# ap229997/hands

Measured on AMD Instinct MI355X. Metric: hands/sec, higher is better.
Workload: dtype f32; 1 GPU; hands_light ResNet-50 x3 + feature_conv + HMR + MANO, 224x224, bz=256 samples/GPU (512 hands, 768 trunk passes); per_gpu_batch=256, global_batch=256, parallelism=dp1, rccl_ranks=1, launched_by=direct, conv3x3_stride1=winograd_f4x4:stages1234

## Files before the change

### hands_amd/_lib.py

```python
from __future__ import annotations

import ctypes as C
import os

_HERE = os.path.dirname(os.path.abspath(__file__))
LIB_PATH = os.environ.get("HANDS_HIP_LIB") or os.path.join(_HERE, "libhands_hip.so")

c_float_p = C.c_void_p


class ConvDesc(C.Structure):
    _fields_ = [(n, C.c_int32) for n in (
        "B", "H", "W", "Cin", "Ho", "Wo", "Cout", "KH", "KW", "stride", "pad",
        "in_pix_stride", "out_pix_stride", "res_pix_stride", "Kpad", "act")]


ACT_NONE, ACT_RELU, ACT_GELU, ACT_LEAKY_RELU = 0, 1, 2, 3


class ManoConsts(C.Structure):
    _fields_ = [("pose_mean", C.c_void_p), ("J_template", C.c_void_p), ("J_shapedirs", C.c_void_p),
                ("lbs_weights", C.c_void_p), ("tip_ids", C.c_void_p)]


class ManoOut(C.Structure):
    _fields_ = [("vertices", C.c_void_p), ("joints3d", C.c_void_p), ("v3d_cam", C.c_void_p),
                ("j3d_cam", C.c_void_p), ("j2d_norm", C.c_void_p), ("cam_t", C.c_void_p)]


class ManoSide(C.Structure):
    _fields_ = [("consts", ManoConsts), ("blend_w", C.c_void_p), ("blend_bias", C.c_void_p), ("rot", C.c_void_p),
                ("betas", C.c_void_p), ("cam_wp", C.c_void_p), ("out", ManoOut)]


class PackedDims(C.Structure):
    _fields_ = [(n, C.c_int32) for n in ("Cin", "Cout", "Cout_pad", "Kpad")]


class EvalIn(C.Structure):
    _fields_ = [(n, C.c_void_p) for n in (
        "pred_j3d_r", "pred_j3d_l", "gt_j3d_r", "gt_j3d_l", "pred_j2d_r", "pred_j2d_l", "gt_j2d_r", "gt_j2d_l",
        "is_valid", "right_valid", "left_valid", "joints_valid_r", "joints_valid_l")]


class EvalOut(C.Structure):
    _fields_ = [(n, C.c_void_p) for n in (
        "mpjpe_ra_h", "mpjpe_pa_ra_r", "mpjpe_pa_ra_l", "mpjpe_pa_ra_h", "mrrpe_rl", "pix_err_r", "pix_err_l")]


class EvalMaskedOut(C.Structure):
    _fields_ = [(n, C.c_void_p) for n in (
        "rao_r", "rao_l", "rao_h", "abs_r", "abs_l", "abs_h", "pa_ra_r", "pa_ra_l", "pa_ra_h")]


class MeshEvalIn(C.Structure):
    _fields_ = [(n, C.c_void_p) for n in (
        "pred_v3d_r", "pred_v3d_l", "gt_v3d_r", "gt_v3d_l", "pred_j3d_r", "pred_j3d_l", "gt_j3d_r", "gt_j3d_l",
        "is_valid", "right_valid", "left_valid")]


MESH_MAX_V, MESH_NQ = 1024, 10
MESH_QUANTITIES = ("mpvpe_ra", "f5_ra", "f15_ra", "auc_ra_v", "auc_ra_j", "mpvpe_pa", "f5_pa", "f15_pa", "auc_pa_v", "auc_pa_j")


class MeshEvalOut(C.Structure):
    _fields_ = [(f"{q}_{s}", C.c_void_p) for q in MESH_QUANTITIES for s in "rlh"]


SURF_MAX_F, SURF_CHUNK, SURF_NQ = 4096, 512, 4
SIGNED_CHUNK = 256
SURF_QUANTITIES = ("p2s_ra", "p2s_pa", "chamfer_ra", "chamfer_pa")


class SurfEvalOut(C.Structure):
    _fields_ = [(f"{q}_{s}", C.c_void_p) for q in SURF_QUANTITIES for s in "rlh"]


ACCEL_NQ = 3
ACCEL_QUANTITIES = ("acc", "acc_j", "acc_abs")


class AccelEvalOut(C.Structure):
    _fields_ = [(f"{q}_{s}", C.c_void_p) for q in ACCEL_QUANTITIES for s in "rlh"]


class SmoothSide(C.Structure):
    _fields_ = [(n, C.c_void_p) for n in ("pose", "beta", "cam", "valid", "pose_out", "beta_out", "cam_out", "state")]


SMOOTH_SHAPE_MODES = {"filter": 0, "mean": 1, "none": 2}


class SmoothCfg(C.Structure):
    _fields_ = [("min_cutoff", C.c_double * 3), ("beta", C.c_double * 3), ("d_cutoff", C.c_double * 3), ("shape_mode", C.c_int)]


class ManoFitConsts(C.Structure):
    _fields_ = [(n, C.c_void_p) for n in ("pose_mean", "J_template", "J_shapedirs", "tip_v_template", "tip_shapedirs",
                                          "tip_lbs_weights", "tip_posedirs")]


class ManoFitSide(C.Structure):
    _fields_ = [("consts", ManoFitConsts)] + [(n, C.c_void_p) for n in (
        "joints", "weights", "valid", "init_pose", "init_beta", "init_transl", "pose", "beta", "transl", "rmse", "steps")]


class FitCfg(C.Structure):
    _fields_ = [("iters", C.c_int), ("lambda_beta", C.c_double), ("lambda_pose", C.c_double), ("mu0", C.c_double)]


class ManoFit2DSide(C.Structure):
    _fields_ = [("consts", ManoFitConsts)] + [(n, C.c_void_p) for n in (
        "kp2d", "weights", "valid", "init_pose", "init_beta", "init_transl", "pose", "beta", "transl", "rmse", "steps", "start",
        "j3d", "j2d")]


class Fit2DCfg(C.Structure):
    _fields_ = [("iters_rigid", C.c_int), ("iters", C.c_int), ("lambda_beta", C.c_double), ("lambda_pose", C.c_double),
                ("mu0", C.c_double), ("robust_sigma", C.c_double), ("z_min", C.c_double), ("fit_shape", C.c_int),
                ("prior_to_init", C.c_int)]


class ManoFitVertsConsts(C.Structure):
    _fields_ = [(n, C.c_void_p) for n in ("pose_mean", "J_template", "J_shapedirs", "v_template", "shapedirs", "lbs_weights",
                                          "posedirs_vm")]


class ManoFitVertsSide(C.Structure):
    _fields_ = [("consts", ManoFitVertsConsts)] + [(n, C.c_void_p) for n in (
        "verts", "weights", "valid", "init_pose", "init_beta", "init_transl", "pose", "beta", "transl", "rmse", "steps", "j3d")]


class LossIn(C.Structure):
    _fields_ = [(n, C.c_void_p) for n in (
        "pred_pose_r", "pred_pose_l", "pred_beta_r", "pred_beta_l", "pred_j3d_r", "pred_j3d_l", "pred_j2d_r", "pred_j2d_l",
        "pred_cam_wp_r", "pred_cam_wp_l", "pred_cam_wp_init_r", "pred_cam_wp_init_l",
        "gt_pose_r", "gt_pose_l", "gt_beta_r", "gt_beta_l", "gt_j3d_r", "gt_j3d_l", "gt_j2d_r", "gt_j2d_l",
        "gt_cam_wp_r", "gt_cam_wp_l", "right_valid", "left_valid", "joints_valid_r", "joints_valid_l",
        "is_cam_loss", "is_j2d_loss", "is_j3d_loss", "is_pose_loss", "is_beta_loss",
        "pred_grasp_r", "pred_grasp_l", "gt_grasp_r", "gt_grasp_l", "grasp_valid_r", "grasp_valid_l", "is_grasp_loss",
        "pred_mask_r", "pred_mask_l", "gt_mask_r", "gt_mask_l", "render_valid_r", "render_valid_l", "is_mask_loss",
        "pred_depth_r", "pred_depth_l", "gt_depth_r", "gt_depth_l", "is_depth_loss",
        "pred_center_r", "pred_center_l", "gt_center_r", "gt_center_l",
        "pred_corner_r", "pred_corner_l", "gt_corner_r", "gt_corner_l")]


LOSS_NKEYS, LOSS_N_MANDATORY = 21, 31


class ShadeMesh(C.Structure):
    _fields_ = [("workspace", C.c_void_p), ("faces", C.c_void_p), ("valid", C.c_void_p), ("n_verts", C.c_int32),
                ("n_faces", C.c_int32), ("face_offset", C.c_int32), ("color", C.c_float * 3), ("metallic", C.c_float),
                ("roughness", C.c_float)]


SHADE_MAX_MESHES = 4


class ShadeScene(C.Structure):
    _fields_ = [("mesh", ShadeMesh * SHADE_MAX_MESHES), ("n_meshes", C.c_int32)]


_P, _I, _F = C.c_void_p, C.c_int, C.c_float
class ConvJob(C.Structure):
    _fields_ = [("desc", C.POINTER(ConvDesc)), ("in_", C.c_void_p), ("w_packed", C.c_void_p), ("bias", C.c_void_p),
                ("residual", C.c_void_p), ("out", C.c_void_p), ("pre_scale", C.c_void_p), ("pre_shift", C.c_void_p)]


SIGNATURES = {
    "hands_conv2d_nhwc_f32": [C.POINTER(ConvDesc), _P, _P, _P, _P, _P, _P],
    "hands_conv3x3_winograd_supported": [C.POINTER(ConvDesc)],
    "hands_conv3x3_winograd_f32": [C.POINTER(ConvDesc), _P, _P, _P, _P, _P],
    "hands_conv3x3_winograd4_supported": [C.POINTER(ConvDesc)],
    "hands_conv3x3_winograd4_f32": [C.POINTER(ConvDesc), _P, _P, _P, _P, _P],
    "hands_conv2d_splitk_factor": [C.POINTER(ConvDesc)],
    "hands_conv2d_group_class": [C.POINTER(ConvDesc), _I],
    "hands_conv2d_group_f32": [C.POINTER(ConvJob), _I, _P],
    "hands_conv2d_nhwc_splitk_f32": [C.POINTER(ConvDesc), _P, _P, _P, _P, _P, _P, C.c_longlong, _P],
    "hands_conv2d_nhwc_splitk_fused_f32": [C.POINTER(ConvDesc), _P, _P, _P, _P, _P, _I, _P, C.c_longlong, _P, C.c_longlong, _P],
    "hands_conv2d_streamk_grid": [C.POINTER(ConvDesc)],
    "hands_conv2d_nhwc_streamk_f32": [C.POINTER(ConvDesc), _P, _P, _P, _P, _P, _P, C.c_longlong, _I, _P],
    "hands_conv1x1_dual_nhwc_f32": [C.POINTER(ConvDesc), _P, _P, _I, _I, _I, _I, _I, _P, _P, _P, _P],
    "hands_conv2d_nhwc_splitk_n_f32": [C.POINTER(ConvDesc), _P, _P, _P, _P, _P, _I, _P, C.c_longlong, _P],
    "hands_conv2d_nhwc_pre_f32": [C.POINTER(ConvDesc), _P, _P, _P, _P, _P, _P, _P, _I, _P, C.c_longlong, _P],
    "hands_stem_conv_maxpool_nhwc_f32": [_P, _P, _P, _P, _I, _I, _I, _I, _P],
    "hands_stem_conv_maxpool_nchw_f32": [_P, _P, _P, _P, _I, _I, _I, _I, _P],
    "hands_nchw3_to_nhwc4_f32": [_P, _P, _I, _I, _I, _P],
    "hands_maxpool3x3s2_nhwc_f32": [_P, _P, _I, _I, _I, _I, _P],
    "hands_sumpool_nhwc_f32": [_P, _P, _I, _I, _I, _I, _P],
    "hands_avgpool_nhwc_f32": [_P, _P, _I, _I, _I, _I, _P],
    "hands_image_posenc_nhwc_f32": [_P, _P, _P, _P, _I, _I, _I, _I, _I, _I, _P],
    "hands_frontend_dense_maps_f32": [_P, _P, _P, _P, _I, _I, _I, _P],
    "hands_dense_posenc_f32": [_P, _P, _P, _P, _I, _I, _I, _I, _I, _I, _I, _I, _I, _I, _P],
    "hands_concat_nhwc_f32": [_P, _I, _I, _P, _I, _P, C.c_longlong, _I, _P, _I, _I, _I, _I, _P],
    "hands_upsample_bilinear_ac_f32": [_P, _P, _I, _I, _I, _I, _I, _I, _P],
    "hands_rot_leftmul_f32": [_P, _P, _I, _P],
    "hands_perspective_correction_f32": [_P, _P, _P, _P, _I, _P],
    "hands_kpe_concat_f32": [_P, _P, _P, _P, _P, _I, _I, _I, _I, _I, _P],
    "hands_hmr_init_f32": [_P, _P, _I, _I, _I, _P],
    "hands_rot6d_to_matrix_f32": [_P, _I, _P, _I, _P],
    "hands_flip_swap_f32": [_P, _P, _P, _P, _P, _P, _P, _P, _P, _I, _P],
    "hands_matrix_to_axis_angle_f32": [_P, _P, C.c_longlong, _P],
    "hands_axis_angle_to_matrix_f32": [_P, _P, C.c_longlong, _P],
    "hands_grasp_input_f32": [_P, _I, _P, _P, _P, _I, _I, _I, _I, _P],
    "hands_mano_pose_f32": [C.POINTER(ManoConsts), _P, _P, _I, _P, _I, _P, _P, _I, _P],
    "hands_mano_heads_f32": [C.POINTER(ManoSide), _I, _P, _I, _F, _F, _I, _I, _P],
    "hands_mano_heads_vsplit": [_I, _I],
    "hands_mano_skin_f32": [C.POINTER(ManoConsts), _P, _I, _P, _P, _P, _P, _F, _F, C.POINTER(ManoOut), _I, _P],
    "hands_resize_crop_nchw3_to_nhwc4_f32": [_P, _P, _I, _I, _I, _I, _I, _I, _P],
    "hands_layernorm_f32": [_P, _P, _P, _P, _P, _I, _I, _I, _F, _P],
    "hands_add_pos_f32": [_P, _P, _P, _I, _I, _I, _P],
    "hands_kpe_encode_f32": [_P, _P, _P, _I, _I, _I, _P],
    "hands_attention_f32": [_P, _P, _I, _I, _I, _I, _F, _P],
    "hands_cross_attention_1q_f32": [_P, _P, _P, _I, _I, _I, _I, _F, _P],
    "hands_rot6d_to_matrix_cols_f32": [_P, _I, _P, _I, _P],
    "hands_vit_tokens_f32": [_P, _P, _P, _P, _I, _I, _I, _P],
    "hands_vit_tail_f32": [_P, _P, _P, _P, _I, _I, _I, _F, _P],
    "hands_wide_attention_f32": [_P, C.c_longlong, _I, _P, C.c_longlong, _I, _P, C.c_longlong, _I, _P, C.c_longlong, _I,
                                 _I, _I, _I, _I, _F, _P],
    "hands_vector_tokens_f32": [_P, _I, _I, _I, _P, _P, _P, _I, _I, _I, _P],
    "hands_token_mean_f32": [_P, _P, _I, _I, _I, _P],
    "hands_upsample_bilinear_add_f32": [_P, _P, _P, _I, _I, _I, _I, _I, _I, _P],
    "hands_pool2x2_nhwc_f32": [_P, _P, _I, _I, _I, _I, _I, _P],
    "hands_channel_pool_f32": [_P, _P, C.c_longlong, _I, _P],
    "hands_gate_apply_f32": [_P, _P, _I, _P, _P, C.c_longlong, _I, _P],
    "hands_add_embed2_f32": [_P, _P, _P, _P, _P, _P, _P, _I, _I, _I, _P],
    "hands_add_rowvec_f32": [_P, _P, _P, _I, _I, _I, _P],
    "hands_token_sum_f32": [_P, _P, _I, _I, _I, _P],
    "hands_bn_leaky_f32": [_P, _P, _P, _P, C.c_longlong, _I, _P],
    "hands_upsample_nearest2x_add_f32": [_P, _P, _P, _I, _I, _I, _I, _P],
    "hands_spatial_softmax_f32": [_P, _I, _P, _P, _I, _I, _I, _I, _P],
    "hands_flash_attention_f32": [_P, _P, _P, _P, _P, _P, _P, _I, _I, _I, _I, _F, _P],
    "hands_ceiling_hbm_read_f32": [_P, C.c_longlong, _P, _P],
    "hands_eval_metrics_f32": [C.POINTER(EvalIn), C.POINTER(EvalOut), _I, _P],
    "hands_eval_metrics_masked_f32": [C.POINTER(EvalIn), _P, _P, C.POINTER(EvalMaskedOut), _I, _P],
    "hands_eval_mesh_metrics_f32": [C.POINTER(MeshEvalIn), C.POINTER(MeshEvalOut), _I, _I, _P],
    "hands_mesh_closest_f32": [_P, _P, _P, _P, _P, _P, _P, _I, _I, _I, _I, _P],
    "hands_mesh_signed_f32": [_P, _P, _P, _P, _P, _P, _P, _I, _I, _I, _I, _P],
    "hands_eval_surface_metrics_f32": [C.POINTER(MeshEvalIn), _P, _P, _I, _I, C.POINTER(SurfEvalOut), _I, _I, _P],
    "hands_accel_error_f32": [_P, _P, _P, _P, _P, _I, _I, _I, _F, _P],
    "hands_eval_accel_metrics_f32": [C.POINTER(MeshEvalIn), _P, C.POINTER(AccelEvalOut), _I, _I, _F, _P],
    "hands_smooth_mano_f32": [C.POINTER(SmoothSide), _I, _P, _I, _I, _F, C.POINTER(SmoothCfg), _P],
    "hands_mano_fit_f32": [C.POINTER(ManoFitSide), _I, C.POINTER(FitCfg), _I, _P],
    "hands_mano_fit2d_f32": [C.POINTER(ManoFit2DSide), _I, _P, C.POINTER(Fit2DCfg), _I, _P],
    "hands_mano_fit_verts_f32": [C.POINTER(ManoFitVertsSide), _I, C.POINTER(FitCfg), _I, _P],
    "hands_loss_light_f32": [C.POINTER(LossIn), _I, _I, _I, _P, _P, _P, _P, _P],
    "hands_mano_pose_aa_f32": [C.POINTER(ManoConsts), _P, _P, _I, _P, _I, _P, _P, _I, _P],
    "hands_gt_targets_f32": [_P, _P, _P, _P, _F, _P, _P, _P, _I, _I, _P],
    "hands_unnormalize_kp2d_f32": [_P, _P, C.c_longlong, _F, _P],
    "hands_frontend_boxes_f32": [_P, _P, _I, _P, _I, _I, _I, C.c_double] + [_P] * 10 + [_P],
    "hands_warp_affine_cubic_norm_f32": [_P, _P, _P, _I, _I, _I, _I, _I, C.POINTER(C.c_float), C.POINTER(C.c_float), _P],
    "hands_render_silhouette_f32": [_P, _I, _I, _P, _I, _P, _I, _I, _F, _F, _I, _P, _P, _P, _P],
    "hands_mesh_prepare_f32": [_P, _I, _I, _P, _I, _P, _P, _P, _P, _I, _I, _P, _P],
    "hands_render_shaded_f32": [C.POINTER(ShadeScene), _P, _I, _I, _P, _P, _P, _P, _P],
    "hands_pack_conv_dims": [_I, _I, _I, _I, _I, C.POINTER(PackedDims)],
    "hands_fold_bn_f32": [_I, C.c_longlong, _P, _P, _P, _P, _P, C.c_double, _P, _P],
    "hands_pack_conv_f64": [_I, _I, _I, _I, _I, _P, _P, _P, _P],
    "hands_pack_linear_f64": [_I, _I, _P, _P, _P, _I, _P, _I, _P, _P],
    "hands_pack_conv1x1_dual_f64": [_I, _I, _I, _P, _P, _P, _P, _P, _P],
    "hands_pack_mano_f32": [_P] * 10,
    "hands_pack_conv3x3_winograd_f64": [_I, _I, _P, _P],
    "hands_pack_conv3x3_winograd4_f64": [_I, _I, _P, _P],
}
EXTRA_SYMBOLS = ("hands_abi_version", "hands_error_string", "hands_conv2d_workspace_floats", "hands_pack_conv3x3_winograd_floats", "hands_conv3x3_winograd_executed_macs",
                 "hands_pack_conv3x3_winograd4_floats", "hands_conv3x3_winograd4_executed_macs",
                 "hands_conv2d_streamk_workspace_bytes", "hands_stream_is_capturing", "hands_csrc_sha16", "hands_ceiling_mfma_f32", "hands_mesh_workspace_floats",
                 "hands_loss_workspace_bytes", "hands_smooth_state_bytes")

ABI_VERSION = 5
_lib = None


def lib():
    global _lib
    if _lib is not None:
        return _lib
    if not os.path.isfile(LIB_PATH):
        raise RuntimeError(
            f"hands_amd: {LIB_PATH} not found. Build it with `python -c 'import __graft_entry__ as g; "
            "g.build()'` or `make -C hands_amd/csrc`. There is no CPU fallback.")
    h = C.CDLL(LIB_PATH)
    h.hands_abi_version.restype = C.c_int
    if h.hands_abi_version() != ABI_VERSION:
        raise RuntimeError(f"hands_amd: {LIB_PATH} has ABI version {h.hands_abi_version()}, this package needs {ABI_VERSION}: "
                           "rebuild it (`make -C hands_amd/csrc`)")
    for name, argtypes in SIGNATURES.items():
        fn = getattr(h, name)
        fn.argtypes = argtypes
        fn.restype = C.c_int
    h.hands_conv2d_workspace_floats.restype = C.c_longlong
    h.hands_conv2d_workspace_floats.argtypes = [C.POINTER(ConvDesc), C.c_int]
    h.hands_conv2d_streamk_workspace_bytes.restype = C.c_longlong
    h.hands_conv2d_streamk_workspace_bytes.argtypes = []
    h.hands_pack_conv3x3_winograd_floats.restype = C.c_longlong
    h.hands_pack_conv3x3_winograd_floats.argtypes = [C.c_int, C.c_int]
    h.hands_conv3x3_winograd_executed_macs.restype = C.c_longlong
    h.hands_conv3x3_winograd_executed_macs.argtypes = [C.POINTER(ConvDesc)]
    h.hands_pack_conv3x3_winograd4_floats.restype = C.c_longlong
    h.hands_pack_conv3x3_winograd4_floats.argtypes = [C.c_int, C.c_int]
    h.hands_conv3x3_winograd4_executed_macs.restype = C.c_longlong
    h.hands_conv3x3_winograd4_executed_macs.argtypes = [C.POINTER(ConvDesc)]
    h.hands_abi_version.restype = C.c_int
    h.hands_stream_is_capturing.restype = C.c_int
    h.hands_stream_is_capturing.argtypes = [C.c_void_p]
    h.hands_csrc_sha16.restype = C.c_char_p
    h.hands_csrc_sha16.argtypes = []
    h.hands_ceiling_mfma_f32.restype = C.c_longlong
    h.hands_ceiling_mfma_f32.argtypes = [C.c_void_p, C.c_longlong, C.c_int, C.c_int, C.c_void_p]
    h.hands_mesh_workspace_floats.restype = C.c_longlong
    h.hands_mesh_workspace_floats.argtypes = [C.c_int, C.c_int]
    h.hands_loss_workspace_bytes.restype = C.c_longlong
    h.hands_loss_workspace_bytes.argtypes = [C.c_int, C.c_int, C.c_int]
    h.hands_smooth_state_bytes.restype = C.c_longlong
    h.hands_smooth_state_bytes.argtypes = []
    h.hands_error_string.restype = C.c_char_p
    h.hands_error_string.argtypes = [C.c_int]
    _lib = h
    return h


def check(code: int, what: str = ""):
    if code != 0:
        msg = lib().hands_error_string(code).decode()
        raise RuntimeError(f"hands_amd: {what} failed with code {code}: {msg}")


def ptr(t, offset_elems: int = 0):
    if t is None:
        return None
    return t.data_ptr() + offset_elems * t.element_size()
```

### hands_amd/csrc/conv_igemm.hip

```cpp
#include <hip/hip_runtime.h>
#include <stdint.h>
#include "hands_hip.h"
#include "common.h"

namespace {

typedef unsigned int u32x4 __attribute__((ext_vector_type(4)));
typedef double f64x4 __attribute__((ext_vector_type(4)));

__device__ __forceinline__ float gelu_erf(float x) { return x * 0.5f * (1.0f + erff(x * 0.70710678118654752440f)); }

__device__ __forceinline__ float4 apply_act(float4 v, int act) {
  if (act == HANDS_ACT_RELU) {
    v = relu_f32(v);
  } else if (act == HANDS_ACT_GELU) {
    v.x = gelu_erf(v.x); v.y = gelu_erf(v.y); v.z = gelu_erf(v.z); v.w = gelu_erf(v.w);
  } else if (act == HANDS_ACT_LEAKY_RELU) {
    v.x = v.x > 0.f ? v.x : 0.01f * v.x; v.y = v.y > 0.f ? v.y : 0.01f * v.y;
    v.z = v.z > 0.f ? v.z : 0.01f * v.z; v.w = v.w > 0.f ? v.w : 0.01f * v.w;
  }
  return v;
}

__device__ __forceinline__ float f4elem(const float4& v, int t) {
  return t == 0 ? v.x : (t == 1 ? v.y : (t == 2 ? v.z : v.w));
}

constexpr int BK = 16;
constexpr int LDS_ROW = 16;
constexpr int LDS_ROW_B3 = 24;

typedef __bf16 bf16x8 __attribute__((ext_vector_type(8)));

__device__ __forceinline__ void split3(float x, uint32_t& u0, uint32_t& u1, uint32_t& u2) {
  u0 = __float_as_uint(x) & 0xffff0000u;
  const float r1 = x - __uint_as_float(u0);
  u1 = __float_as_uint(r1) & 0xffff0000u;
  const float r2 = r1 - __uint_as_float(u1);
  u2 = __float_as_uint(r2);
}

__device__ __forceinline__ void store_split4(float* dst, float4 v) {
  uint32_t a0, a1, a2, b0, b1, b2, c0, c1, c2, d0, d1, d2;
  split3(v.x, a0, a1, a2); split3(v.y, b0, b1, b2); split3(v.z, c0, c1, c2); split3(v.w, d0, d1, d2);
  *reinterpret_cast<uint2*>(dst) = make_uint2((a0 >> 16) | b0, (c0 >> 16) | d0);
  *reinterpret_cast<uint2*>(dst + 8) = make_uint2((a1 >> 16) | b1, (c1 >> 16) | d1);
  *reinterpret_cast<uint2*>(dst + 16) = make_uint2((a2 >> 16) | (b2 & 0xffff0000u), (c2 >> 16) | (d2 & 0xffff0000u));
}

struct ConvArgs {
  const float* __restrict__ in;
  const float* __restrict__ w;
  const float* __restrict__ bias;
  const float* res;
  float* out;
  int M, N, Kpad;
  int H, W, Cin, Ho, Wo, KH, KW, stride, pad;
  int in_ps, out_ps, res_ps;
  int relu;
  int nblk_m, nblk_n;
  const float* __restrict__ in2;
  int K0, H2, W2, stride2, in2_ps;
  int ksplit;
  float* partial;
  int part_ps;
  const float* pre_scale;
  const float* pre_shift;
  int* counters = nullptr;
  const float* fin_res = nullptr;
  int fin_act = 0;
};

__device__ __forceinline__ int xcd_remap(int bid, int nwg) {
  const int q = nwg >> 3, r = nwg & 7;
  const int xcd = bid & 7, idx = bid >> 3;
  const int base = (xcd < r) ? xcd * (q + 1) : r * (q + 1) + (xcd - r) * q;
  return base + idx;
}

typedef float f32x2 __attribute__((ext_vector_type(2)));

constexpr int EROW = 68;
constexpr int EPI_FLOATS = 4 * 32 * EROW;
template <int ACT, bool RES>
__device__ __forceinline__ void epilogue_full(const f32x16 (&acc)[2][2], float* sE, int lane, const float* bias_p,
                                              const char* res_u, int res_ps, char* out_u, int out_ps) {
  const int half = lane >> 5;
  float* wr = sE + (lane & 31) * EROW + half * 4;
  const float* rd = sE + (lane >> 4) * EROW + (lane & 15) * 4;
  const uint32_t o_off = (uint32_t)((lane >> 4) * out_ps + (lane & 15) * 4) * 4u;
  const uint32_t r_off = (uint32_t)((lane >> 4) * res_ps + (lane & 15) * 4) * 4u;
  const float4 bv4 = *reinterpret_cast<const float4*>(bias_p);
#ifndef HANDS_EPI_SCALAR_ADDS
  const f32x2 b01 = {bv4.x, bv4.y}, b23 = {bv4.z, bv4.w};
#endif
#pragma unroll
  for (int j = 0; j < 2; ++j) {
#pragma unroll
    for (int i = 0; i < 2; ++i)
#pragma unroll
      for (int q = 0; q < 4; ++q)
        *reinterpret_cast<float4*>(wr + i * 32 + q * 8) =
            make_float4(acc[i][j][q * 4 + 0], acc[i][j][q * 4 + 1], acc[i][j][q * 4 + 2], acc[i][j][q * 4 + 3]);
    float4 rv[RES ? 8 : 1];
    if constexpr (RES) {
#pragma unroll
      for (int r = 0; r < 8; ++r)
        rv[r] = *reinterpret_cast<const float4*>(res_u + (size_t)(j * 32 + 4 * r) * (size_t)res_ps * 4 + r_off);
    }
#pragma unroll
    for (int r = 0; r < 8; ++r) {
      const float4 t = *reinterpret_cast<const float4*>(rd + 4 * r * EROW);
#ifdef HANDS_EPI_SCALAR_ADDS
      float4 v = make_float4(t.x + bv4.x, t.y + bv4.y, t.z + bv4.z, t.w + bv4.w);
      if constexpr (RES) { v.x += rv[r].x; v.y += rv[r].y; v.z += rv[r].z; v.w += rv[r].w; }
      asm volatile("" : "+v"(v.x), "+v"(v.y), "+v"(v.z), "+v"(v.w));
#else
      f32x2 v01 = {t.x, t.y}, v23 = {t.z, t.w};
      v01 = v01 + b01;
      v23 = v23 + b23;
      if constexpr (RES) {
        const f32x2 r01 = {rv[r].x, rv[r].y}, r23 = {rv[r].z, rv[r].w};
        v01 = v01 + r01;
        v23 = v23 + r23;
      }
      float4 v = make_float4(v01.x, v01.y, v23.x, v23.y);
#endif
      if constexpr (ACT != HANDS_ACT_NONE) v = apply_act(v, ACT);
      *reinterpret_cast<float4*>(out_u + (size_t)(j * 32 + 4 * r) * (size_t)out_ps * 4 + o_off) = v;
      if (r & 1) __builtin_amdgcn_sched_barrier(0);
    }
  }
}

template <int BM, int BN, bool F64>
__device__ __forceinline__ void splitk_fused_tail(const ConvArgs& a, float* lds, int tile, int m0, int n0, int wave_u) {
  const int tid = wave_u * 64 + (int)__builtin_amdgcn_mbcnt_hi(~0u, __builtin_amdgcn_mbcnt_lo(~0u, 0u));
  volatile int& s_last = *reinterpret_cast<volatile int*>(lds);
  asm volatile("s_waitcnt vmcnt(0)" ::: "memory");
  __syncthreads();
  if (tid == 0) {
    __builtin_amdgcn_fence(__ATOMIC_RELEASE, "agent");
    asm volatile("s_waitcnt vmcnt(0)" ::: "memory");
    const int old = __hip_atomic_fetch_add(a.counters + tile, 1, __ATOMIC_RELAXED, __HIP_MEMORY_SCOPE_AGENT);
    const int last = old == a.ksplit - 1;
    if (last) __hip_atomic_store(a.counters + tile, 0, __ATOMIC_RELAXED, __HIP_MEMORY_SCOPE_AGENT);
    s_last = last;
  }
  __syncthreads();
  if (!s_last) return;
  __builtin_amdgcn_fence(__ATOMIC_ACQUIRE, "agent");
  const size_t slice = (size_t)a.M * a.part_ps;
  if constexpr (F64) {
    const double* part = reinterpret_cast<const double*>(a.partial);
    for (int idx = tid; idx < BM * BN; idx += 256) {
      const int m = m0 + idx / BN, n = n0 + idx % BN;
      if (m >= a.M || n >= a.N) continue;
      const double* p = part + (size_t)m * a.part_ps + n;
      double v = p[0];
      for (int sl = 1; sl < a.ksplit; ++sl) v += p[sl * slice];
      float f = (float)(v + (double)a.bias[n]);
      if (a.fin_res) f += a.fin_res[(size_t)m * a.res_ps + n];
      if (a.fin_act == HANDS_ACT_RELU) f = relu_f32(f);
      else if (a.fin_act == HANDS_ACT_GELU) f = gelu_erf(f);
      else if (a.fin_act == HANDS_ACT_LEAKY_RELU) f = f > 0.f ? f : 0.01f * f;
      a.out[(size_t)m * a.out_ps + n] = f;
    }
  } else {
    constexpr int C4 = BN / 4;
    for (int idx = tid; idx < BM * C4; idx += 256) {
      const int m = m0 + idx / C4, n = n0 + (idx % C4) * 4;
      if (m >= a.M || n >= a.N) continue;
      const float* p = a.partial + (size_t)m * a.part_ps + n;
      float4 v = *reinterpret_cast<const float4*>(p);
      for (int sl = 1; sl < a.ksplit; ++sl) {
        const float4 q = *reinterpret_cast<const float4*>(p + sl * slice);
        v.x += q.x; v.y += q.y; v.z += q.z; v.w += q.w;
      }
      const float4 b = *reinterpret_cast<const float4*>(a.bias + n);
      v.x += b.x; v.y += b.y; v.z += b.z; v.w += b.w;
      if (a.fin_res) {
        const float4 r = *reinterpret_cast<const float4*>(a.fin_res + (size_t)m * a.res_ps + n);
        v.x += r.x; v.y += r.y; v.z += r.z; v.w += r.w;
      }
      *reinterpret_cast<float4*>(a.out + (size_t)m * a.out_ps + n) = apply_act(v, a.fin_act);
    }
  }
}

constexpr int SK_SLOT_FLOATS = 4 * 64 * 64;

__device__ __forceinline__ void tile_coords(const ConvArgs& a, int tile, int& mt, int& nt) {
  constexpr int RASTER_GM = 8;
  if (a.nblk_n >= 8 && a.nblk_m >= RASTER_GM) {
    const int per = RASTER_GM * a.nblk_n;
    const int gidx = tile / per, idx = tile - gidx * per;
    const int gm = min(RASTER_GM, a.nblk_m - gidx * RASTER_GM);
    nt = idx / gm; mt = gidx * RASTER_GM + (idx - nt * gm);
  } else { mt = tile / a.nblk_n; nt = tile - mt * a.nblk_n; }
}

template <int WAVES_M, int WAVES_N, int MODE, int PREC = 0, bool PRE = false, int BLK = 0>
__device__ __forceinline__ void conv_tile(const ConvArgs& a, float* lds, int tile, int split, int kt0, int kt1,
                                          const float* acc_in, float* acc_out) {
  constexpr int ROW = PREC == 1 ? LDS_ROW_B3 : LDS_ROW;
  constexpr bool F64 = PREC == 2;
  constexpr bool STEM = MODE == 1;
  constexpr bool DUAL = MODE == 2;
  constexpr int BM = 64 * WAVES_M;
  constexpr int BN = 64 * WAVES_N;
  constexpr int A_ROWS = BM / 64;
  constexpr int W_ROWS = BN / 64;
  static_assert(WAVES_M * WAVES_N == 4, "4 waves per block");

  float* sX = lds;
  float* sW = lds + 2 * BM * ROW;

  const int tid = threadIdx.x;
  const int lane = tid & 63;
  const int wave = tid >> 6;
  const int wm = wave / WAVES_N;
  const int wn = wave % WAVES_N;

  int mt, nt;
  tile_coords(a, tile, mt, nt);
  const int m0 = mt * BM, n0 = nt * BN;

  const int srow = tid >> 2;
  const int chunk = tid & 3;
  const int swz_chunk = chunk ^ ((srow >> 2) & 3);
  int x_base[A_ROWS];
  int x_hi0[A_ROWS], x_wi0[A_ROWS];
  bool x_ok[A_ROWS];
  int x_base2[DUAL ? A_ROWS : 1];
  uint32_t x_mask[MODE == 0 ? A_ROWS : 1];
  int x_offb[MODE == 0 ? A_ROWS : 1];
  int x_b[A_ROWS];
  const int HoWo = a.Ho * a.Wo;
  const bool same_pixel = DUAL && a.K0 >= a.Kpad && a.stride == 1 && a.H == a.Ho && a.W == a.Wo;
#pragma unroll
  for (int i = 0; i < A_ROWS; ++i) {
    const int m = m0 + srow + 64 * i;
    x_ok[i] = m < a.M;
    const int mm = x_ok[i] ? m : 0;
    if (same_pixel) {
      x_b[i] = 0; x_hi0[i] = 0; x_wi0[i] = 0;
      x_base[i] = mm * a.in_ps;
      if constexpr (DUAL) x_base2[i] = 0;
      continue;
    }
    const int b = mm / HoWo;
    const int rem = mm - b * HoWo;
    const int ho = rem / a.Wo;
    const int wo = rem - ho * a.Wo;
    x_b[i] = b;
    x_hi0[i] = ho * a.stride - a.pad;
    x_wi0[i] = wo * a.stride - a.pad;
    x_base[i] = ((b * a.H + x_hi0[i]) * a.W + x_wi0[i]) * a.in_ps;
    if constexpr (DUAL) {
      x_base2[i] = ((b * a.H2 + ho * a.stride2) * a.W2 + wo * a.stride2) * a.in2_ps;
    }
  }
  __amdgpu_buffer_rsrc_t x_rsrc = __builtin_amdgcn_make_buffer_rsrc(const_cast<float*>(a.in), 0, (int)0x80000000u, 0x00020000);
  if constexpr (MODE == 0) {
    const int b_w = __builtin_amdgcn_readfirstlane(x_b[0]);
    x_rsrc = __builtin_amdgcn_make_buffer_rsrc(const_cast<float*>(a.in) + (size_t)b_w * a.H * a.W * a.in_ps, 0,
                                               (int)0x80000000u, 0x00020000);
#pragma unroll
    for (int i = 0; i < A_ROWS; ++i) {
      const int hb = max(0, -x_hi0[i]), he = min(a.KH, a.H - x_hi0[i]);
      const int wb = max(0, -x_wi0[i]), we = min(a.KW, a.W - x_wi0[i]);
      const uint32_t hm = he > hb ? ((1u << he) - 1u) & ~((1u << hb) - 1u) : 0u;
      const uint32_t wm = we > wb ? ((1u << we) - 1u) & ~((1u << wb) - 1u) : 0u;
      x_mask[i] = (x_ok[i] && hm != 0u && wm != 0u) ? (hm | (wm << 16)) : 0u;
      x_offb[i] = (((((x_b[i] - b_w) * a.H + x_hi0[i]) * a.W + x_wi0[i]) * a.in_ps) + chunk * 4) * 4;
    }
  }
  int x_off1[DUAL ? A_ROWS : 1], x_off2[DUAL ? A_ROWS : 1];
  __amdgpu_buffer_rsrc_t x_rsrc2 = x_rsrc;
  if constexpr (DUAL) {
    const int base1 = __builtin_amdgcn_readfirstlane(x_base[0]);
    const int base2 = __builtin_amdgcn_readfirstlane(x_base2[0]);
    x_rsrc = __builtin_amdgcn_make_buffer_rsrc(const_cast<float*>(a.in) + base1, 0, (int)0x80000000u, 0x00020000);
    x_rsrc2 = __builtin_amdgcn_make_buffer_rsrc(const_cast<float*>(a.in2) + base2, 0, (int)0x80000000u, 0x00020000);
#pragma unroll
    for (int i = 0; i < A_ROWS; ++i) {
      x_off1[i] = x_ok[i] ? (x_base[i] - base1 + chunk * 4) * 4 : chunk * 16;
      x_off2[i] = x_ok[i] ? (x_base2[i] - base2 + chunk * 4) * 4 : chunk * 16;
    }
  }
  const __amdgpu_buffer_rsrc_t w_rsrc =
      __builtin_amdgcn_make_buffer_rsrc(const_cast<float*>(a.w) + (size_t)n0 * a.Kpad, 0, (int)0x80000000u, 0x00020000);
  int w_offb[W_ROWS];
#pragma unroll
  for (int i = 0; i < W_ROWS; ++i) w_offb[i] = ((srow + 64 * i) * a.Kpad + chunk * 4) * 4;

  float4 xr[A_ROWS], wr[W_ROWS];
  static_assert(!PRE || (MODE == 2 && PREC != 1), "the input affine + LeakyReLU exists for exact-fp32 pointwise layers");
  float4 psr = make_float4(1.f, 1.f, 1.f, 1.f), pbr = make_float4(0.f, 0.f, 0.f, 0.f);
  int kh = 0, kw = 0, c0 = 0, woff = 0;
  const int ntaps = a.KH * a.KW;
  const int cw = (a.Cin & 31) == 0 ? 2 * BK : BK;

#define LOAD_TILES(KT)                                                                              \
  do {                                                                                              \
    if constexpr (STEM) {                                                                           \
                                          \
      const int tap = (KT) * 4 + chunk;                                                             \
      const int tkh = tap / a.KW;                                                                   \
      const int tkw = tap - tkh * a.KW;                                                             \
      const int toff = (tkh * a.W + tkw) * a.in_ps;                                                 \
      _Pragma("unroll") for (int i = 0; i < A_ROWS; ++i) {                                          \
        const bool ok = x_ok[i] && tap < ntaps && (unsigned)(x_hi0[i] + tkh) < (unsigned)a.H &&     \
                        (unsigned)(x_wi0[i] + tkw) < (unsigned)a.W;                                 \
        xr[i] = ok ? *reinterpret_cast<const float4*>(a.in + (x_base[i] + toff))                    \
                   : make_float4(0.f, 0.f, 0.f, 0.f);                                               \
      }                                                                                             \
    } else if constexpr (DUAL) {                                                                    \
       \
       \
       \
      const bool second = (KT) * BK >= a.K0;                                                        \
      const int soff = ((KT) * BK - (second ? a.K0 : 0)) * 4;                                       \
      _Pragma("unroll") for (int i = 0; i < A_ROWS; ++i) {                                          \
        const u32x4 ld = second ? __builtin_amdgcn_raw_buffer_load_b128(x_rsrc2, x_off2[i], soff, 0) \
                                : __builtin_amdgcn_raw_buffer_load_b128(x_rsrc, x_off1[i], soff, 0);  \
        xr[i] = make_float4(__uint_as_float(ld.x), __uint_as_float(ld.y), __uint_as_float(ld.z), __uint_as_float(ld.w)); \
      }                                                                                             \
    } else {                                                                                        \
       \
       \
       \
      const bool kvalid = c0 < a.Cin;              \
      const uint32_t sel = kvalid ? ((1u << kh) | (0x10000u << kw)) : 0x80000000u;   \
      const int toffb = ((kh * a.W + kw) * a.in_ps + c0) * 4;                                       \
      _Pragma("unroll") for (int i = 0; i < A_ROWS; ++i) {                                          \
        const bool ok = (x_mask[i] & sel) == sel;                                                   \
        const u32x4 ld = __builtin_amdgcn_raw_buffer_load_b128(x_rsrc, ok ? x_offb[i] + toffb : (int)0x80000000u, 0, 0); \
        xr[i] = make_float4(__uint_as_float(ld.x), __uint_as_float(ld.y), __uint_as_float(ld.z), __uint_as_float(ld.w)); \
      }                                                                                             \
      woff = kvalid ? (kh * a.KW + kw) * a.Cin + c0 : (KT) * BK;                                    \
      c0 += BK;                                                                                     \
      if ((c0 & (cw - 1)) == 0) {              \
        c0 -= cw;                                                                                   \
        if (++kw == a.KW) { kw = 0; if (++kh == a.KH) { kh = 0; c0 += cw; } }                       \
      }                                                                                             \
    }                                                                                               \
    if constexpr (MODE != 0) woff = (KT) * BK;                                                      \
    if constexpr (PRE) {                                                                            \
      psr = *reinterpret_cast<const float4*>(a.pre_scale + (KT) * BK + chunk * 4);                  \
      pbr = *reinterpret_cast<const float4*>(a.pre_shift + (KT) * BK + chunk * 4);                  \
    }                                                                                               \
    _Pragma("unroll") for (int i = 0; i < W_ROWS; ++i) {                                            \
      const u32x4 ld = __builtin_amdgcn_raw_buffer_load_b128(w_rsrc, w_offb[i], woff * 4, 0);        \
      wr[i] = make_float4(__uint_as_float(ld.x), __uint_as_float(ld.y), __uint_as_float(ld.z), __uint_as_float(ld.w)); \
    }                                                                                               \
  } while (0)

#define STORE_TILES(BUF)                                                                            \
  do {                                                                                              \
    if constexpr (PRE) {                                                                            \
      _Pragma("unroll") for (int i = 0; i < A_ROWS; ++i) {                                          \
        float4 v = make_float4(xr[i].x * psr.x + pbr.x, xr[i].y * psr.y + pbr.y, xr[i].z * psr.z + pbr.z, xr[i].w * psr.w + pbr.w); \
        v.x = v.x > 0.f ? v.x : 0.01f * v.x; v.y = v.y > 0.f ? v.y : 0.01f * v.y;                   \
        v.z = v.z > 0.f ? v.z : 0.01f * v.z; v.w = v.w > 0.f ? v.w : 0.01f * v.w;                   \
        xr[i] = v;                                                                                  \
      }                                                                                             \
    }                                                                                               \
    if constexpr (PREC != 1) {                                                                      \
      float* dx = sX + (BUF) * BM * ROW + srow * ROW + swz_chunk * 4;                               \
      float* dw = sW + (BUF) * BN * ROW + srow * ROW + swz_chunk * 4;                               \
      _Pragma("unroll") for (int i = 0; i < A_ROWS; ++i)                                            \
        *reinterpret_cast<float4*>(dx + 64 * i * ROW) = xr[i];                                      \
      _Pragma("unroll") for (int i = 0; i < W_ROWS; ++i)                                            \
        *reinterpret_cast<float4*>(dw + 64 * i * ROW) = wr[i];                                      \
    } else {                                                                                        \
      float* dx = sX + (BUF) * BM * ROW + srow * ROW + chunk * 2;                                   \
      float* dw = sW + (BUF) * BN * ROW + srow * ROW + chunk * 2;                                   \
      _Pragma("unroll") for (int i = 0; i < A_ROWS; ++i) store_split4(dx + 64 * i * ROW, xr[i]);    \
      _Pragma("unroll") for (int i = 0; i < W_ROWS; ++i) store_split4(dw + 64 * i * ROW, wr[i]);    \
    }                                                                                               \
  } while (0)

  f64x4 accd[F64 ? 4 : 1][F64 ? 4 : 1];
  if constexpr (F64) {
#pragma unroll
    for (int i = 0; i < 4; ++i)
#pragma unroll
      for (int j = 0; j < 4; ++j) accd[i][j] = f64x4{0.0, 0.0, 0.0, 0.0};
  }
  f32x16 acc[2][2];
  if (acc_in != nullptr) {
    const float4* src = reinterpret_cast<const float4*>(acc_in) + (wave * 16) * 64 + lane;
#pragma unroll
    for (int i = 0; i < 2; ++i)
#pragma unroll
      for (int j = 0; j < 2; ++j)
#pragma unroll
        for (int q = 0; q < 4; ++q) {
          const float4 v = src[((i * 2 + j) * 4 + q) * 64];
          acc[i][j][q * 4 + 0] = v.x; acc[i][j][q * 4 + 1] = v.y; acc[i][j][q * 4 + 2] = v.z; acc[i][j][q * 4 + 3] = v.w;
        }
  } else {
#pragma unroll
    for (int i = 0; i < 2; ++i)
#pragma unroll
      for (int j = 0; j < 2; ++j)
#pragma unroll
        for (int r = 0; r < 16; ++r) acc[i][j][r] = 0.f;
  }

  if constexpr (MODE == 0) {
    if (kt0 > 0) {
      const int spt = cw / BK;
      const int ch0 = kt0 / (ntaps * spt);
      const int r0 = kt0 - ch0 * ntaps * spt;
      const int tap0 = r0 / spt;
      c0 = ch0 * cw + (r0 - tap0 * spt) * BK;
      kh = tap0 / a.KW;
      kw = tap0 - kh * a.KW;
    }
  }
#ifdef HANDS_PRO_PRIO
  __builtin_amdgcn_s_setprio(HANDS_PRO_PRIO);
#endif
  LOAD_TILES(kt0);
  STORE_TILES(0);
  __syncthreads();
#ifdef HANDS_PRO_PRIO
  __builtin_amdgcn_s_setprio(0);
#endif

  const int frag = PREC == 1 ? (lane & 31) * ROW + (lane >> 5) * 4
                   : F64     ? (lane & 15) * ROW + (((lane >> 4) ^ ((lane >> 2) & 3)) * 4)
                             : (lane & 31) * ROW + (((lane >> 5) ^ ((lane >> 2) & 3)) * 4);
  const float* fw = sW + (wn * 64) * ROW + frag;
  const float* fx = sX + (wm * 64) * ROW + frag;
  const float* fw1 = sW + (wn * 64) * ROW + (frag ^ 8);
  const float* fx1 = sX + (wm * 64) * ROW + (frag ^ 8);

#define COMPUTE_STEP(BUF)                                                                           \
  do {                                                                                              \
    if constexpr (F64) {                                                                            \
      float4 wf[4], xf[4];                 \
      _Pragma("unroll") for (int i = 0; i < 4; ++i) {                                               \
        wf[i] = *reinterpret_cast<const float4*>(fw + (BUF) * BN * ROW + i * 16 * ROW);             \
        xf[i] = *reinterpret_cast<const float4*>(fx + (BUF) * BM * ROW + i * 16 * ROW);             \
      }                                                                                             \
      _Pragma("unroll") for (int t = 0; t < 4; ++t) {                                               \
        double wd[4], xd[4];                                                                        \
        _Pragma("unroll") for (int i = 0; i < 4; ++i) {                                             \
          wd[i] = (double)f4elem(wf[i], t);                                                         \
          xd[i] = (double)f4elem(xf[i], t);                                                         \
        }                                                                                           \
        _Pragma("unroll") for (int i = 0; i < 4; ++i) {                                             \
          _Pragma("unroll") for (int j = 0; j < 4; ++j) {                                           \
            accd[i][j] = __builtin_amdgcn_mfma_f64_16x16x4f64(wd[i], xd[j], accd[i][j], 0, 0, 0);   \
          }                                                                                         \
        }                                                                                           \
      }                                                                                             \
    } else if constexpr (PREC == 0) {                                                               \
      float4 wf[2][2], xf[2][2];                                            \
      _Pragma("unroll") for (int kk = 0; kk < 2; ++kk) {                                            \
        _Pragma("unroll") for (int i = 0; i < 2; ++i) {                                             \
          wf[i][kk] = *reinterpret_cast<const float4*>((kk ? fw1 : fw) + (BUF) * BN * ROW + i * 32 * ROW); \
          xf[i][kk] = *reinterpret_cast<const float4*>((kk ? fx1 : fx) + (BUF) * BM * ROW + i * 32 * ROW); \
        }                                                                                           \
      }                                                                                             \
      _Pragma("unroll") for (int kk = 0; kk < 2; ++kk) {                                            \
        _Pragma("unroll") for (int t = 0; t < 4; ++t) {                                             \
          _Pragma("unroll") for (int i = 0; i < 2; ++i) {                                           \
            _Pragma("unroll") for (int j = 0; j < 2; ++j) {                                         \
              acc[i][j] = __builtin_amdgcn_mfma_f32_32x32x2f32(f4elem(wf[i][kk], t), f4elem(xf[j][kk], t), \
                                                               acc[i][j], 0, 0, 0);                  \
            }                                                                                       \
          }                                                                                         \
        }                                                                                           \
      }                                                                                             \
    } else {                                                                                        \
        \
      bf16x8 wf[2][3], xf[2][3];                                         \
      _Pragma("unroll") for (int p = 0; p < 3; ++p) {                                               \
        _Pragma("unroll") for (int i = 0; i < 2; ++i) {                                             \
          wf[i][p] = *reinterpret_cast<const bf16x8*>(fw + (BUF) * BN * ROW + i * 32 * ROW + p * 8); \
          xf[i][p] = *reinterpret_cast<const bf16x8*>(fx + (BUF) * BM * ROW + i * 32 * ROW + p * 8); \
        }                                                                                           \
      }                                                                                             \
                             \
      _Pragma("unroll") for (int q = 0; q < 6; ++q) {                                               \
        constexpr int PA[6] = {2, 1, 0, 1, 0, 0};                                                   \
        constexpr int PB[6] = {0, 1, 2, 0, 1, 0};                                                   \
        _Pragma("unroll") for (int i = 0; i < 2; ++i) {                                             \
          _Pragma("unroll") for (int j = 0; j < 2; ++j) {                                           \
            acc[i][j] = __builtin_amdgcn_mfma_f32_32x32x16_bf16(wf[i][PA[q]], xf[j][PB[q]], acc[i][j], 0, 0, 0); \
          }                                                                                         \
        }                                                                                           \
      }                                                                                             \
    }                                                                                               \
  } while (0)

  static_assert(BLK == 0 || ((BLK & (BLK - 1)) == 0 && PREC == 0), "block length: a power of two k-steps, exact fp32 only");
  static_assert(!F64 || (WAVES_M == 2 && WAVES_N == 2), "fp64 accumulation: the 128 x 128 tile only");
  f32x16 tot[BLK ? 2 : 1][BLK ? 2 : 1];
  if constexpr (BLK > 0) {
#pragma unroll
    for (int i = 0; i < 2; ++i)
#pragma unroll
      for (int j = 0; j < 2; ++j)
#pragma unroll
        for (int r = 0; r < 16; ++r) tot[i][j][r] = 0.f;
  }
  for (int kt = kt0; kt + 1 < kt1; ++kt) {
    const int buf = (kt - kt0) & 1;
    LOAD_TILES(kt + 1);
    COMPUTE_STEP(buf);
    if constexpr (BLK > 0) {
      if (((kt - kt0 + 1) & (BLK - 1)) == 0) {
#pragma unroll
        for (int i = 0; i < 2; ++i)
#pragma unroll
          for (int j = 0; j < 2; ++j)
#pragma unroll
            for (int r = 0; r < 16; ++r) { tot[i][j][r] += acc[i][j][r]; acc[i][j][r] = 0.f; }
      }
    }
    STORE_TILES(buf ^ 1);
    __syncthreads();
  }
  COMPUTE_STEP((kt1 - 1 - kt0) & 1);
#ifdef HANDS_EPI_PRIO
  __builtin_amdgcn_s_setprio(HANDS_EPI_PRIO);
#endif
  if constexpr (BLK > 0) {
#pragma unroll
    for (int i = 0; i < 2; ++i)
#pragma unroll
      for (int j = 0; j < 2; ++j)
#pragma unroll
        for (int r = 0; r < 16; ++r) acc[i][j][r] += tot[i][j][r];
  }
#undef COMPUTE_STEP

  __syncthreads();
  if (acc_out != nullptr) {
    float4* dst = reinterpret_cast<float4*>(acc_out) + (wave * 16) * 64 + lane;
#pragma unroll
    for (int i = 0; i < 2; ++i)
#pragma unroll
      for (int j = 0; j < 2; ++j)
#pragma unroll
        for (int q = 0; q < 4; ++q)
          dst[((i * 2 + j) * 4 + q) * 64] =
              make_float4(acc[i][j][q * 4 + 0], acc[i][j][q * 4 + 1], acc[i][j][q * 4 + 2], acc[i][j][q * 4 + 3]);
    return;
  }
  float* sE = lds + wave * (32 * EROW);
  const int half = lane >> 5;
  const int c4 = lane & 15;
  const int n_lane = n0 + wn * 64 + c4 * 4;
  const bool n_ok = n_lane < a.N;
  const bool part = a.ksplit > 1;
#ifdef HANDS_ABL_NO_EPI
  if (!part && m0 + BM <= a.M && n0 + BN <= a.N) {
    float sacc = 0.f;
#pragma unroll
    for (int i = 0; i < 2; ++i)
#pragma unroll
      for (int j = 0; j < 2; ++j) sacc += acc[i][j][0] + acc[i][j][7] + acc[i][j][15];
    if (sacc == 123456.789f) a.out[(size_t)m0 * a.out_ps + n0 + lane] = sacc;
    return;
  }
#endif
  if (!F64 && !part && m0 + BM <= a.M && n0 + BN <= a.N) {
    const int wave_u = __builtin_amdgcn_readfirstlane(wave);
    const int mw = m0 + (wave_u / WAVES_N) * 64, nw = n0 + (wave_u % WAVES_N) * 64;
    char* ou = reinterpret_cast<char*>(a.out) + ((size_t)mw * a.out_ps + nw) * 4;
    const char* ru = reinterpret_cast<const char*>(a.res) + ((size_t)mw * a.res_ps + nw) * 4;
    const float* bp = a.bias + n_lane;
#define HANDS_EPI(ACT)                                                                            \
    if (a.res != nullptr) epilogue_full<ACT, true>(acc, sE, lane, bp, ru, a.res_ps, ou, a.out_ps); \
    else                  epilogue_full<ACT, false>(acc, sE, lane, bp, ru, a.res_ps, ou, a.out_ps)
    if (a.relu == HANDS_ACT_RELU) { HANDS_EPI(HANDS_ACT_RELU); }
    else if (a.relu == HANDS_ACT_NONE) { HANDS_EPI(HANDS_ACT_NONE); }
    else if (a.relu == HANDS_ACT_LEAKY_RELU) { HANDS_EPI(HANDS_ACT_LEAKY_RELU); }
    else { HANDS_EPI(HANDS_ACT_GELU); }
#undef HANDS_EPI
    return;
  }
  const float4 bv = (part || F64) ? make_float4(0.f, 0.f, 0.f, 0.f) : *reinterpret_cast<const float4*>(a.bias + n_lane);
  double bd[F64 ? 4 : 1][F64 ? 4 : 1];
  if constexpr (F64) {
#pragma unroll
    for (int i = 0; i < 4; ++i)
#pragma unroll
      for (int r = 0; r < 4; ++r) {
        const int ch = n0 + wn * 64 + 16 * i + (lane >> 4) + 4 * r;
        bd[i][r] = (!part && ch < a.N) ? (double)a.bias[ch] : 0.0;
      }
    if (part) {
      double* pd = reinterpret_cast<double*>(a.partial) + (size_t)split * a.M * a.part_ps;
#pragma unroll
      for (int i = 0; i < 4; ++i)
#pragma unroll
        for (int jb = 0; jb < 4; ++jb)
#pragma unroll
          for (int r = 0; r < 4; ++r) {
            const int ch = n0 + wn * 64 + 16 * i + (lane >> 4) + 4 * r;
            const int m = m0 + wm * 64 + 16 * jb + (lane & 15);
            if (m < a.M && ch < a.N) pd[(size_t)m * a.part_ps + ch] = accd[i][jb][r];
          }
      return;
    }
  }
  const bool has_res = !part && a.res != nullptr;
  const int act = part ? HANDS_ACT_NONE : a.relu;
  float* const obase = part ? a.partial + (size_t)split * a.M * a.part_ps : a.out;
  const int ops = part ? a.part_ps : a.out_ps;
#pragma unroll
  for (int j = 0; j < 2; ++j) {
    if constexpr (F64) {
#pragma unroll
      for (int i = 0; i < 4; ++i)
#pragma unroll
        for (int jj = 0; jj < 2; ++jj)
#pragma unroll
          for (int r = 0; r < 4; ++r)
            sE[(jj * 16 + (lane & 15)) * EROW + 16 * i + (lane >> 4) + 4 * r] = (float)(accd[i][2 * j + jj][r] + bd[i][r]);
    } else {
#pragma unroll
    for (int i = 0; i < 2; ++i)
#pragma unroll
      for (int q = 0; q < 4; ++q)
        *reinterpret_cast<float4*>(sE + (lane & 31) * EROW + i * 32 + q * 8 + half * 4) =
            make_float4(acc[i][j][q * 4 + 0], acc[i][j][q * 4 + 1], acc[i][j][q * 4 + 2], acc[i][j][q * 4 + 3]);
    }
    const int mbase = m0 + wm * 64 + j * 32 + (lane >> 4);
    float4 rv[8];
#pragma unroll
    for (int r = 0; r < 8; ++r) {
      const int m = mbase + 4 * r;
      const int mc = m < a.M ? m : a.M - 1;
      rv[r] = has_res ? *reinterpret_cast<const float4*>(a.res + (size_t)mc * a.res_ps + (n_ok ? n_lane : 0))
                      : make_float4(0.f, 0.f, 0.f, 0.f);
    }
#pragma unroll
    for (int r = 0; r < 8; ++r) {
      const int m = mbase + 4 * r;
      const float4 t = *reinterpret_cast<const float4*>(sE + ((lane >> 4) + 4 * r) * EROW + c4 * 4);
      float4 v;
      v.x = t.x + bv.x + rv[r].x;
      v.y = t.y + bv.y + rv[r].y;
      v.z = t.z + bv.z + rv[r].z;
      v.w = t.w + bv.w + rv[r].w;
      v = apply_act(v, act);
      if (m < a.M && n_ok) *reinterpret_cast<float4*>(obase + (size_t)m * ops + n_lane) = v;
    }
  }
#undef LOAD_TILES
#undef STORE_TILES
}

template <int WAVES_M, int WAVES_N, int MODE, int PREC = 0, bool PRE = false, int BLK = 0>
__global__ void __launch_bounds__(256, 2) conv_igemm_f32_kernel(ConvArgs a) {
  constexpr int RING = 2 * (64 * WAVES_M + 64 * WAVES_N) * (PREC == 1 ? LDS_ROW_B3 : LDS_ROW);
  __shared__ __attribute__((aligned(16))) float lds[RING > EPI_FLOATS ? RING : EPI_FLOATS];
  const int ntiles = a.nblk_m * a.nblk_n;
  const int split = a.ksplit > 1 ? blockIdx.x / ntiles : 0;
  const int tile = xcd_remap(a.ksplit > 1 ? blockIdx.x - split * ntiles : blockIdx.x, ntiles);
  const int nk_all = a.Kpad / BK;
  const int kt0 = a.ksplit > 1 ? (int)((long long)split * nk_all / a.ksplit) : 0;
  const int kt1 = a.ksplit > 1 ? (int)((long long)(split + 1) * nk_all / a.ksplit) : nk_all;
  const int wave_u = __builtin_amdgcn_readfirstlane((int)(threadIdx.x >> 6));
  conv_tile<WAVES_M, WAVES_N, MODE, PREC, PRE, BLK>(a, lds, tile, split, kt0, kt1, nullptr, nullptr);
  if (a.ksplit > 1 && a.counters != nullptr) {
    int mt, nt;
    tile_coords(a, tile, mt, nt);
    splitk_fused_tail<64 * WAVES_M, 64 * WAVES_N, PREC == 2>(a, lds, tile, mt * 64 * WAVES_M, nt * 64 * WAVES_N, wave_u);
  }
}

constexpr int GROUP_MAX = 8;
struct GroupArgs {
  ConvArgs a[GROUP_MAX];
  int start[GROUP_MAX + 1];
  int n;
};

template <int WAVES_M, int WAVES_N, int MODE, bool PRE, int BLK>
__global__ void __launch_bounds__(256, 2) conv_igemm_group_f32_kernel(GroupArgs g) {
  constexpr int RING = 2 * (64 * WAVES_M + 64 * WAVES_N) * LDS_ROW;
  __shared__ __attribute__((aligned(16))) float lds[RING > EPI_FLOATS ? RING : EPI_FLOATS];
  int p = 0;
#pragma unroll
  for (int i = 1; i < GROUP_MAX; ++i)
    if (i < g.n && (int)blockIdx.x >= g.start[i]) p = i;
  const ConvArgs& a = g.a[p];
  const int ntiles = a.nblk_m * a.nblk_n;
  const int local = (int)blockIdx.x - g.start[p];
  if ((local >> 3) >= (ntiles >> 3) + ((local & 7) < (ntiles & 7) ? 1 : 0)) return;
  conv_tile<WAVES_M, WAVES_N, MODE, 0, PRE, BLK>(a, lds, xcd_remap(local, ntiles), 0, 0, a.Kpad / BK, nullptr, nullptr);
}

struct SkArgs {
  float* slots;
  int* flags;
  int epoch;
};

template <int WAVES_M, int WAVES_N, int MODE>
__global__ void __launch_bounds__(256, 2) conv_igemm_sk_f32_kernel(ConvArgs a, SkArgs sk) {
  constexpr int RING = 2 * (64 * WAVES_M + 64 * WAVES_N) * LDS_ROW;
  __shared__ __attribute__((aligned(16))) float lds[RING > EPI_FLOATS ? RING : EPI_FLOATS];
  __shared__ int s_ready;
  const int G = gridDim.x;
  const int g = xcd_remap(blockIdx.x, G);
  const int ntiles = a.nblk_m * a.nblk_n;
  const int nk = a.Kpad / BK;
  const long long total = (long long)ntiles * nk;
  const long long u0 = total * g / G, u1 = total * (g + 1) / G;
  const int ta = (int)(u0 / nk), ka = (int)(u0 - (long long)ta * nk);
  const int tb = (int)(u1 / nk), kb = (int)(u1 - (long long)tb * nk);

  const bool inside = ta == tb;
  const int first_full = ka > 0 ? ta + 1 : ta;
  const int nfull = inside ? 0 : tb - first_full;
  const int head = (!inside && kb > 0) ? 1 : 0;
  const int nseg = inside ? 1 : head + nfull + (ka > 0 ? 1 : 0);
  for (int sgi = 0; sgi < nseg; ++sgi) {
    int tile, k0 = 0, k1 = nk;
    const float* ain = nullptr;
    float* aout = nullptr;
    if (sgi < head) {
      tile = tb; k1 = kb;
      aout = sk.slots + (size_t)g * SK_SLOT_FLOATS;
    } else if (sgi - head < nfull) {
      tile = first_full + (sgi - head);
    } else if (inside && ka == 0) {
      tile = ta; k1 = kb;
      aout = sk.slots + (size_t)g * SK_SLOT_FLOATS;
    } else {
      if (threadIdx.x == 0) {
        int ok = 0;
        for (int spin = 0; spin < 4096 && !ok; ++spin) {
          ok = __hip_atomic_load(sk.flags + (g - 1), __ATOMIC_RELAXED, __HIP_MEMORY_SCOPE_AGENT) == sk.epoch;
          if (!ok) __builtin_amdgcn_s_sleep(8);
        }
        if (ok) __builtin_amdgcn_fence(__ATOMIC_ACQUIRE, "agent");
        s_ready = ok;
      }
      __syncthreads();
      tile = ta;
      if (s_ready != 0) { k0 = ka; ain = sk.slots + (size_t)(g - 1) * SK_SLOT_FLOATS; }
      if (inside) { k1 = kb; aout = sk.slots + (size_t)g * SK_SLOT_FLOATS; }
    }
    __syncthreads();
    conv_tile<WAVES_M, WAVES_N, MODE>(a, lds, tile, 0, k0, k1, ain, aout);
    if (aout != nullptr) {
      asm volatile("s_waitcnt vmcnt(0)" ::: "memory");
      __syncthreads();
      if (threadIdx.x == 0) {
        __builtin_amdgcn_fence(__ATOMIC_RELEASE, "agent");
        asm volatile("s_waitcnt vmcnt(0)" ::: "memory");
        if (sk.epoch > 0) __hip_atomic_store(sk.flags + g, sk.epoch, __ATOMIC_RELAXED, __HIP_MEMORY_SCOPE_AGENT);
      }
    }
  }
}

template <int WAVES_M, int WAVES_N, int MODE, int PREC = 0, bool PRE = false, int BLK = 0>
int launch(ConvArgs& a, hipStream_t stream) {
  constexpr int BM = 64 * WAVES_M, BN = 64 * WAVES_N;
  a.nblk_m = (a.M + BM - 1) / BM;
  a.nblk_n = (a.N + BN - 1) / BN;
  const long long nwg = (long long)a.nblk_m * a.nblk_n * (a.ksplit > 1 ? a.ksplit : 1);
  if (nwg <= 0 || nwg > 0x7fffffffLL) return HANDS_EINVAL;
  hipLaunchKernelGGL((conv_igemm_f32_kernel<WAVES_M, WAVES_N, MODE, PREC, PRE, BLK>), dim3((unsigned)nwg), dim3(256), 0,
                     stream, a);
  return (int)hipGetLastError();
}

template <int MODE, bool PRE = false>
int launch_fp32(const hands_conv_desc* d, ConvArgs& a, hipStream_t s) {
  const bool narrow = d->Cout <= 64;
  if (d->act & HANDS_ACC_F64) return launch<2, 2, MODE, 2, PRE>(a, s);
  if (d->act & HANDS_SUM_BLOCK128) return narrow ? launch<4, 1, MODE, 0, PRE, 8>(a, s) : launch<2, 2, MODE, 0, PRE, 8>(a, s);
  if (d->act & HANDS_SUM_BLOCK64) return narrow ? launch<4, 1, MODE, 0, PRE, 4>(a, s) : launch<2, 2, MODE, 0, PRE, 4>(a, s);
  return narrow ? launch<4, 1, MODE, 0, PRE>(a, s) : launch<2, 2, MODE, 0, PRE>(a, s);
}

constexpr int SK_MAX_G = 1024;

int device_cus() {
  static int cus = 0;
  if (cus == 0) {
    int dev = 0, n = 0;
    if (hipGetDevice(&dev) == hipSuccess &&
        hipDeviceGetAttribute(&n, hipDeviceAttributeMultiprocessorCount, dev) == hipSuccess && n > 0)
      cus = n;
    else
      cus = 256;
  }
  return cus;
}

template <int WAVES_M, int WAVES_N, int MODE>
int sk_blocks_per_cu() {
  static int occ = 0;
  if (occ == 0) {
    int n = 0;
    if (hipOccupancyMaxActiveBlocksPerMultiprocessor(&n, conv_igemm_sk_f32_kernel<WAVES_M, WAVES_N, MODE>, 256, 0) != hipSuccess || n < 1)
      n = 1;
    occ = n > 4 ? 4 : n;
  }
  return occ;
}

int streamk_grid(long long ntiles, int nk, int cus, int max_per_cu) {
  if (ntiles > cus + cus / 8 && ntiles < 2LL * cus && nk >= 128 && max_per_cu >= 2) {
    return 2 * cus;
  }
  if (nk < 16 || ntiles < 2LL * cus || ntiles > 8LL * cus) return 0;
  const double per_cu = (double)ntiles / cus;
  const long long rounds = (ntiles + cus - 1) / cus;
  if (per_cu / (double)rounds > 0.95) return 0;
  long long j = ntiles / cus;
  if (j > max_per_cu) j = max_per_cu;
  long long G = j * cus;
  if (G > SK_MAX_G) G = SK_MAX_G / cus * cus;
  return G >= cus ? (int)G : 0;
}

template <int WAVES_M, int WAVES_N, int MODE>
int launch_streamk(ConvArgs& a, hipStream_t stream, void* workspace, long long workspace_bytes, int epoch) {
  constexpr int BM = 64 * WAVES_M, BN = 64 * WAVES_N;
  a.nblk_m = (a.M + BM - 1) / BM;
  a.nblk_n = (a.N + BN - 1) / BN;
  const long long ntiles = (long long)a.nblk_m * a.nblk_n;
  const int G = (workspace && epoch != 0 && a.ksplit <= 1)
                    ? streamk_grid(ntiles, a.Kpad / BK, device_cus(), sk_blocks_per_cu<WAVES_M, WAVES_N, MODE>()) : 0;
  const long long need = (long long)G * SK_SLOT_FLOATS * 4 + (long long)SK_MAX_G * 4;
  if (G == 0 || workspace_bytes < need) return launch<WAVES_M, WAVES_N, MODE>(a, stream);
  SkArgs sk;
  sk.flags = reinterpret_cast<int*>(workspace);
  sk.slots = reinterpret_cast<float*>(reinterpret_cast<char*>(workspace) + SK_MAX_G * 4);
  sk.epoch = epoch;
  hipLaunchKernelGGL((conv_igemm_sk_f32_kernel<WAVES_M, WAVES_N, MODE>), dim3((unsigned)G), dim3(256), 0, stream, a, sk);
  return (int)hipGetLastError();
}

__global__ void splitk_reduce_kernel(const float* __restrict__ partial, int S, int M, int N4, int part_ps,
                                     const float* __restrict__ bias, const float* res, int res_ps, float* out, int out_ps,
                                     int act) {
  const long long total = (long long)M * N4;
  for (long long i = blockIdx.x * (long long)blockDim.x + threadIdx.x; i < total; i += (long long)gridDim.x * blockDim.x) {
    const int n = (int)(i % N4) * 4;
    const long long m = i / N4;
    float4 v = *reinterpret_cast<const float4*>(partial + m * part_ps + n);
    for (int s = 1; s < S; ++s) {
      const float4 p = *reinterpret_cast<const float4*>(partial + ((long long)s * M + m) * part_ps + n);
      v.x += p.x; v.y += p.y; v.z += p.z; v.w += p.w;
    }
    const float4 b = *reinterpret_cast<const float4*>(bias + n);
    v.x += b.x; v.y += b.y; v.z += b.z; v.w += b.w;
    if (res) {
      const float4 r = *reinterpret_cast<const float4*>(res + m * res_ps + n);
      v.x += r.x; v.y += r.y; v.z += r.z; v.w += r.w;
    }
    *reinterpret_cast<float4*>(out + m * out_ps + n) = apply_act(v, act);
  }
}

__global__ void splitk_reduce_f64_kernel(const double* __restrict__ partial, int S, int M, int N, int part_ps,
                                         const float* __restrict__ bias, const float* res, int res_ps, float* out, int out_ps,
                                         int act) {
  const long long total = (long long)M * N;
  for (long long i = blockIdx.x * (long long)blockDim.x + threadIdx.x; i < total; i += (long long)gridDim.x * blockDim.x) {
    const int n = (int)(i % N);
    const long long m = i / N;
    double v = partial[m * part_ps + n];
    for (int s = 1; s < S; ++s) v += partial[((long long)s * M + m) * part_ps + n];
    float f = (float)(v + (double)bias[n]);
    if (res) f += res[m * res_ps + n];
    if (act == HANDS_ACT_RELU) f = relu_f32(f);
    else if (act == HANDS_ACT_GELU) f = gelu_erf(f);
    else if (act == HANDS_ACT_LEAKY_RELU) f = f > 0.f ? f : 0.01f * f;
    out[m * out_ps + n] = f;
  }
}

int splitk_factor(const hands_conv_desc* d) {
  if (d->KH != 1 || d->KW != 1 || d->H != 1 || d->W != 1 || d->stride != 1 || d->pad != 0 || d->Cin == 4) return 1;
  const long long M = d->B;
  if (M > 2048 || d->Kpad < 512) return 1;
  int s = d->Kpad / 256;
  return s > 8 ? 8 : s;
}

bool conv_geometry_ok(const hands_conv_desc* d) {
  if (d->B <= 0 || d->H <= 0 || d->W <= 0 || d->Ho <= 0 || d->Wo <= 0 || d->KH <= 0 || d->KW <= 0 || d->stride <= 0 ||
      d->pad < 0)
    return false;
  if ((d->act & HANDS_ACT_MASK) > HANDS_ACT_LEAKY_RELU || (d->act & ~(HANDS_ACT_MASK | HANDS_MATH_BF16X3 | HANDS_SUM_BLOCK128 | HANDS_SUM_BLOCK64 | HANDS_ACC_F64))) return false;
  if ((d->act & HANDS_ACC_F64) && ((d->act & (HANDS_MATH_BF16X3 | HANDS_SUM_BLOCK128 | HANDS_SUM_BLOCK64)) || d->Cin == 4)) return false;
  if ((d->act & HANDS_SUM_BLOCK128) && (d->act & (HANDS_SUM_BLOCK64 | HANDS_MATH_BF16X3))) return false;
  if ((d->act & HANDS_SUM_BLOCK64) && (d->act & HANDS_MATH_BF16X3)) return false;
  if (d->Cin % 4 || d->Cout % 4 || d->Kpad % BK || d->Kpad < d->KH * d->KW * d->Cin) return false;
  if (d->Cin != 4 && d->Cin % 16) return false;
  if (d->in_pix_stride < d->Cin || d->out_pix_stride < d->Cout) return false;
  if (d->in_pix_stride % 4 || d->out_pix_stride % 4) return false;
  if (d->H + 2 * d->pad < d->KH || d->W + 2 * d->pad < d->KW) return false;
  if (d->Ho > (d->H + 2 * d->pad - d->KH) / d->stride + 1 || d->Wo > (d->W + 2 * d->pad - d->KW) / d->stride + 1) return false;
  if ((long long)d->B * d->H * d->W * d->in_pix_stride >= (1LL << 31)) return false;
  if (d->Cin != 4) {
    const long long imgs = 256 / ((long long)d->Ho * d->Wo) + 2;
    if (imgs * d->H * d->W * d->in_pix_stride * 4 >= (1LL << 31)) return false;
    if (256LL * d->Kpad * 4 >= (1LL << 31)) return false;
    if (!(d->KH == 1 && d->KW == 1 && d->pad == 0) && (d->KH > 15 || d->KW > 15)) return false;
  }
  return true;
}

bool residual_ok(const hands_conv_desc* d, const float* residual) {
  return residual == nullptr || (d->res_pix_stride >= 0 && d->res_pix_stride % 4 == 0);
}

bool pointwise_route_ok(const hands_conv_desc* d) {
  return d->KH == 1 && d->KW == 1 && d->pad == 0 && d->Cin != 4 && d->Kpad == d->Cin &&
         (long long)(d->Ho - 1) * d->stride < d->H && (long long)(d->Wo - 1) * d->stride < d->W;
}

void fill_plain_args(const hands_conv_desc* d, const float* in, const float* w_packed, const float* bias, const float* residual,
                     float* out, const float* pre_scale, const float* pre_shift, ConvArgs& a) {
  a.in = in; a.w = w_packed; a.bias = bias; a.res = residual; a.out = out;
  a.M = d->B * d->Ho * d->Wo; a.N = d->Cout; a.Kpad = d->Kpad;
  a.H = d->H; a.W = d->W; a.Cin = d->Cin; a.Ho = d->Ho; a.Wo = d->Wo;
  a.KH = d->KH; a.KW = d->KW; a.stride = d->stride; a.pad = d->pad;
  a.in_ps = d->in_pix_stride; a.out_ps = d->out_pix_stride; a.res_ps = d->res_pix_stride;
  a.relu = d->act & HANDS_ACT_MASK;
  a.ksplit = 1; a.partial = nullptr; a.part_ps = 0; a.pre_scale = pre_scale; a.pre_shift = pre_shift;
  a.in2 = in; a.K0 = 1 << 30; a.H2 = a.W2 = a.stride2 = a.in2_ps = 0;
  a.nblk_m = a.nblk_n = 0;
}

int launch_conv(const hands_conv_desc* d, ConvArgs& a, bool pre, bool bf16x3, hipStream_t s) {
  const bool narrow = d->Cout <= 64;
  if (d->Cin == 4) return narrow ? launch<4, 1, 1>(a, s) : launch<2, 2, 1>(a, s);
  if (pre) return launch_fp32<2, true>(d, a, s);
  const bool pointwise = a.K0 < a.Kpad || pointwise_route_ok(d);
  if (bf16x3) {
    if (pointwise) return narrow ? launch<4, 1, 2, 1>(a, s) : launch<2, 2, 2, 1>(a, s);
    return narrow ? launch<4, 1, 0, 1>(a, s) : launch<2, 2, 0, 1>(a, s);
  }
  return pointwise ? launch_fp32<2>(d, a, s) : launch_fp32<0>(d, a, s);
}

int group_class(const hands_conv_desc* d, bool pre) {
  if (!d || !conv_geometry_ok(d) || !pointwise_route_ok(d)) return -1;
  if (d->act & (HANDS_MATH_BF16X3 | HANDS_SUM_BLOCK128 | HANDS_ACC_F64)) return -1;
  return (d->Cout <= 64 ? 1 : 0) | ((d->act & HANDS_SUM_BLOCK64) ? 2 : 0) | (pre ? 4 : 0);
}

template <int WAVES_M, int WAVES_N, bool PRE, int BLK>
int launch_group(GroupArgs& g, hipStream_t stream) {
  constexpr int BM = 64 * WAVES_M, BN = 64 * WAVES_N;
  long long total = 0;
  for (int p = 0; p < g.n; ++p) {
    ConvArgs& a = g.a[p];
    a.nblk_m = (a.M + BM - 1) / BM;
    a.nblk_n = (a.N + BN - 1) / BN;
    g.start[p] = (int)total;
    total += ((long long)a.nblk_m * a.nblk_n + 7) / 8 * 8;
    if (total > 0x7fffffffLL) return HANDS_EINVAL;
  }
  for (int p = g.n; p <= GROUP_MAX; ++p) g.start[p] = (int)total;
  hipLaunchKernelGGL((conv_igemm_group_f32_kernel<WAVES_M, WAVES_N, 2, PRE, BLK>), dim3((unsigned)total), dim3(256), 0, stream, g);
  return (int)hipGetLastError();
}

}

extern "C" int hands_conv2d_group_class(const hands_conv_desc* d, int pre) { return group_class(d, pre != 0); }

extern "C" int hands_conv2d_group_f32(const hands_conv_job* jobs, int n, hands_stream_t stream) {
  if (!jobs || n < 1 || n > GROUP_MAX) return HANDS_EINVAL;
  GroupArgs g{};
  g.n = n;
  int cls = -2;
  for (int p = 0; p < n; ++p) {
    const hands_conv_job& j = jobs[p];
    if (!j.desc || !j.in || !j.w_packed || !j.bias || !j.out || ((j.pre_scale != nullptr) != (j.pre_shift != nullptr))) return HANDS_EINVAL;
    const int c = group_class(j.desc, j.pre_scale != nullptr);
    if (c < 0 || (cls != -2 && c != cls)) return HANDS_EINVAL;
    if (!residual_ok(j.desc, j.residual)) return HANDS_EINVAL;
    cls = c;
    fill_plain_args(j.desc, j.in, j.w_packed, j.bias, j.residual, j.out, j.pre_scale, j.pre_shift, g.a[p]);
  }
  hipStream_t s = (hipStream_t)stream;
  switch (cls) {
    case 0: return launch_group<2, 2, false, 0>(g, s);
    case 1: return launch_group<4, 1, false, 0>(g, s);
    case 2: return launch_group<2, 2, false, 4>(g, s);
    case 3: return launch_group<4, 1, false, 4>(g, s);
    case 4: return launch_group<2, 2, true, 0>(g, s);
    case 5: return launch_group<4, 1, true, 0>(g, s);
    case 6: return launch_group<2, 2, true, 4>(g, s);
    case 7: return launch_group<4, 1, true, 4>(g, s);
  }
  return HANDS_EINVAL;
}

extern "C" int hands_conv2d_splitk_factor(const hands_conv_desc* d) { return d ? splitk_factor(d) : 0; }

extern "C" long long hands_conv2d_workspace_floats(const hands_conv_desc* d, int S) {
  if (!d || !conv_geometry_ok(d)) return -1;
  if (S <= 0) S = splitk_factor(d);
  if (S > d->Kpad / BK) S = d->Kpad / BK;
  if (S <= 1) return 0;
  return (long long)S * d->B * d->Ho * d->Wo * d->Cout * ((d->act & HANDS_ACC_F64) ? 2 : 1);
}

extern "C" int hands_conv2d_nhwc_f32(const hands_conv_desc* d, const float* in, const float* w_packed,
                                     const float* bias, const float* residual, float* out,
                                     hands_stream_t stream) {
  if (!d || !in || !w_packed || !bias || !out) return HANDS_EINVAL;
  if (!conv_geometry_ok(d) || !residual_ok(d, residual)) return HANDS_EINVAL;
  ConvArgs a;
  fill_plain_args(d, in, w_packed, bias, residual, out, nullptr, nullptr, a);
  return launch_conv(d, a, false, (d->act & HANDS_MATH_BF16X3) != 0, (hipStream_t)stream);
}

extern "C" long long hands_conv2d_streamk_workspace_bytes(void) {
  return (long long)SK_MAX_G * SK_SLOT_FLOATS * 4 + (long long)SK_MAX_G * 4;
}

extern "C" int hands_conv2d_streamk_grid(const hands_conv_desc* d) {
  if (!d || !conv_geometry_ok(d) || d->Cin == 4) return 0;
  const bool narrow = d->Cout <= 64;
  const long long M = (long long)d->B * d->Ho * d->Wo;
  const long long ntiles = narrow ? ((M + 255) / 256) * ((d->Cout + 63) / 64) : ((M + 127) / 128) * ((d->Cout + 127) / 128);
  return streamk_grid(ntiles, d->Kpad / BK, device_cus(), 4);
}

extern "C" int hands_conv2d_nhwc_streamk_f32(const hands_conv_desc* d, const float* in, const float* w_packed,
                                             const float* bias, const float* residual, float* out, void* workspace,
                                             long long workspace_bytes, int epoch, hands_stream_t stream) {
  if (!d || !in || !w_packed || !bias || !out) return HANDS_EINVAL;
  if (!conv_geometry_ok(d) || !residual_ok(d, residual)) return HANDS_EINVAL;
  if (d->Cin == 4 || (d->act & (HANDS_MATH_BF16X3 | HANDS_SUM_BLOCK128 | HANDS_SUM_BLOCK64 | HANDS_ACC_F64)))
    return hands_conv2d_nhwc_f32(d, in, w_packed, bias, residual, out, stream);
  ConvArgs a;
  fill_plain_args(d, in, w_packed, bias, residual, out, nullptr, nullptr, a);
  hipStream_t s = (hipStream_t)stream;
  if (pointwise_route_ok(d))
    return (d->Cout <= 64) ? launch_streamk<4, 1, 2>(a, s, workspace, workspace_bytes, epoch)
                           : launch_streamk<2, 2, 2>(a, s, workspace, workspace_bytes, epoch);
  return (d->Cout <= 64) ? launch_streamk<4, 1, 0>(a, s, workspace, workspace_bytes, epoch)
                         : launch_streamk<2, 2, 0>(a, s, workspace, workspace_bytes, epoch);
}

extern "C" int hands_conv1x1_dual_nhwc_f32(const hands_conv_desc* d, const float* in, const float* in2, int Cin2, int H2,
                                           int W2, int stride2, int in2_pix_stride, const float* w_packed,
                                           const float* bias, float* out, hands_stream_t stream) {
  if (!d || !in || !in2 || !w_packed || !bias || !out) return HANDS_EINVAL;
  if (d->B <= 0 || d->KH != 1 || d->KW != 1 || d->stride != 1 || d->pad != 0 || d->H != d->Ho || d->W != d->Wo)
    return HANDS_EINVAL;
  if (d->Cin % 16 || Cin2 <= 0 || Cin2 % 16 || d->Cout % 4 || d->Kpad != d->Cin + Cin2) return HANDS_EINVAL;
  if (d->in_pix_stride < d->Cin || in2_pix_stride < Cin2 || d->out_pix_stride < d->Cout || stride2 < 1) return HANDS_EINVAL;
  if (d->in_pix_stride % 4 || in2_pix_stride % 4 || d->out_pix_stride % 4) return HANDS_EINVAL;
  if ((d->Ho - 1) * stride2 >= H2 || (d->Wo - 1) * stride2 >= W2) return HANDS_EINVAL;
  if ((long long)d->B * d->H * d->W * d->in_pix_stride >= (1LL << 31) ||
      (long long)d->B * H2 * W2 * in2_pix_stride >= (1LL << 31))
    return HANDS_EINVAL;
  {
    const long long imgs = 256 / ((long long)d->Ho * d->Wo) + 2;
    if (imgs * d->H * d->W * d->in_pix_stride * 4 >= (1LL << 31) || imgs * H2 * W2 * in2_pix_stride * 4 >= (1LL << 31) ||
        256LL * d->Kpad * 4 >= (1LL << 31))
      return HANDS_EINVAL;
  }
  if (d->act & HANDS_ACC_F64) return HANDS_EINVAL;
  ConvArgs a;
  fill_plain_args(d, in, w_packed, bias, nullptr, out, nullptr, nullptr, a);
  a.in2 = in2; a.K0 = d->Cin; a.H2 = H2; a.W2 = W2; a.stride2 = stride2; a.in2_ps = in2_pix_stride;
  hands_conv_desc one_chain = *d;
  one_chain.act &= ~(HANDS_SUM_BLOCK128 | HANDS_SUM_BLOCK64);
  return launch_conv(&one_chain, a, false, (d->act & HANDS_MATH_BF16X3) != 0, (hipStream_t)stream);
}

namespace {
int splitk_launch(const hands_conv_desc* d, const float* in, const float* w_packed, const float* bias, const float* residual,
                  float* out, int S, float* workspace, long long workspace_floats,
                  hands_stream_t stream, const float* pre_scale = nullptr, const float* pre_shift = nullptr,
                  int* counters = nullptr, long long n_counters = 0) {
  if (!d) return HANDS_EINVAL;
  const bool pre = pre_scale != nullptr;
  if (pre && (!pre_shift || !pointwise_route_ok(d) || (d->act & HANDS_MATH_BF16X3))) return HANDS_EINVAL;
  const long long M = (long long)d->B * d->Ho * d->Wo;
  const int part_ps = d->Cout;
  if (S > d->Kpad / BK) S = d->Kpad / BK;
  const bool f64 = (d->act & HANDS_ACC_F64) != 0;
  const bool split = S > 1 && workspace && workspace_floats >= (long long)S * M * part_ps * (f64 ? 2 : 1) &&
                     !(f64 && (((uintptr_t)workspace) & 7));
  if (!split && !pre) return hands_conv2d_nhwc_f32(d, in, w_packed, bias, residual, out, stream);
  if (!in || !w_packed || !bias || !out || !conv_geometry_ok(d) || !residual_ok(d, residual) || (split && S > 64)) return HANDS_EINVAL;
  ConvArgs a;
  fill_plain_args(d, in, w_packed, bias, residual, out, pre_scale, pre_shift, a);
  if (split) {
    a.ksplit = S; a.partial = workspace; a.part_ps = part_ps;
    const bool narrow = d->Cout <= 64 && !f64;
    const long long ntiles = narrow ? ((M + 255) / 256) * ((d->Cout + 63) / 64) : ((M + 127) / 128) * ((d->Cout + 127) / 128);
    if (counters && n_counters >= ntiles) { a.counters = counters; a.fin_res = residual; a.fin_act = d->act & HANDS_ACT_MASK; }
  }
  hipStream_t s = (hipStream_t)stream;
  const int rc = launch_conv(d, a, pre, false, s);
  if (rc || !split || a.counters != nullptr) return rc;
  if (f64) {
    hipLaunchKernelGGL(splitk_reduce_f64_kernel, dim3(hands_grid_1d(M * d->Cout, 256)), dim3(256), 0, s,
                       reinterpret_cast<const double*>(workspace), S, (int)M, d->Cout, part_ps, bias, residual, d->res_pix_stride,
                       out, d->out_pix_stride, d->act & HANDS_ACT_MASK);
    return (int)hipGetLastError();
  }
  const long long total = M * (d->Cout / 4);
  hipLaunchKernelGGL(splitk_reduce_kernel, dim3(hands_grid_1d(total, 256)), dim3(256), 0, s, workspace, S, (int)M,
                     d->Cout / 4, part_ps, bias, residual, d->res_pix_stride, out, d->out_pix_stride, d->act & HANDS_ACT_MASK);
  return (int)hipGetLastError();
}
}

extern "C" int hands_conv2d_nhwc_pre_f32(const hands_conv_desc* d, const float* in, const float* pre_scale,
                                         const float* pre_shift, const float* w_packed, const float* bias,
                                         const float* residual, float* out, int S, float* workspace,
                                         long long workspace_floats, hands_stream_t stream) {
  if (!pre_scale || !pre_shift) return HANDS_EINVAL;
  return splitk_launch(d, in, w_packed, bias, residual, out, S, workspace, workspace_floats, stream, pre_scale, pre_shift);
}

extern "C" int hands_conv2d_nhwc_splitk_n_f32(const hands_conv_desc* d, const float* in, const float* w_packed,
                                              const float* bias, const float* residual, float* out, int S,
                                              float* workspace, long long workspace_floats, hands_stream_t stream) {
  return splitk_launch(d, in, w_packed, bias, residual, out, S, workspace, workspace_floats, stream);
}

extern "C" int hands_conv2d_nhwc_splitk_fused_f32(const hands_conv_desc* d, const float* in, const float* w_packed,
                                                  const float* bias, const float* residual, float* out, int S,
                                                  float* workspace, long long workspace_floats, int* counters,
                                                  long long n_counters, hands_stream_t stream) {
  return splitk_launch(d, in, w_packed, bias, residual, out, S, workspace, workspace_floats, stream, nullptr, nullptr, counters,
                       n_counters);
}

extern "C" int hands_conv2d_nhwc_splitk_f32(const hands_conv_desc* d, const float* in, const float* w_packed,
                                            const float* bias, const float* residual, float* out, float* workspace,
                                            long long workspace_floats, hands_stream_t stream) {
  if (!d) return HANDS_EINVAL;
  return hands_conv2d_nhwc_splitk_n_f32(d, in, w_packed, bias, residual, out, splitk_factor(d), workspace,
                                        workspace_floats, stream);
}
```

### hands_amd/engine.py

```python
from __future__ import annotations

import ctypes as C
from typing import NamedTuple

import torch

from ._lib import ConvDesc, ConvJob, check, ptr

MATH_BF16X3 = 0x100
_SUM_BLOCK = {128: 0x200, 64: 0x400}
ACC_F64 = 0x800


class ConvEngine:
    def __init__(self):
        self.use_splitk = True
        self.latency_mode = False
        self.overlap = True
        self.fuse_stem_pool = True
        self.fuse_downsample = True
        self.stream_k = "auto"
        self.math = "fp32"
        self.winograd = True
        self.winograd4 = False
        self.fuse_mano = True
        self.fuse_pre = True
        self.chain_limit = 0
        self.chain_min_k = 0
        self.chain_skip_tokens = False
        self.chain_max_pix = 0
        self.chain_in_kernel = False
        self.acc64 = True
        self.fuse_splitk_reduce = True
        self.group_launches = True
        self.last_acc64 = False
        self.hook = None
        self.last_wino_macs = 0
        self.last_sum_block = 0
        self._splitk_ws = {}
        self._sk_ws = {}
        self._capture_ws = {}
        self._capture_tables = {}
        self._capture_seq = 0

    def clone_settings(self) -> "ConvEngine":
        e = ConvEngine()
        for k in ("use_splitk", "latency_mode", "overlap", "fuse_stem_pool", "fuse_downsample", "winograd", "winograd4", "fuse_mano", "fuse_pre", "stream_k", "math", "chain_limit",
                  "chain_min_k", "chain_max_pix", "chain_skip_tokens", "chain_in_kernel", "acc64", "group_launches", "fuse_splitk_reduce"):
            setattr(e, k, getattr(self, k))
        return e

    def begin_capture(self) -> int:
        self._capture_seq += 1
        self._capture_ws = self._capture_tables[self._capture_seq] = {}
        return self._capture_seq

    def drop_capture(self, token: int):
        t = self._capture_tables.pop(token, None)
        if t is not None and t is self._capture_ws:
            self._capture_ws = {}

    def release_workspaces(self, dev=None):
        for table in (self._splitk_ws, self._sk_ws, self._capture_ws, *self._capture_tables.values()):
            for key in [k for k in table if dev is None or k[0] == dev]:
                del table[key]

    @staticmethod
    def _capturing(L, stream):
        st = L.hands_stream_is_capturing(stream)
        if st < 0:
            raise RuntimeError(f"hands_amd: hipStreamIsCapturing failed: {L.hands_error_string(-st).decode()}")
        return bool(st)

    def _workspace(self, dev, stream, need, capturing):
        key = (dev, stream)
        table = self._capture_ws if capturing else self._splitk_ws
        ws = table.get(key)
        if ws is None or ws.numel() < need:
            if ws is not None and not capturing:
                torch.cuda.synchronize(dev)
            ws = table[key] = torch.empty(max(need, 1 << 22), dtype=torch.float32, device=dev)
        return ws

    def _counters(self, L, dev, stream):
        if self._capturing(L, stream):
            return None
        key = (dev, stream, "ctr")
        c = self._splitk_ws.get(key)
        if c is None:
            c = self._splitk_ws[key] = torch.zeros(16384, dtype=torch.int32, device=dev)
            torch.cuda.current_stream(dev).synchronize()
        return c

    def _desc(self, pc, B, H, W, act, in_ps, out_ps, res_ps, has_res, out_hw=None):
        Ho = (H + 2 * pc.pad - pc.KH) // pc.stride + 1
        Wo = (W + 2 * pc.pad - pc.KW) // pc.stride + 1
        if out_hw is not None:
            if not (0 < out_hw[0] <= Ho and 0 < out_hw[1] <= Wo):
                raise ValueError(f"hands_amd: out_hw {tuple(out_hw)} is not inside the layer's {Ho} x {Wo} output map")
            Ho, Wo = out_hw
        return ConvDesc(B, H, W, pc.Cin, Ho, Wo, pc.Cout, pc.KH, pc.KW, pc.stride, pc.pad, in_ps or pc.Cin, out_ps or pc.Cout,
                        (pc.Cout if res_ps is None else res_ps) if has_res else 0, pc.Kpad,
                        int(act) | (MATH_BF16X3 if self.math == "bf16x3" else 0))

    def _route(self, L, pc, d, stream, kind="conv", has_res=False, pre=False, splitk=False, splitk_n=0, aligned=False):
        fp32 = self.math == "fp32"
        acc64 = bool(self.acc64 and pc.acc64 and fp32 and pc.Cin != 4)
        if acc64:
            d.act |= ACC_F64
        if kind == "dual":
            return _Route("dual", 1, 0, acc64, "conv_igemm_f32_kernel")
        S = 1
        if kind == "conv":
            if self.use_splitk:
                S = splitk_n if splitk_n > 1 else (L.hands_conv2d_splitk_factor(C.byref(d)) if splitk else 1)
            if self.latency_mode and not acc64:
                bm, bn = (256, 64) if pc.Cout <= 64 else (128, 128)
                tiles = -(-(d.B * d.Ho * d.Wo) // bm) * -(-pc.Cout // bn)
                if tiles <= 128:
                    S = max(S, min(256 // tiles, pc.Kpad // 128, 32))
            if not acc64 and self.winograd and not has_res and not pre and S <= 1 and fp32 and aligned:
                if self.winograd4 and pc.wino4 is not None and L.hands_conv3x3_winograd4_supported(C.byref(d)):
                    return _Route("wino4", S, 0, False, "conv_wino4_f32_kernel")
                if pc.wino is not None and L.hands_conv3x3_winograd_supported(C.byref(d)):
                    return _Route("wino", S, 0, False, "conv_wino_f32_kernel")
        limit = self.chain_limit if pc.sum_block < 0 else (pc.sum_block if self.chain_limit else 0)
        sum_block = 0
        if (limit and not acc64 and fp32 and (self.chain_in_kernel or self.use_splitk)
                and pc.Kpad >= max(2 * limit, self.chain_min_k)
                and (not self.chain_max_pix or d.Ho * d.Wo <= self.chain_max_pix)
                and not (self.chain_skip_tokens and d.H * d.W == 1 and d.B >= 4096)):
            sum_block = limit
            if self.chain_in_kernel:
                if limit not in _SUM_BLOCK:
                    raise ValueError(f"hands_amd: chain_in_kernel takes chain_limit 64 or 128, not {limit}")
                d.act |= _SUM_BLOCK[limit]
            else:
                S = max(S, min(pc.Kpad // limit, 32))
        if kind == "group":
            groupable = not acc64 and (self.chain_in_kernel or not limit)
            cls = L.hands_conv2d_group_class(C.byref(d), int(pre)) if groupable else -1
            return _Route("group" if cls >= 0 else "conv", S, sum_block, acc64, "conv_igemm_group_f32_kernel", cls=cls)
        if S > 1:
            capturing = self._capturing(L, stream)
            entry = "pre" if pre else ("splitk_fused" if self.fuse_splitk_reduce and not capturing else "splitk")
            return _Route(entry, S, sum_block, acc64, "conv_igemm_splitk_f32_kernel", capturing)
        if pre:
            return _Route("pre", S, sum_block, acc64, "conv_igemm_f32_kernel")
        if (not sum_block and not acc64 and fp32 and ((not self.overlap) if self.stream_k == "auto" else self.stream_k)
                and L.hands_conv2d_streamk_grid(C.byref(d)) > 0 and not self._capturing(L, stream)):
            return _Route("streamk", S, 0, False, "conv_igemm_sk_f32_kernel")
        return _Route("plain", S, sum_block, acc64, "conv_igemm_f32_kernel")

    def _launch(self, kernel, pc, npix, stream, has_res, fn, *args):
        hook = self.hook
        if hook is not None:
            hook("begin", pc, npix, stream, has_res, kernel)
        check(fn(*args), fn.__name__)
        if hook is not None:
            hook("end", pc, npix, stream, has_res, kernel)

    def conv(self, L, pc, x, B, H, W, out, relu, stream, res=None, in_ps=None, out_ps=None, res_ps=None,
             x_off=0, out_off=0, res_off=0, splitk=False, splitk_n=0, pre=None, out_hw=None):
        d = self._desc(pc, B, H, W, relu, in_ps, out_ps, res_ps, res is not None, out_hw)
        xp, op, wp, bp = ptr(x, x_off), ptr(out, out_off), ptr(pc.w), ptr(pc.bias)
        rp = ptr(res, res_off) if res is not None else None
        r = self._route(L, pc, d, stream, "conv", res is not None, pre is not None, splitk, splitk_n, (xp | op) % 16 == 0)
        self.last_sum_block, self.last_acc64 = r.sum_block, r.acc64
        dp = C.byref(d)
        if r.entry == "wino4":
            if self.hook is not None:
                self.last_wino_macs = L.hands_conv3x3_winograd4_executed_macs(dp)
            fn, args = L.hands_conv3x3_winograd4_f32, (dp, xp, ptr(pc.wino4), bp, op, stream)
        elif r.entry == "wino":
            if self.hook is not None:
                self.last_wino_macs = L.hands_conv3x3_winograd_executed_macs(dp)
            fn, args = L.hands_conv3x3_winograd_f32, (dp, xp, ptr(pc.wino), bp, op, stream)
        elif r.entry == "streamk":
            key = (x.device, stream)
            sk = self._sk_ws.get(key)
            if sk is None:
                nbytes = L.hands_conv2d_streamk_workspace_bytes()
                sk = self._sk_ws[key] = [torch.zeros(nbytes // 4, dtype=torch.int32, device=x.device), 0]
                torch.cuda.current_stream(x.device).synchronize()
            sk[1] = sk[1] % 0x7FFFFFF0 + 1
            fn, args = L.hands_conv2d_nhwc_streamk_f32, (dp, xp, wp, bp, rp, op, ptr(sk[0]), sk[0].numel() * 4, sk[1], stream)
        elif r.entry == "plain":
            fn, args = L.hands_conv2d_nhwc_f32, (dp, xp, wp, bp, rp, op, stream)
        else:
            ws = self._workspace(x.device, stream, L.hands_conv2d_workspace_floats(dp, r.S), r.capturing) if r.S > 1 else None
            wsp, wsn = (ptr(ws), ws.numel()) if ws is not None else (None, 0)
            if r.entry == "pre":
                fn, args = L.hands_conv2d_nhwc_pre_f32, (dp, xp, ptr(pre[0]), ptr(pre[1]), wp, bp, rp, op, r.S, wsp, wsn, stream)
            elif r.entry == "splitk_fused":
                ctr = self._counters(L, x.device, stream)
                fn, args = L.hands_conv2d_nhwc_splitk_fused_f32, (dp, xp, wp, bp, rp, op, r.S, wsp, wsn, ptr(ctr), ctr.numel(), stream)
            else:
                fn, args = L.hands_conv2d_nhwc_splitk_n_f32, (dp, xp, wp, bp, rp, op, r.S, wsp, wsn, stream)
        self._launch(r.kernel, pc, B * d.Ho * d.Wo, stream, res is not None, fn, *args)
        return d.Ho, d.Wo

    def conv_group(self, L, jobs, stream):
        single = lambda j: self.conv(L, j["pc"], j["x"], j["B"], j["H"], j["W"], j["out"], j.get("relu", 0), stream,
                                     **{k: j[k] for k in ("res", "pre", "in_ps", "out_ps", "res_ps", "x_off", "out_off", "res_off") if k in j})
        if len(jobs) < 2 or not self.group_launches or self.latency_mode or self.math != "fp32":
            for j in jobs:
                single(j)
            return
        classes = {}
        for j in jobs:
            pc = j["pc"]
            d = self._desc(pc, j["B"], j["H"], j["W"], j.get("relu", 0), j.get("in_ps"), j.get("out_ps"), j.get("res_ps"),
                           j.get("res") is not None)
            r = self._route(L, pc, d, stream, "group", pre=j.get("pre") is not None)
            j["_d"], j["_npix"], j["_sum_block"] = d, j["B"] * d.Ho * d.Wo, r.sum_block
            classes.setdefault(r.cls, []).append(j)
        for cls, members in classes.items():
            for chunk in ([members[i:i + 8] for i in range(0, len(members), 8)] if cls >= 0 else [[j] for j in members]):
                if len(chunk) == 1:
                    single(chunk[0])
                    continue
                arr = (ConvJob * len(chunk))()
                for k, j in enumerate(chunk):
                    pc, res, pre = j["pc"], j.get("res"), j.get("pre")
                    arr[k] = ConvJob(C.pointer(j["_d"]), ptr(j["x"], j.get("x_off", 0)), ptr(pc.w), ptr(pc.bias),
                                     ptr(res, j.get("res_off", 0)) if res is not None else None, ptr(j["out"], j.get("out_off", 0)),
                                     ptr(pre[0]) if pre is not None else None, ptr(pre[1]) if pre is not None else None)
                self.last_sum_block, self.last_acc64 = chunk[0]["_sum_block"], False
                gp = _GroupPC(chunk) if self.hook is not None else None
                self._launch("conv_igemm_group_f32_kernel", gp, gp.npix if gp else 0, stream,
                             any(j.get("res") is not None for j in chunk), L.hands_conv2d_group_f32, arr, len(chunk), stream)

    def conv_dual(self, L, pc, split, x, x2, B, Ho, Wo, H2, W2, out, stream, act=1, out_off=0):
        K0, K1, stride2 = split
        d = ConvDesc(B, Ho, Wo, K0, Ho, Wo, pc.Cout, 1, 1, 1, 0, K0, pc.Cout, 0, pc.Kpad,
                     int(act) | (MATH_BF16X3 if self.math == "bf16x3" else 0))
        if self._route(L, pc, d, stream, "dual").acc64:
            raise ValueError("hands_amd: conv_dual has no fp64 accumulation (hands_conv1x1_dual_nhwc_f32): a layer marked acc64 "
                             "takes its conv3 and downsample as separate launches")
        self._launch("conv_igemm_f32_kernel", pc, B * Ho * Wo, stream, False, L.hands_conv1x1_dual_nhwc_f32,
                     C.byref(d), ptr(x), ptr(x2), K1, H2, W2, stride2, K1, ptr(pc.w), ptr(pc.bias), ptr(out, out_off), stream)

    def stem_pool(self, L, pc, x4, x_off, out, B, H, W, act, stream):
        Hc, Wc = (H - 1) // 2 + 1, (W - 1) // 2 + 1
        self._launch("stem_pool_kernel", pc, B * Hc * Wc, stream, False, L.hands_stem_conv_maxpool_nhwc_f32,
                     ptr(x4, x_off), ptr(pc.w), ptr(pc.bias), ptr(out), B, H, W, int(act), stream)
        return Hc, Wc

    def stem_pool_nchw(self, L, pc, x, x_off, out, out_off, B, H, W, act, stream):
        Hc, Wc = (H - 1) // 2 + 1, (W - 1) // 2 + 1
        self._launch("stem_pool_planar_kernel", pc, B * Hc * Wc, stream, False, L.hands_stem_conv_maxpool_nchw_f32,
                     ptr(x, x_off), ptr(pc.w), ptr(pc.bias), ptr(out, out_off), B, H, W, int(act), stream)
        return Hc, Wc


class _Route(NamedTuple):
    entry: str
    S: int
    sum_block: int
    acc64: bool
    kernel: str
    capturing: bool = False
    cls: int = -1


class _GroupPC:

    def __init__(self, chunk):
        self.npix = sum(j["_npix"] for j in chunk)
        self.group_macs = sum(j["pc"].macs_per_pixel * j["_npix"] for j in chunk)
        self.group_bytes = sum(4.0 * (j["_npix"] * j["pc"].Cout * (2 if j.get("res") is not None else 1)
                                      + j["_npix"] * j["pc"].stride ** 2 * j["pc"].Cin + j["pc"].w.numel()) for j in chunk)
        pc0 = chunk[0]["pc"]
        self.Cin, self.Cout, self.KH, self.stride, self.w, self.Kpad = pc0.Cin, pc0.Cout, 1, pc0.stride, pc0.w, pc0.Kpad
        self.macs_per_pixel = self.group_macs / max(self.npix, 1)
        self.members = len(chunk)


DEFAULT_ENGINE = ConvEngine()


def linear_chain(engine, L, layers, x, rows, stream, buf, names, out=None, in_ps=None, x_off=0, out_ps=None, out_off=0):
    last = len(layers) - 1
    for i, (pc, act, splitk) in enumerate(layers):
        y = out if (i == last and out is not None) else buf(names[i], rows * pc.Cout)
        kw = {"in_ps": in_ps, "x_off": x_off} if i == 0 else {}
        if i == last:
            kw.update(out_ps=out_ps, out_off=out_off)
        engine.conv(L, pc, x, rows, 1, 1, y, act, stream, splitk=splitk, **kw)
        x = y
    return x


class EngineSwitches:

    @property
    def latency_mode(self):
        return self.engine.latency_mode

    @latency_mode.setter
    def latency_mode(self, v):
        self.engine.latency_mode = bool(v)

    @property
    def overlap_trunks(self):
        return self.engine.overlap

    @overlap_trunks.setter
    def overlap_trunks(self, v):
        self.engine.overlap = bool(v)

    @property
    def conv_hook(self):
        return self.engine.hook

    @conv_hook.setter
    def conv_hook(self, fn):
        self.engine.hook = fn
```

### hands_amd/hands_light.py

```python
from __future__ import annotations

import torch
import torch.nn as nn

from . import _lib
from ._lib import check, ptr
from .engine import DEFAULT_ENGINE, ConvEngine, EngineSwitches, linear_chain
from .grasp_head import GRASP_SPLITK, pack_grasp_head, run_grasp_head
from .hmr_head import TF_PASS, HandHMR, depth_head, iter_head, pack_hmr_head, tf_head
from .mano_head import MANOHead, ManoHeadsPlan, pack_mano_pair, run_mano_heads
from .packing import HMR_VEC, pack_conv, pack_linear
from .resnet50 import ResNet50Params, pack_resnet50_trunk, resnet50_trunk
from .streams import SideJobs
from .vit_b16 import ViTB16Params, pack_vit_b16_trunk, vit_b16_trunk, vit_conv_params
from .xdict import _Args, args_getter, stream_xdict, xdict

BACKBONES = ("resnet50", "vit_b_16")

LATENT_ENC = ("center+corner_latent", "sinusoidal_cc")
IMAGE_ENC = {"center": 1, "corner": 2, "center+corner": 3}

DEFAULT_ARGS = _Args(backbone="resnet50", pos_enc="center+corner_latent", n_freq_pos_enc=4,
                     use_glb_feat=True, separate_hands=False, tf_decoder=False, use_grasp_loss=True,
                     use_glb_feat_w_grasp=True, no_crops=False, use_depth_loss=False,
                     regress_center_corner=False, use_render_seg_loss=False, img_res=224,
                     focal_length=1000.0)


class _PackedHolder:

    def __init__(self):
        self.packed, self.dev, self.version = None, None, 0

    def invalidate(self):
        self.packed = None
        self.version += 1


class HandsLight(EngineSwitches, nn.Module):
    def __init__(self, backbone="resnet50", focal_length=1000.0, img_res=224, args=None,
                 mano_assets=None, tf_decoder=False):
        super().__init__()
        self.engine = ConvEngine()
        self.winograd4_stages = (1, 2, 3, 4)
        self.engine.winograd4 = True
        self.trunk_chunks = (1, 2)
        self.async_tail = True
        self._calls = 0
        args = args if args is not None else DEFAULT_ARGS
        get = args_getter(args)
        self.args = args
        if backbone not in BACKBONES:
            raise NotImplementedError(f"hands_amd.HandsLight: backbone={backbone!r} is not built (built: {BACKBONES})")
        self.backbone_name = backbone
        pos_enc = get("pos_enc")
        self.pos_enc = pos_enc
        self.enc_mode = ("latent" if pos_enc in LATENT_ENC else "image" if pos_enc in IMAGE_ENC else
                         "dense" if pos_enc == "dense" else "dense_latent" if pos_enc in ("dense_latent", "cam_conv") else
                         "none" if pos_enc in (None, "pcl", "perspective_correction") else None)
        self.rot_fix = {"pcl": 1, "perspective_correction": 2}.get(pos_enc, 0)
        self.use_depth_loss = bool(get("use_depth_loss", False))
        self.img_res_ds = int(get("img_res_ds", img_res) or img_res)
        self.no_crops = bool(get("no_crops", False))
        self.use_grasp_loss = bool(get("use_grasp_loss", False))
        self.use_glb_feat_w_grasp = bool(get("use_glb_feat_w_grasp", False))
        self.separate_hands = bool(get("separate_hands", False))
        self.regress_center_corner = bool(get("regress_center_corner", False))
        self.use_glb_feat = bool(get("use_glb_feat", False))
        self.tf_decoder = bool(tf_decoder)
        self.tf_pass = TF_PASS
        tf = self.tf_decoder
        unsupported = {
            f"pos_enc={pos_enc!r}": self.enc_mode is None,
            "args.tf_decoder (the transformer head is built: ask for it with HandsLight(..., tf_decoder=True))":
                bool(get("tf_decoder", False)) and not tf,
            "tf_decoder with sinusoidal_cc": tf and pos_enc == "sinusoidal_cc",
            "tf_decoder with cam_conv": tf and pos_enc == "cam_conv",
            "tf_decoder with no_crops": tf and self.no_crops,
            "tf_decoder with regress_center_corner": tf and self.regress_center_corner,
            f"tf_decoder with pos_enc={pos_enc!r} (checked: 'center+corner_latent', 'dense_latent', None)":
                tf and pos_enc not in ("center+corner_latent", "dense_latent", None, "sinusoidal_cc", "cam_conv"),
            "use_depth_loss with no_crops": self.use_depth_loss and self.no_crops,
            "use_render_seg_loss (call hands_amd.MANORenderer on the output instead)": bool(get("use_render_seg_loss", False)),
            "use_glb_feat=False with no_crops": not self.use_glb_feat and self.no_crops,
            "use_glb_feat=False with use_glb_feat_w_grasp": (not self.use_glb_feat and self.use_grasp_loss and self.use_glb_feat_w_grasp),
            "regress_center_corner with no_crops": self.regress_center_corner and self.no_crops,
            "separate_hands with a widened conv_proj on vit_b_16": (backbone == "vit_b_16" and self.separate_hands
                                                                    and self.enc_mode in ("image", "dense")),
        }
        bad = [k for k, v in unsupported.items() if v]
        if bad:
            raise NotImplementedError(f"hands_amd.HandsLight: unsupported config switches {bad}")
        self.n_freq = int(get("n_freq_pos_enc", 4))
        feat_dim = 2048
        self.feat_dim = feat_dim
        vit = backbone == "vit_b_16"
        Trunk = ViTB16Params if vit else ResNet50Params
        self.backbone = Trunk()
        if vit:
            self.vit_conv = vit_conv_params()
            self.trunk_chunks = (1, 1)
        self.enc_channels = ({1: 4, 2: 16, 3: 20}[IMAGE_ENC[pos_enc]] * self.n_freq if self.enc_mode == "image" else
                             4 * self.n_freq if self.enc_mode == "dense" else 0)
        if self.separate_hands:
            self.hand_backbone_r = Trunk(3 + self.enc_channels)
            self.hand_backbone_l = Trunk(3 + self.enc_channels)
            if vit:
                self.hand_backbone_r_vit_conv = vit_conv_params()
                self.hand_backbone_l_vit_conv = vit_conv_params()
        else:
            self.hand_backbone = Trunk(3 + self.enc_channels)
            if vit:
                self.hand_backbone_vit_conv = vit_conv_params()
        self.latent_channels = (5 * 4 * self.n_freq if self.enc_mode == "latent" else 4 * self.n_freq if pos_enc == "dense_latent" else
                                6 if pos_enc == "cam_conv" else 0)
        fc_dim = feat_dim + self.latent_channels
        self.head_r = HandHMR(feat_dim, True, 3, tf_in=fc_dim if tf else None)
        self.head_l = HandHMR(feat_dim, False, 3, tf_in=fc_dim if tf else None)
        self.feature_conv = nn.Sequential(
            nn.Conv2d(fc_dim, 1024, 1, bias=False), nn.ReLU(inplace=True),
            nn.Conv2d(1024, 512, 3, bias=False), nn.ReLU(inplace=True),
            nn.Conv2d(512, 256, 3, bias=False), nn.ReLU(inplace=True),
            nn.Flatten(), nn.Linear(256 * 3 * 3, feat_dim), nn.ReLU(inplace=True))
        assets = mano_assets or (None, None)
        self.mano_r = MANOHead(True, focal_length, img_res, assets[0])
        self.mano_l = MANOHead(False, focal_length, img_res, assets[1])
        if self.use_grasp_loss:
            gdim = 10 + 144 + (feat_dim if self.use_glb_feat_w_grasp else 0)
            self.grasp_classifier = nn.Sequential(
                nn.Linear(gdim, 1024), nn.ReLU(inplace=True), nn.Linear(1024, 512),
                nn.ReLU(inplace=True), nn.Linear(512, 128), nn.ReLU(inplace=True), nn.Linear(128, 9))
        if self.use_depth_loss:
            cv = lambda i, o: nn.Conv2d(i, o, 3, 1, 1)
            up = lambda k: nn.Upsample(scale_factor=k, mode="bilinear", align_corners=True)
            self.depth_mlp = nn.Sequential(
                cv(fc_dim + 2, 256), nn.ReLU(True), cv(256, 256), nn.ReLU(True), up(4), cv(256, 128), nn.ReLU(True),
                cv(128, 128), nn.ReLU(True), up(4), cv(128, 64), nn.ReLU(True), cv(64, 32), nn.ReLU(True), up(2),
                cv(32, 16), nn.ReLU(True), cv(16, 1))
        if self.regress_center_corner:
            mk = lambda n: nn.Sequential(nn.Linear(feat_dim, 512), nn.ReLU(inplace=True), nn.Linear(512, 128),
                                         nn.ReLU(inplace=True), nn.Linear(128, n))
            self.corner_head = mk(8)
            self.center_head = mk(2)
        self.mode = "train"
        self.img_res = img_res
        self.focal_length = focal_length
        self._holder = _PackedHolder()
        self._ws = {}
        self.register_load_state_dict_post_hook(lambda m, k: m.invalidate_packed())

    @property
    def _packed(self):
        return self._holder.packed

    def invalidate_packed(self):
        self._holder.invalidate()
        if any(isinstance(v, torch.Tensor) and v.is_cuda for v in self._ws.values()):
            torch.cuda.synchronize()
        self._ws = {}

    def _apply(self, fn, *a, **k):
        self.invalidate_packed()
        return super()._apply(fn, *a, **k)

    @torch.no_grad()
    def _pack(self, dev):
        cpu = lambda t: t.detach().cpu()
        F = self.feat_dim
        P = {"head_r": pack_hmr_head(self.head_r, dev, F, self.tf_decoder), "head_l": pack_hmr_head(self.head_l, dev, F, self.tf_decoder)}
        if self.backbone_name == "vit_b_16":
            pack_trunk = lambda name: pack_vit_b16_trunk(getattr(self, name), getattr(self, "vit_conv" if name == "backbone" else name + "_vit_conv"), dev)
        else:
            pack_trunk = lambda name: pack_resnet50_trunk(getattr(self, name), dev, self.winograd4_stages)
        if self.use_glb_feat:
            P["backbone"] = pack_trunk("backbone")
        if not self.no_crops:
            if self.separate_hands:
                P["hand_backbone_r"] = pack_trunk("hand_backbone_r")
                P["hand_backbone_l"] = pack_trunk("hand_backbone_l")
            else:
                P["hand_backbone"] = pack_trunk("hand_backbone")
        if self.regress_center_corner:
            for nm, head in (("cc_center", self.center_head), ("cc_corner", self.corner_head)):
                P[nm] = [pack_linear(cpu(head[0].weight), cpu(head[0].bias), dev), pack_linear(cpu(head[2].weight), cpu(head[2].bias), dev),
                         pack_linear(cpu(head[4].weight), cpu(head[4].bias), dev, n_total=8)]
        fc = self.feature_conv
        if not self.tf_decoder:
            P["fc0"] = pack_conv(cpu(fc[0].weight), None, 1, 0, dev,
                                 cin_pad_to=self._cat_ld() if self.enc_mode == "dense_latent" else None)
        if self.use_depth_loss:
            dm = self.depth_mlp
            P["depth"] = [pack_conv(cpu(dm[i].weight), cpu(dm[i].bias), 1, 1, dev,
                                    cin_pad_to=self._depth_ld() if i == 0 else None) for i in (0, 2, 5, 7, 10, 12, 15, 17)]
            lin = torch.linspace(-1, 1, 7)
            xg, yg = torch.meshgrid(lin, lin, indexing="ij")
            P["depth_grid"] = torch.stack([xg, yg], dim=-1).reshape(49, 2).contiguous().to(dev)
        if not self.tf_decoder:
            P["fc2"] = pack_conv(cpu(fc[2].weight), None, 1, 0, dev)
            P["fc4"] = pack_conv(cpu(fc[4].weight), None, 1, 0, dev)
            col = [(k % 9) * 256 + (k // 9) for k in range(256 * 9)]
            P["fc7"] = pack_linear(cpu(fc[7].weight), cpu(fc[7].bias), dev, col_index=col)
        if self.use_grasp_loss:
            P["grasp"] = pack_grasp_head(self.grasp_classifier[0::2], dev, F if self.use_glb_feat_w_grasp else 0)
        P["mano_r"], P["mano_l"] = pack_mano_pair(self.mano_r, self.mano_l, dev)
        return P

    def _cat_ld(self):
        n = self.feat_dim + self.latent_channels
        return (n + 15) // 16 * 16 if self.enc_mode == "dense_latent" else n

    def _depth_ld(self):
        return (self.feat_dim + self.latent_channels + 2 + 15) // 16 * 16

    def replica(self):
        self.packed(next(self.parameters()).device)
        import copy
        r = copy.copy(self)
        r._ws = {}
        r.engine = self.engine.clone_settings()
        return r

    def packed(self, dev):
        h = self._holder
        if h.packed is None or h.dev != dev:
            h.packed, h.dev = self._pack(dev), dev
        return h.packed

    def _side_stream(self, dev, name="side_stream"):
        st = self._ws.get(name)
        if st is None or st.device != dev:
            st = torch.cuda.Stream(device=dev)
            self._ws[name] = st
        return st

    def _buf(self, name, numel, dev):
        t = self._ws.get(name)
        if t is None or t.numel() < numel or t.device != dev:
            if t is not None and t.is_cuda:
                torch.cuda.synchronize(t.device)
            t = torch.empty(numel, dtype=torch.float32, device=dev)
            self._ws[name] = t
        return t

    _conv = staticmethod(lambda *a, **kw: DEFAULT_ENGINE.conv(*a, **kw))
    _conv_dual = staticmethod(lambda *a, **kw: DEFAULT_ENGINE.conv_dual(*a, **kw))

    def _trunk(self, L, P, segs, B, res_in, stream, tag, cap_B, out=None, out_off=0):
        dev = segs[0][0].device
        trunk = vit_b16_trunk if "vit" in P else resnet50_trunk
        return trunk(self.engine, lambda name, numel: self._buf(name, numel, dev), L, P, segs, B, res_in, stream, tag, cap_B, out, out_off)

    @torch.no_grad()
    def forward(self, inputs, meta_info):
        L = _lib.lib()
        img = inputs["img"]
        dev = img.device
        if dev.type != "cuda":
            raise RuntimeError("hands_amd.HandsLight runs on a HIP device only (no CPU fallback); "
                               "move the module and its inputs to 'cuda'")
        f32 = lambda t: t.to(device=dev, dtype=torch.float32).contiguous()
        img, r_img, l_img = f32(img), f32(inputs["r_img"]), f32(inputs["l_img"])
        K = f32(meta_info["intrinsics"])
        assert K.shape[1:] == (3, 3)
        bz, c, res, res_w = img.shape
        assert c == 3 and res == res_w and r_img.shape == img.shape and l_img.shape == img.shape
        B2 = 2 * bz
        F = self.feat_dim
        P = self.packed(dev)
        stream = torch.cuda.current_stream(dev).cuda_stream
        buf = lambda n, numel: self._buf(n, numel, dev)

        main = torch.cuda.current_stream(dev)
        async_tail = bool(self.async_tail and self.engine.overlap and not torch.cuda.is_current_stream_capturing())
        par = self._calls & 1 if async_tail else 0
        self._calls += 1
        if not torch.cuda.is_current_stream_capturing():
            for q in ((par,) if async_tail else (0, 1)):
                prev_tail = self._ws.get(f"tail_done{q}")
                if prev_tail is not None:
                    main.wait_event(prev_tail)
        featg = buf(f"feat_g{par}", bz * 49 * F) if self.use_glb_feat else None
        feath = buf(f"feat_h{par}", B2 * 49 * F) if not self.no_crops else None
        gch, hch = self.trunk_chunks if self.engine.overlap else (1, 1)
        if self.no_crops:
            gch, hch = (2 if self.engine.overlap else 1), 0
        if self.separate_hands and hch:
            hch = 2
        gch, hch = (max(1, min(gch, bz)) if self.use_glb_feat else 0), min(hch, B2)
        need_cc = (not self.no_crops) and self.enc_mode in ("latent", "image")
        center = (torch.cat([f32(inputs["r_center_angle"]), f32(inputs["l_center_angle"])], 0)
                  if (need_cc or self.rot_fix == 2) else None)
        corner = torch.cat([f32(inputs["r_corner_angle"]), f32(inputs["l_corner_angle"])], 0) if need_cc else None
        rot_in = torch.cat([f32(inputs["r_rot"]), f32(inputs["l_rot"])], 0) if self.rot_fix == 1 else None
        wide = None
        dense_enc = None
        if self.enc_mode in ("dense", "dense_latent") and not self.no_crops:
            ang = [f32(inputs["r_dense_angle"]), f32(inputs["l_dense_angle"])]
            msk = [f32(inputs["r_dense_mask"]), f32(inputs["l_dense_mask"])]
            Ca, Hs, Ws = ang[0].shape[1:]
            L_enc = 0 if self.pos_enc == "cam_conv" else self.n_freq
            assert (2 * L_enc * Ca if L_enc else Ca) == (self.enc_channels if self.enc_mode == "dense" else self.latent_channels)
            if self.enc_mode == "dense":
                assert res == self.img_res_ds, "pos_enc='dense': the crops must have the size args.img_res_ds"
                Cp = P["hand_backbone_r" if self.separate_hands else "hand_backbone"]["stem_wide"].Cin
                wide = buf("wide_in", B2 * res * res * Cp)
                for side, im in enumerate((r_img, l_img)):
                    check(L.hands_dense_posenc_f32(ptr(ang[side]), ptr(msk[side]), ptr(im), ptr(wide, side * bz * res * res * Cp),
                                                   bz, Ca, Hs, Ws, L_enc, self.img_res_ds, res, res, Cp, 3, stream), "dense_posenc")
            else:
                Ce = self.latent_channels
                dense_enc = buf(f"dense_enc{par}", B2 * 49 * Ce)
                for side in (0, 1):
                    check(L.hands_dense_posenc_f32(ptr(ang[side]), ptr(msk[side]), None, ptr(dense_enc, side * bz * 49 * Ce),
                                                   bz, Ca, Hs, Ws, L_enc, self.img_res_ds, 7, 7, Ce, 0, stream), "dense_posenc")
        if self.enc_mode == "image" and not self.no_crops:
            Cp = P["hand_backbone_r" if self.separate_hands else "hand_backbone"]["stem_wide"].Cin
            wide = buf("wide_in", B2 * res * res * Cp)
            mode = IMAGE_ENC[self.pos_enc]
            for side, im in enumerate((r_img, l_img)):
                check(L.hands_image_posenc_nhwc_f32(ptr(im), ptr(center, side * bz * 2), ptr(corner, side * bz * 8),
                                                    ptr(wide, side * bz * res * res * Cp), bz, res, res, self.n_freq, mode, Cp,
                                                    stream), "image_posenc")
        jobs = []
        for c in range(gch):
            lo, hi = c * bz // gch, (c + 1) * bz // gch
            jobs.append((P["backbone"], [(img, lo, hi - lo)], lo, hi - lo, featg))
        for c in range(hch):
            lo, hi = c * B2 // hch, (c + 1) * B2 // hch
            segs = []
            if wide is not None:
                segs.append((wide, lo, hi - lo))
            else:
                if lo < bz:
                    segs.append((r_img, lo, min(hi, bz) - lo))
                if hi > bz:
                    segs.append((l_img, max(lo, bz) - bz, hi - max(lo, bz)))
            jobs.append((P[("hand_backbone_r", "hand_backbone_l")[c]] if self.separate_hands else P["hand_backbone"], segs, lo, hi - lo, feath))
        side_jobs = SideJobs(main)
        fh = fw = 7
        for ji, (Pt, segs, lo, n, ob) in enumerate(jobs):
            st = main if (ji == len(jobs) - 1 or not self.engine.overlap) else self._side_stream(dev, f"side{ji}")
            side_jobs.begin(st)
            _, fh, fw = self._trunk(L, Pt, segs, n, res, st.cuda_stream, f"j{ji}", n, out=ob, out_off=lo * 49 * F)
            side_jobs.end(st)
        side_jobs.join()
        assert fh * fw == 49
        HW = fh * fw
        flipped = meta_info["is_flipped"].to(device=dev, dtype=torch.int64).contiguous()
        if async_tail:
            K, flipped = K.clone(), flipped.clone()
            tail = self._side_stream(dev, "tail")
            evt = torch.cuda.Event()
            evt.record(main)
            tail.wait_event(evt)
            for t in (center, corner, K, flipped, rot_in):
                if t is not None:
                    t.record_stream(tail)
        else:
            tail = main
        with torch.cuda.stream(tail):
            output = self._forward_tail(L, P, dev, tail, bz, fh, fw, featg, feath, center, corner, K, flipped, dense_enc, rot_in)
        if not async_tail:
            return output
        ready = torch.cuda.Event()
        ready.record(tail)
        self._ws[f"tail_done{par}"] = ready
        return stream_xdict(output, ready, dev)

    def _forward_tail(self, L, P, dev, main, bz, fh, fw, featg, feath, center, corner, K, flipped, dense_enc=None, rot_in=None):
        B2, F, HW = 2 * bz, self.feat_dim, fh * fw
        stream = main.cuda_stream
        buf = lambda n, numel: self._buf(n, numel, dev)
        feat_vec = buf("feat_vec", bz * F)
        if self.use_grasp_loss and self.use_glb_feat_w_grasp:
            check(L.hands_sumpool_nhwc_f32(ptr(featg), ptr(feat_vec), bz, HW, F, F, stream), "sumpool")
        ld, vo = (HMR_VEC, 0) if self.tf_decoder else (F + HMR_VEC, F)
        state = buf("state", B2 * ld)
        cat_ld = self._cat_ld() if self.enc_mode in ("latent", "dense_latent") else F
        if self.no_crops:
            for side in (0, 1):
                check(L.hands_avgpool_nhwc_f32(ptr(featg), ptr(state, side * bz * ld), bz, HW, F, ld, stream), "avgpool")
        else:
            if self.enc_mode == "latent":
                Cc = F + 20 * self.n_freq
                cat = buf("cat", B2 * HW * Cc)
                check(L.hands_kpe_concat_f32(ptr(feath), ptr(featg) if self.use_glb_feat else None, ptr(center), ptr(corner),
                                             ptr(cat), B2, bz, HW, F, self.n_freq, stream), "kpe_concat")
            elif self.enc_mode == "dense_latent":
                Cc, Ce = self._cat_ld(), self.latent_channels
                cat = buf("cat", B2 * HW * Cc)
                check(L.hands_concat_nhwc_f32(ptr(feath), F, F, ptr(featg) if self.use_glb_feat else None, F, ptr(dense_enc),
                                              HW * Ce, Ce, ptr(cat), Cc, B2, bz, HW, stream), "concat")
            else:
                cat = feath
            depth = (depth_head(self.engine, buf, L, P, dev, stream, cat, B2, bz, fh, fw, F + self.latent_channels, cat_ld, self._depth_ld())
                     if self.use_depth_loss else None)
            if not self.tf_decoder:
                f1 = buf("fc1", B2 * HW * 1024)
                self.engine.conv(L, P["fc0"], cat, B2, fh, fw, f1, True, stream)
                f2 = buf("fc2", B2 * (fh - 2) * (fw - 2) * 512)
                h2, w2 = self.engine.conv(L, P["fc2"], f1, B2, fh, fw, f2, True, stream)
                f3 = buf("fc3", B2 * (h2 - 2) * (w2 - 2) * 256)
                h3, w3 = self.engine.conv(L, P["fc4"], f2, B2, h2, w2, f3, True, stream, splitk_n=8)
                assert h3 * w3 * 256 == P["fc7"].Cin
                self.engine.conv(L, P["fc7"], f3, B2, 1, 1, state, True, stream, out_ps=ld, splitk=True)

        caminit4 = buf("caminit4", B2 * 4)
        heads = SideJobs(main)
        for side, hp in ((0, P["head_r"]), (1, P["head_l"])):
            hs = main if (side == 1 or not self.engine.overlap) else self._side_stream(dev, "side_head")
            heads.begin(hs)
            sh = hs.cuda_stream
            if self.tf_decoder:
                tf_head(self.engine, buf, L, hp, sh, side, bz, HW, cat, state, caminit4, F, cat_ld, self.tf_pass)
            else:
                iter_head(self.engine, buf, L, hp, sh, side, bz, state, caminit4, F)
            heads.end(hs)
        heads.join()
        rotmat = buf("rotmat", B2 * 144)
        check(L.hands_rot6d_to_matrix_f32(ptr(state, vo), ld, ptr(rotmat), B2, stream), "rot6d")
        if self.rot_fix == 1:
            check(L.hands_rot_leftmul_f32(ptr(rotmat), ptr(rot_in), B2, stream), "rot_leftmul")
        st = state[: B2 * ld].view(B2, ld)
        shape = st[:, vo + 96:vo + 106].contiguous()
        cam = st[:, vo + 108:vo + 111].contiguous()
        caminit = caminit4[: B2 * 4].view(B2, 4)[:, :3].contiguous()

        rot_m = torch.empty(B2, 16, 3, 3, device=dev)
        shape_m = torch.empty(B2, 10, device=dev)
        cam_m = torch.empty(B2, 3, device=dev)
        caminit_m = torch.empty(B2, 3, device=dev)
        check(L.hands_flip_swap_f32(ptr(flipped), ptr(rotmat), ptr(shape), ptr(cam), ptr(caminit),
                                    ptr(rot_m), ptr(shape_m), ptr(cam_m), ptr(caminit_m), bz, stream),
              "flip_swap")

        if self.rot_fix == 2:
            check(L.hands_perspective_correction_f32(ptr(rot_m), ptr(rotmat), ptr(center), ptr(flipped), bz, stream), "persp")

        output = run_mano_heads(L, P["mano_r"], P["mano_l"], rot_m, shape_m, cam_m, caminit_m, K,
                                float(self.img_res), bz, stream, buf, self.engine)

        extra = None
        if self.regress_center_corner:
            extra = xdict()
            for nm, key in (("cc_center", "center"), ("cc_corner", "corner")):
                l0, l1, l2 = P[nm]
                o = torch.empty(B2, 8, device=dev)
                linear_chain(self.engine, L, [(l0, True, True), (l1, True, True), (l2, False, False)], state, B2, stream, buf,
                             ("cc_h1", "cc_h2"), out=o, in_ps=ld)
                n = 2 if key == "center" else 8
                extra[key + ".r"] = o[:bz, :n].contiguous()
                extra[key + ".l"] = o[bz:, :n].contiguous()
        if self.use_depth_loss and not self.no_crops:
            dx = xdict()
            dx["depth.r"], dx["depth.l"] = depth
            if extra is None:
                extra = dx
            else:
                dx.merge(extra)
                extra = dx
        if not self.use_grasp_loss:
            if extra is not None:
                output.merge(extra)
            return output
        output.merge(run_grasp_head(self.engine, L, P["grasp"], GRASP_SPLITK["hands_light"], state, rotmat, bz, stream, buf, shape_ld=ld,
                                    shape_off=vo + 96, feat=feat_vec, feat_dim=F if self.use_glb_feat_w_grasp else 0))
        if extra is not None:
            output.merge(extra)
        return output
```

### include/hands_hip.h

```cpp
#ifndef HANDS_HIP_H
#define HANDS_HIP_H

#include <stddef.h>
#include <stdint.h>

#ifdef __cplusplus
extern "C" {
#endif

#define HANDS_EINVAL 10001
#define HANDS_ABI_VERSION 5

typedef void* hands_stream_t;

int hands_abi_version(void);
const char* hands_error_string(int code);
int hands_stream_is_capturing(hands_stream_t stream);
const char* hands_csrc_sha16(void);

long long hands_ceiling_mfma_f32(float* out, long long out_floats, int iters, int random_operands, hands_stream_t stream);
int hands_ceiling_hbm_read_f32(const float* in, long long n_floats, float* out, hands_stream_t stream);

typedef struct hands_conv_desc {
  int32_t B, H, W, Cin;
  int32_t Ho, Wo, Cout;
  int32_t KH, KW, stride, pad;
  int32_t in_pix_stride;
  int32_t out_pix_stride;
  int32_t res_pix_stride;
  int32_t Kpad;
  int32_t act;
} hands_conv_desc;

#define HANDS_ACT_NONE 0
#define HANDS_ACT_RELU 1
#define HANDS_ACT_GELU 2
#define HANDS_ACT_LEAKY_RELU 3
#define HANDS_ACT_MASK 0xff
#define HANDS_MATH_BF16X3 0x100
#define HANDS_SUM_BLOCK128 0x200
#define HANDS_SUM_BLOCK64 0x400
#define HANDS_ACC_F64 0x800

int hands_conv2d_nhwc_f32(const hands_conv_desc* d, const float* in, const float* w_packed,
                          const float* bias, const float* residual, float* out,
                          hands_stream_t stream);

typedef struct hands_conv_job {
  const hands_conv_desc* desc;
  const float* in;
  const float* w_packed;
  const float* bias;
  const float* residual;
  float* out;
  const float* pre_scale;
  const float* pre_shift;
} hands_conv_job;
int hands_conv2d_group_class(const hands_conv_desc* d, int pre);
int hands_conv2d_group_f32(const hands_conv_job* jobs, int n, hands_stream_t stream);

int hands_conv3x3_winograd_supported(const hands_conv_desc* d);
long long hands_conv3x3_winograd_executed_macs(const hands_conv_desc* d);
int hands_conv3x3_winograd_f32(const hands_conv_desc* d, const float* in, const float* u_packed, const float* bias,
                               float* out, hands_stream_t stream);

int hands_conv3x3_winograd4_supported(const hands_conv_desc* d);
long long hands_conv3x3_winograd4_executed_macs(const hands_conv_desc* d);
int hands_conv3x3_winograd4_f32(const hands_conv_desc* d, const float* in, const float* u_packed, const float* bias,
                                float* out, hands_stream_t stream);

int hands_conv2d_splitk_factor(const hands_conv_desc* d);
int hands_conv2d_nhwc_splitk_f32(const hands_conv_desc* d, const float* in, const float* w_packed,
                                 const float* bias, const float* residual, float* out, float* workspace,
                                 long long workspace_floats, hands_stream_t stream);
int hands_conv2d_nhwc_splitk_n_f32(const hands_conv_desc* d, const float* in, const float* w_packed,
                                   const float* bias, const float* residual, float* out, int S,
                                   float* workspace, long long workspace_floats, hands_stream_t stream);
int hands_conv2d_nhwc_splitk_fused_f32(const hands_conv_desc* d, const float* in, const float* w_packed,
                                       const float* bias, const float* residual, float* out, int S,
                                       float* workspace, long long workspace_floats, int* counters,
                                       long long n_counters, hands_stream_t stream);

int hands_conv2d_nhwc_pre_f32(const hands_conv_desc* desc, const float* in, const float* pre_scale, const float* pre_shift,
                              const float* w_packed, const float* bias, const float* residual, float* out, int S,
                              float* workspace, long long workspace_floats, hands_stream_t stream);

long long hands_conv2d_streamk_workspace_bytes(void);
int hands_conv2d_streamk_grid(const hands_conv_desc* d);
int hands_conv2d_nhwc_streamk_f32(const hands_conv_desc* d, const float* in, const float* w_packed,
                                  const float* bias, const float* residual, float* out, void* workspace,
                                  long long workspace_bytes, int epoch, hands_stream_t stream);

int hands_conv1x1_dual_nhwc_f32(const hands_conv_desc* d, const float* in, const float* in2, int Cin2, int H2,
                                int W2, int stride2, int in2_pix_stride, const float* w_packed,
                                const float* bias, float* out, hands_stream_t stream);

int hands_stem_conv_maxpool_nhwc_f32(const float* x4, const float* w_packed, const float* bias, float* out,
                                     int B, int H, int W, int act, hands_stream_t stream);

int hands_stem_conv_maxpool_nchw_f32(const float* x_nchw, const float* w_planar, const float* bias, float* out,
                                     int B, int H, int W, int act, hands_stream_t stream);

int hands_nchw3_to_nhwc4_f32(const float* in, float* out, int B, int H, int W, hands_stream_t stream);

int hands_maxpool3x3s2_nhwc_f32(const float* in, float* out, int B, int H, int W, int C,
                                hands_stream_t stream);

int hands_sumpool_nhwc_f32(const float* feat, float* out, int B, int HW, int C, int out_stride,
                           hands_stream_t stream);

int hands_avgpool_nhwc_f32(const float* feat, float* out, int B, int HW, int C, int out_stride,
                           hands_stream_t stream);

int hands_image_posenc_nhwc_f32(const float* img_nchw, const float* center_angle, const float* corner_angle, float* out,
                                int B, int H, int W, int n_freq, int mode, int Cpad, hands_stream_t stream);


int hands_dense_posenc_f32(const float* angle, const float* mask, const float* img_nchw, float* out, int B, int Ca, int Hs, int Ws,
                           int n_freq, int R, int Ho, int Wo, int ld, int c_off, hands_stream_t stream);

int hands_concat_nhwc_f32(const float* a, int lda, int Ca, const float* add, int ld_add, const float* extra,
                          long long extra_batch_stride, int Cb, float* out, int ld, int B, int Bg, int HW, hands_stream_t stream);

int hands_upsample_bilinear_ac_f32(const float* x, float* out, int B, int h, int w, int H, int W, int C, hands_stream_t stream);

int hands_rot_leftmul_f32(float* rotmat, const float* rot, int B, hands_stream_t stream);

int hands_perspective_correction_f32(float* rot_swapped, float* rotmat, const float* center_angle, const int64_t* is_flipped,
                                     int Bg, hands_stream_t stream);

int hands_kpe_concat_f32(const float* crop, const float* glb, const float* center_angle,
                         const float* corner_angle, float* out, int B2, int Bg, int HW, int C,
                         int n_freq, hands_stream_t stream);

int hands_hmr_init_f32(float* state, const float* cam_init, int B, int ld, int F,
                       hands_stream_t stream);

int hands_rot6d_to_matrix_f32(const float* pose6d, int ld6, float* rotmat, int B,
                              hands_stream_t stream);

int hands_flip_swap_f32(const int64_t* is_flipped, const float* rotmat, const float* shape,
                        const float* cam, const float* cam_init, float* rotmat_out,
                        float* shape_out, float* cam_out, float* cam_init_out, int Bg,
                        hands_stream_t stream);

int hands_matrix_to_axis_angle_f32(const float* rotmat, float* axis_angle, long long n, hands_stream_t stream);
int hands_axis_angle_to_matrix_f32(const float* axis_angle, float* rotmat, long long n, hands_stream_t stream);

int hands_grasp_input_f32(const float* shape, int ld_shape, const float* rotmat,
                          const float* feat_vec, float* out, int B2, int Bg, int F, int ld_out,
                          hands_stream_t stream);

typedef struct hands_mano_consts {
  const float* pose_mean;
  const float* J_template;
  const float* J_shapedirs;
  const float* lbs_weights;
  const int32_t* tip_ids;
} hands_mano_consts;

int hands_mano_pose_f32(const hands_mano_consts* c, const float* rotmat, const float* betas,
                        int ld_betas, float* blend_in, int ld_blend, float* A, float* joints16,
                        int B, hands_stream_t stream);

typedef struct hands_mano_out {
  float* vertices;
  float* joints3d;
  float* v3d_cam;
  float* j3d_cam;
  float* j2d_norm;
  float* cam_t;
} hands_mano_out;

int hands_mano_skin_f32(const hands_mano_consts* c, const float* v_posed, int ld_vp,
                        const float* A, const float* joints16, const float* cam_wp,
                        const float* K, float img_res, float min_s, const hands_mano_out* out,
                        int B, hands_stream_t stream);

typedef struct hands_mano_side {
  hands_mano_consts consts;
  const float* blend_w;
  const float* blend_bias;
  const float* rot;
  const float* betas;
  const float* cam_wp;
  hands_mano_out out;
} hands_mano_side;

int hands_mano_heads_f32(const hands_mano_side* sides, int n_sides, const float* K, int ld_betas,
                         float img_res, float min_s, int B, int axis_angle_input, hands_stream_t stream);
int hands_mano_heads_vsplit(int B, int n_sides);


int hands_resize_crop_nchw3_to_nhwc4_f32(const float* in, float* out, int B, int Hin, int Win, int S,
                                         int col0, int Wc, hands_stream_t stream);

int hands_layernorm_f32(const float* x, const float* gamma, const float* beta, float* out,
                        const float* addvec, int rows_per_vec, int M, int C, float eps,
                        hands_stream_t stream);

int hands_add_pos_f32(float* x, const float* pos, const float* vec, int B, int T, int C,
                      hands_stream_t stream);

int hands_kpe_encode_f32(const float* center_angle, const float* corner_angle, float* out, int B, int ld,
                         int n_freq, hands_stream_t stream);

int hands_attention_f32(const float* qkv, float* out, int B, int T, int heads, int head_dim, float scale,
                        hands_stream_t stream);


int hands_vit_tokens_f32(const float* patch, const float* class_token, const float* pos, float* x, int B, int T, int C,
                         hands_stream_t stream);

int hands_vit_tail_f32(const float* x, const float* gamma, const float* beta, float* out, int B, int grid, int C, float eps,
                       hands_stream_t stream);


int hands_wide_attention_f32(const float* q, long long q_batch_stride, int ldq, const float* k, long long k_batch_stride, int ldk,
                             const float* v, long long v_batch_stride, int ldv, float* out, long long out_batch_stride, int ldo,
                             int B, int Tq, int Tk, int D, float scale, hands_stream_t stream);

int hands_vector_tokens_f32(const float* vec, int ldvec, int split, int gap, const float* w, const float* bias, float* out, int B,
                            int T, int C, hands_stream_t stream);

int hands_token_mean_f32(const float* x, float* out, int B, int N, int C, hands_stream_t stream);

int hands_cross_attention_1q_f32(const float* q, const float* kv, float* out, int B, int T, int heads,
                                 int head_dim, float scale, hands_stream_t stream);

int hands_rot6d_to_matrix_cols_f32(const float* pose6d, int ld6, float* rotmat, int B,
                                   hands_stream_t stream);


int hands_upsample_bilinear_add_f32(const float* x, const float* y, float* out, int B, int h, int w,
                                    int H, int W, int C, hands_stream_t stream);

int hands_pool2x2_nhwc_f32(const float* in, float* out, int B, int H, int W, int C, int mode,
                           hands_stream_t stream);

int hands_channel_pool_f32(const float* x, float* out, long long npix, int C, hands_stream_t stream);

int hands_gate_apply_f32(const float* x, const float* logit, int logit_stride, float* primary,
                         float* secondary, long long npix, int C, hands_stream_t stream);

int hands_add_embed2_f32(const float* query, const float* key, const float* q_emb, const float* k_emb,
                         const float* kpe, float* out_q, float* out_k, int B, int N, int C,
                         hands_stream_t stream);

int hands_add_rowvec_f32(const float* x, const float* vec, float* out, int B, int N, int C,
                         hands_stream_t stream);

int hands_token_sum_f32(const float* x, float* out, int B, int N, int C, hands_stream_t stream);

int hands_bn_leaky_f32(const float* x, const float* scale, const float* shift, float* out,
                       long long npix, int C, hands_stream_t stream);

int hands_upsample_nearest2x_add_f32(const float* low, const float* up1, float* out, int B, int h,
                                     int w, int C, hands_stream_t stream);

int hands_spatial_softmax_f32(const float* latents, int ld_in, const float* betas, float* heatmaps,
                              int ld_out, int B, int N, int J, hands_stream_t stream);

int hands_flash_attention_f32(const float* q, const float* k, const float* v, const float* q2,
                              const float* k2sum, const float* resid, float* out, int B, int N,
                              int heads, int head_dim, float scale, hands_stream_t stream);

typedef struct hands_eval_in {
  const float *pred_j3d_r, *pred_j3d_l, *gt_j3d_r, *gt_j3d_l;
  const float *pred_j2d_r, *pred_j2d_l, *gt_j2d_r, *gt_j2d_l;
  const float *is_valid, *right_valid, *left_valid, *joints_valid_r, *joints_valid_l;
} hands_eval_in;

typedef struct hands_eval_out {
  float *mpjpe_ra_h, *mpjpe_pa_ra_r, *mpjpe_pa_ra_l, *mpjpe_pa_ra_h, *mrrpe_rl;
  float *pix_err_r, *pix_err_l;
} hands_eval_out;

int hands_eval_metrics_f32(const hands_eval_in* in, const hands_eval_out* out, int B,
                           hands_stream_t stream);

typedef struct hands_eval_masked_out {
  float *rao_r, *rao_l, *rao_h, *abs_r, *abs_l, *abs_h, *pa_ra_r, *pa_ra_l, *pa_ra_h;
} hands_eval_masked_out;

int hands_eval_metrics_masked_f32(const hands_eval_in* in, const float* joints3d_valid_r, const float* joints3d_valid_l,
                                  const hands_eval_masked_out* out, int B, hands_stream_t stream);

#define HANDS_MESH_MAX_V 1024
#define HANDS_MESH_NQ 10
typedef struct hands_mesh_eval_in {
  const float *pred_v3d_r, *pred_v3d_l, *gt_v3d_r, *gt_v3d_l;
  const float *pred_j3d_r, *pred_j3d_l, *gt_j3d_r, *gt_j3d_l;
  const float *is_valid, *right_valid, *left_valid;
} hands_mesh_eval_in;

typedef struct hands_mesh_eval_out {
  float *mpvpe_ra_r, *mpvpe_ra_l, *mpvpe_ra_h, *f5_ra_r, *f5_ra_l, *f5_ra_h, *f15_ra_r, *f15_ra_l, *f15_ra_h;
  float *auc_ra_v_r, *auc_ra_v_l, *auc_ra_v_h, *auc_ra_j_r, *auc_ra_j_l, *auc_ra_j_h;
  float *mpvpe_pa_r, *mpvpe_pa_l, *mpvpe_pa_h, *f5_pa_r, *f5_pa_l, *f5_pa_h, *f15_pa_r, *f15_pa_l, *f15_pa_h;
  float *auc_pa_v_r, *auc_pa_v_l, *auc_pa_v_h, *auc_pa_j_r, *auc_pa_j_l, *auc_pa_j_h;
} hands_mesh_eval_out;

int hands_eval_mesh_metrics_f32(const hands_mesh_eval_in* in, const hands_mesh_eval_out* out, int B, int V,
                                hands_stream_t stream);

#define HANDS_SURF_MAX_F 4096
#define HANDS_SURF_CHUNK 512
#define HANDS_SURF_NQ 4
int hands_mesh_closest_f32(const float* points, const float* verts, const int32_t* faces, const float* valid, float* dist,
                           int32_t* face_idx, float* closest, int B, int P, int V, int F, hands_stream_t stream);
#define HANDS_SIGNED_CHUNK 256
int hands_mesh_signed_f32(const float* points, const float* verts, const int32_t* faces, const float* valid, float* sdf,
                          float* winding, int32_t* face_idx, int B, int P, int V, int F, hands_stream_t stream);

typedef struct hands_surf_eval_out {
  float *p2s_ra_r, *p2s_ra_l, *p2s_ra_h, *p2s_pa_r, *p2s_pa_l, *p2s_pa_h;
  float *chamfer_ra_r, *chamfer_ra_l, *chamfer_ra_h, *chamfer_pa_r, *chamfer_pa_l, *chamfer_pa_h;
} hands_surf_eval_out;

int hands_eval_surface_metrics_f32(const hands_mesh_eval_in* in, const int32_t* faces_r, const int32_t* faces_l, int F_r,
                                   int F_l, const hands_surf_eval_out* out, int B, int V, hands_stream_t stream);

#define HANDS_ACCEL_NQ 3
int hands_accel_error_f32(const float* gt, const float* pred, const float* valid, const int32_t* seq_id, float* out, int T,
                          int N, int D, float fps, hands_stream_t stream);

typedef struct hands_accel_eval_out {
  float *acc_r, *acc_l, *acc_h, *acc_j_r, *acc_j_l, *acc_j_h, *acc_abs_r, *acc_abs_l, *acc_abs_h;
} hands_accel_eval_out;

int hands_eval_accel_metrics_f32(const hands_mesh_eval_in* in, const int32_t* seq_id, const hands_accel_eval_out* out, int T,
                                 int V, float fps, hands_stream_t stream);

#define HANDS_SMOOTH_SHAPE_FILTER 0
#define HANDS_SMOOTH_SHAPE_MEAN 1
#define HANDS_SMOOTH_SHAPE_NONE 2

typedef struct hands_smooth_side {
  const float *pose, *beta, *cam, *valid;
  float *pose_out, *beta_out, *cam_out;
  void* state;
} hands_smooth_side;

typedef struct hands_smooth_cfg {
  double min_cutoff[3], beta[3], d_cutoff[3];
  int shape_mode;
} hands_smooth_cfg;

long long hands_smooth_state_bytes(void);
int hands_smooth_mano_f32(const hands_smooth_side* sides, int nsides, const long long* seq_id, int T, int S, float fps,
                          const hands_smooth_cfg* cfg, hands_stream_t stream);

typedef struct hands_mano_fit_consts {
  const float *pose_mean, *J_template, *J_shapedirs;
  const float *tip_v_template, *tip_shapedirs, *tip_lbs_weights, *tip_posedirs;
} hands_mano_fit_consts;

typedef struct hands_mano_fit_side {
  hands_mano_fit_consts consts;
  const float *joints, *weights, *valid, *init_pose, *init_beta, *init_transl;
  float *pose, *beta, *transl, *rmse;
  int32_t* steps;
} hands_mano_fit_side;

typedef struct hands_fit_cfg {
  int iters;
  double lambda_beta, lambda_pose, mu0;
} hands_fit_cfg;

int hands_mano_fit_f32(const hands_mano_fit_side* sides, int n_sides, const hands_fit_cfg* cfg, int B, hands_stream_t stream);

typedef struct hands_mano_fit2d_side {
  hands_mano_fit_consts consts;
  const float *kp2d, *weights, *valid, *init_pose, *init_beta, *init_transl;
  float *pose, *beta, *transl, *rmse;
  int32_t *steps, *start;
  float *j3d, *j2d;
} hands_mano_fit2d_side;

typedef struct hands_fit2d_cfg {
  int iters_rigid, iters;
  double lambda_beta, lambda_pose, mu0, robust_sigma, z_min;
  int fit_shape, prior_to_init;
} hands_fit2d_cfg;

int hands_mano_fit2d_f32(const hands_mano_fit2d_side* sides, int n_sides, const float* K, const hands_fit2d_cfg* cfg, int B,
                         hands_stream_t stream);

typedef struct hands_mano_fit_verts_consts {
  const float *pose_mean, *J_template, *J_shapedirs;
  const float *v_template, *shapedirs, *lbs_weights;
  const float* posedirs_vm;
} hands_mano_fit_verts_consts;

typedef struct hands_mano_fit_verts_side {
  hands_mano_fit_verts_consts consts;
  const float *verts, *weights, *valid, *init_pose, *init_beta, *init_transl;
  float *pose, *beta, *transl, *rmse;
  int32_t* steps;
  float* j3d;
} hands_mano_fit_verts_side;

int hands_mano_fit_verts_f32(const hands_mano_fit_verts_side* sides, int n_sides, const hands_fit_cfg* cfg, int B,
                             hands_stream_t stream);

#define HANDS_LOSS_NKEYS 21
#define HANDS_LOSS_N_MANDATORY 31
typedef struct hands_loss_in {
  const float *pred_pose_r, *pred_pose_l, *pred_beta_r, *pred_beta_l, *pred_j3d_r, *pred_j3d_l, *pred_j2d_r, *pred_j2d_l;
  const float *pred_cam_wp_r, *pred_cam_wp_l, *pred_cam_wp_init_r, *pred_cam_wp_init_l;
  const float *gt_pose_r, *gt_pose_l, *gt_beta_r, *gt_beta_l, *gt_j3d_r, *gt_j3d_l, *gt_j2d_r, *gt_j2d_l;
  const float *gt_cam_wp_r, *gt_cam_wp_l;
  const float *right_valid, *left_valid, *joints_valid_r, *joints_valid_l;
  const float *is_cam_loss, *is_j2d_loss, *is_j3d_loss, *is_pose_loss, *is_beta_loss;
  const float *pred_grasp_r, *pred_grasp_l;
  const long long *gt_grasp_r, *gt_grasp_l;
  const float *grasp_valid_r, *grasp_valid_l, *is_grasp_loss;
  const float *pred_mask_r, *pred_mask_l, *gt_mask_r, *gt_mask_l, *render_valid_r, *render_valid_l, *is_mask_loss;
  const float *pred_depth_r, *pred_depth_l, *gt_depth_r, *gt_depth_l, *is_depth_loss;
  const float *pred_center_r, *pred_center_l, *gt_center_r, *gt_center_l;
  const float *pred_corner_r, *pred_corner_l, *gt_corner_r, *gt_corner_l;
} hands_loss_in;

long long hands_loss_workspace_bytes(int B, int S_mask, int S_depth);
int hands_loss_light_f32(const hands_loss_in* in, int B, int S_mask, int S_depth, void* workspace,
                         float* out_unweighted21, float* out_weighted21, float* out_total, hands_stream_t stream);

int hands_mano_pose_aa_f32(const hands_mano_consts* c, const float* axis_angle, const float* betas,
                           int ld_betas, float* blend_in, int ld_blend, float* A, float* joints16,
                           int B, hands_stream_t stream);
int hands_gt_targets_f32(const float* joints, const float* verts, const float* j3d_full, const float* K,
                         float img_res, float* v3d_cam, float* cam_t, float* cam_t_wp, int B, int NV,
                         hands_stream_t stream);
int hands_unnormalize_kp2d_f32(const float* x, float* out, long long n, float img_res,
                               hands_stream_t stream);

int hands_frontend_dense_maps_f32(const int32_t* bbox, const float* K, float* angle, float* mask, int B, int img_res, int nch,
                                  hands_stream_t stream);

int hands_frontend_boxes_f32(const float* j2d_r, const float* j2d_l, int ld, const float* K, int B,
                             int img_res, int out_res, double bbox_scale,
                             int32_t* bbox_r, int32_t* bbox_l, int32_t* bbox_og_r, int32_t* bbox_og_l,
                             float* trans_r, float* trans_l, float* center_r, float* center_l,
                             float* corner_r, float* corner_l, hands_stream_t stream);
int hands_warp_affine_cubic_norm_f32(const float* src, const float* trans, float* out, int B, int H, int W,
                                     int Ho, int Wo, const float* mean3, const float* std3,
                                     hands_stream_t stream);

int hands_render_silhouette_f32(const float* verts, int ld_verts, int n_verts, const int32_t* faces, int n_faces, const float* K, int B, int S, float sigma, float blur_radius, int faces_per_pixel, float* mask, int32_t* face_idx, float* zbuf, hands_stream_t stream);

#define HANDS_SHADE_MAX_MESHES 4
#define HANDS_SHADE_TILE_W 32
#define HANDS_SHADE_TILE_H 8
#define HANDS_SHADE_LIST_CAP 384
typedef struct hands_shade_mesh {
  const float* workspace;
  const int32_t* faces;
  const float* valid;
  int32_t n_verts, n_faces;
  int32_t face_offset;
  float color[3];
  float metallic, roughness;
} hands_shade_mesh;
typedef struct hands_shade_scene {
  hands_shade_mesh mesh[HANDS_SHADE_MAX_MESHES];
  int32_t n_meshes;
} hands_shade_scene;
long long hands_mesh_workspace_floats(int B, int n_verts);
int hands_mesh_prepare_f32(const float* verts, int ld_verts, int n_verts, const int32_t* faces, int n_faces, const int32_t* csr_off, const int32_t* csr_face, const float* K, const float* T, int B, int S, float* workspace, hands_stream_t stream);
int hands_render_shaded_f32(const hands_shade_scene* scene, const float* image, int B, int S, float* rgb, unsigned char* rgb8, float* depth, int32_t* face_id, hands_stream_t stream);

typedef struct hands_packed_dims {
  int32_t Cin;
  int32_t Cout;
  int32_t Cout_pad;
  int32_t Kpad;
} hands_packed_dims;

int hands_pack_conv_dims(int Cout, int Cin, int KH, int KW, int cin_pad_to, hands_packed_dims* dims);
int hands_fold_bn_f32(int Cout, long long per_out, const float* w, const float* gamma, const float* beta,
                      const float* mean, const float* var, double eps, double* w_folded, double* bias_folded);
int hands_pack_conv_f64(int Cout, int Cin, int KH, int KW, int cin_pad_to, const double* w_oihw,
                        const double* bias, float* w_packed, float* bias_packed);
int hands_pack_linear_f64(int N, int K, const double* w, const double* bias, const int32_t* col_index,
                          int k_total, const int32_t* row_index, int n_total, float* w_packed,
                          float* bias_packed);
int hands_pack_conv1x1_dual_f64(int Cout, int K0, int K1, const double* w0, const double* b0,
                                const double* w1, const double* b1, float* w_packed, float* bias_packed);
int hands_pack_mano_f32(const float* v_template, const float* shapedirs, const float* posedirs,
                        const float* J_regressor, const float* hands_mean, float* pose_mean,
                        float* J_template, float* J_shapedirs, float* blend_w_packed,
                        float* blend_bias_packed);
long long hands_conv2d_workspace_floats(const hands_conv_desc* d, int S);
long long hands_pack_conv3x3_winograd_floats(int Cout, int Cin);
int hands_pack_conv3x3_winograd_f64(int Cout, int Cin, const double* w_oihw, float* u_packed);
long long hands_pack_conv3x3_winograd4_floats(int Cout, int Cin);
int hands_pack_conv3x3_winograd4_f64(int Cout, int Cin, const double* w_oihw, float* u_packed);

#ifdef __cplusplus
}
#endif
#endif
```

Measured before the change: 12160 hands/s.

## Add half-height wave tile conv kernel for small-tile-count pointwise layers

Adds a conv_tile variant in which each wave computes 32 pixels by 64 channels instead of 64 by 64. It comes with its own epilogue, C entry points and engine routing. Pointwise and dual 1x1 layers with few plain tiles take this path, which is meant to launch more blocks and fill more CUs on late, small-M stages. The trade is lower per-wave reuse of weight fragments, plus more template code and kernel variants. It is enabled by default for hands_light and disabled for the ViT configuration.

```diff
diff --git a/hands_amd/_lib.py b/hands_amd/_lib.py
--- a/hands_amd/_lib.py
+++ b/hands_amd/_lib.py
@@ -181,6 +181,9 @@
     "hands_conv2d_streamk_grid": [C.POINTER(ConvDesc)],
     "hands_conv2d_nhwc_streamk_f32": [C.POINTER(ConvDesc), _P, _P, _P, _P, _P, _P, C.c_longlong, _I, _P],
     "hands_conv1x1_dual_nhwc_f32": [C.POINTER(ConvDesc), _P, _P, _I, _I, _I, _I, _I, _P, _P, _P, _P],
+    "hands_conv2d_ht_supported": [C.POINTER(ConvDesc)],
+    "hands_conv2d_nhwc_ht_f32": [C.POINTER(ConvDesc), _P, _P, _P, _P, _P, _P],
+    "hands_conv1x1_dual_nhwc_ht_f32": [C.POINTER(ConvDesc), _P, _P, _I, _I, _I, _I, _I, _P, _P, _P, _P],
     "hands_conv2d_nhwc_splitk_n_f32": [C.POINTER(ConvDesc), _P, _P, _P, _P, _P, _I, _P, C.c_longlong, _P],
     "hands_conv2d_nhwc_pre_f32": [C.POINTER(ConvDesc), _P, _P, _P, _P, _P, _P, _P, _I, _P, C.c_longlong, _P],
     "hands_stem_conv_maxpool_nhwc_f32": [_P, _P, _P, _P, _I, _I, _I, _I, _P],
diff --git a/hands_amd/csrc/conv_igemm.hip b/hands_amd/csrc/conv_igemm.hip
--- a/hands_amd/csrc/conv_igemm.hip
+++ b/hands_amd/csrc/conv_igemm.hip
@@ -133,6 +133,48 @@
   }
 }
 
+constexpr int EROW_H = 36;
+constexpr int EPI_FLOATS_H = 4 * 32 * EROW_H;
+template <int ACT, bool RES>
+__device__ __forceinline__ void epilogue_full_ht(const f32x16 (&acc)[2][1], float* sE, int lane, const float* bias_p,
+                                                 const char* res_u, int res_ps, char* out_u, int out_ps) {
+  float* wr = sE + (lane & 31) * EROW_H + (lane >> 5) * 4;
+  const float* rd = sE + (lane >> 3) * EROW_H + (lane & 7) * 4;
+  const uint32_t o_off = (uint32_t)((lane >> 3) * out_ps + (lane & 7) * 4) * 4u;
+  const uint32_t r_off = (uint32_t)((lane >> 3) * res_ps + (lane & 7) * 4) * 4u;
+#pragma unroll
+  for (int i = 0; i < 2; ++i) {
+    const float4 bv4 = *reinterpret_cast<const float4*>(bias_p + i * 32);
+    const f32x2 b01 = {bv4.x, bv4.y}, b23 = {bv4.z, bv4.w};
+#pragma unroll
+    for (int q = 0; q < 4; ++q)
+      *reinterpret_cast<float4*>(wr + q * 8) =
+          make_float4(acc[i][0][q * 4 + 0], acc[i][0][q * 4 + 1], acc[i][0][q * 4 + 2], acc[i][0][q * 4 + 3]);
+    float4 rv[RES ? 4 : 1];
+    if constexpr (RES) {
+#pragma unroll
+      for (int r = 0; r < 4; ++r)
+        rv[r] = *reinterpret_cast<const float4*>(res_u + (size_t)(8 * r) * (size_t)res_ps * 4 + i * 128 + r_off);
+    }
+#pragma unroll
+    for (int r = 0; r < 4; ++r) {
+      const float4 t = *reinterpret_cast<const float4*>(rd + 8 * r * EROW_H);
+      f32x2 v01 = {t.x, t.y}, v23 = {t.z, t.w};
+      v01 = v01 + b01;
+      v23 = v23 + b23;
+      if constexpr (RES) {
+        const f32x2 r01 = {rv[r].x, rv[r].y}, r23 = {rv[r].z, rv[r].w};
+        v01 = v01 + r01;
+        v23 = v23 + r23;
+      }
+      float4 v = make_float4(v01.x, v01.y, v23.x, v23.y);
+      if constexpr (ACT != HANDS_ACT_NONE) v = apply_act(v, ACT);
+      *reinterpret_cast<float4*>(out_u + (size_t)(8 * r) * (size_t)out_ps * 4 + i * 128 + o_off) = v;
+      if (r & 1) __builtin_amdgcn_sched_barrier(0);
+    }
+  }
+}
+
 template <int BM, int BN, bool F64>
 __device__ __forceinline__ void splitk_fused_tail(const ConvArgs& a, float* lds, int tile, int m0, int n0, int wave_u) {
   const int tid = wave_u * 64 + (int)__builtin_amdgcn_mbcnt_hi(~0u, __builtin_amdgcn_mbcnt_lo(~0u, 0u));
@@ -200,18 +242,20 @@
   } else { mt = tile / a.nblk_n; nt = tile - mt * a.nblk_n; }
 }
 
-template <int WAVES_M, int WAVES_N, int MODE, int PREC = 0, bool PRE = false, int BLK = 0>
+template <int WAVES_M, int WAVES_N, int MODE, int PREC = 0, bool PRE = false, int BLK = 0, int NJ = 2>
 __device__ __forceinline__ void conv_tile(const ConvArgs& a, float* lds, int tile, int split, int kt0, int kt1,
                                           const float* acc_in, float* acc_out) {
   constexpr int ROW = PREC == 1 ? LDS_ROW_B3 : LDS_ROW;
   constexpr bool F64 = PREC == 2;
   constexpr bool STEM = MODE == 1;
   constexpr bool DUAL = MODE == 2;
-  constexpr int BM = 64 * WAVES_M;
+  constexpr int BM = 32 * NJ * WAVES_M;
   constexpr int BN = 64 * WAVES_N;
   constexpr int A_ROWS = BM / 64;
   constexpr int W_ROWS = BN / 64;
   static_assert(WAVES_M * WAVES_N == 4, "4 waves per block");
+  static_assert(NJ == 2 || (NJ == 1 && MODE == 2 && PREC == 0 && !PRE && BLK == 0 && BM % 64 == 0),
+                "the half-height wave tile exists for exact-fp32 pointwise launches only");
 
   float* sX = lds;
   float* sW = lds + 2 * BM * ROW;
@@ -389,23 +433,23 @@
 #pragma unroll
       for (int j = 0; j < 4; ++j) accd[i][j] = f64x4{0.0, 0.0, 0.0, 0.0};
   }
-  f32x16 acc[2][2];
+  f32x16 acc[2][NJ];
   if (acc_in != nullptr) {
-    const float4* src = reinterpret_cast<const float4*>(acc_in) + (wave * 16) * 64 + lane;
+    const float4* src = reinterpret_cast<const float4*>(acc_in) + (wave * 8 * NJ) * 64 + lane;
 #pragma unroll
     for (int i = 0; i < 2; ++i)
 #pragma unroll
-      for (int j = 0; j < 2; ++j)
+      for (int j = 0; j < NJ; ++j)
 #pragma unroll
         for (int q = 0; q < 4; ++q) {
-          const float4 v = src[((i * 2 + j) * 4 + q) * 64];
+          const float4 v = src[((i * NJ + j) * 4 + q) * 64];
           acc[i][j][q * 4 + 0] = v.x; acc[i][j][q * 4 + 1] = v.y; acc[i][j][q * 4 + 2] = v.z; acc[i][j][q * 4 + 3] = v.w;
         }
   } else {
 #pragma unroll
     for (int i = 0; i < 2; ++i)
 #pragma unroll
-      for (int j = 0; j < 2; ++j)
+      for (int j = 0; j < NJ; ++j)
 #pragma unroll
         for (int r = 0; r < 16; ++r) acc[i][j][r] = 0.f;
   }
@@ -435,9 +479,9 @@
                    : F64     ? (lane & 15) * ROW + (((lane >> 4) ^ ((lane >> 2) & 3)) * 4)
                              : (lane & 31) * ROW + (((lane >> 5) ^ ((lane >> 2) & 3)) * 4);
   const float* fw = sW + (wn * 64) * ROW + frag;
-  const float* fx = sX + (wm * 64) * ROW + frag;
+  const float* fx = sX + (wm * 32 * NJ) * ROW + frag;
   const float* fw1 = sW + (wn * 64) * ROW + (frag ^ 8);
-  const float* fx1 = sX + (wm * 64) * ROW + (frag ^ 8);
+  const float* fx1 = sX + (wm * 32 * NJ) * ROW + (frag ^ 8);
 
 #define COMPUTE_STEP(BUF)                                                                           \
   do {                                                                                              \
@@ -460,17 +504,18 @@
         }                                                                                           \
       }                                                                                             \
     } else if constexpr (PREC == 0) {                                                               \
-      float4 wf[2][2], xf[2][2];                                            \
+      float4 wf[2][2], xf[NJ][2];                                           \
       _Pragma("unroll") for (int kk = 0; kk < 2; ++kk) {                                            \
         _Pragma("unroll") for (int i = 0; i < 2; ++i) {                                             \
           wf[i][kk] = *reinterpret_cast<const float4*>((kk ? fw1 : fw) + (BUF) * BN * ROW + i * 32 * ROW); \
-          xf[i][kk] = *reinterpret_cast<const float4*>((kk ? fx1 : fx) + (BUF) * BM * ROW + i * 32 * ROW); \
+          if (i < NJ)                                                                               \
+            xf[i % NJ][kk] = *reinterpret_cast<const float4*>((kk ? fx1 : fx) + (BUF) * BM * ROW + i * 32 * ROW); \
         }                                                                                           \
       }                                                                                             \
       _Pragma("unroll") for (int kk = 0; kk < 2; ++kk) {                                            \
         _Pragma("unroll") for (int t = 0; t < 4; ++t) {                                             \
           _Pragma("unroll") for (int i = 0; i < 2; ++i) {                                           \
-            _Pragma("unroll") for (int j = 0; j < 2; ++j) {                                         \
+            _Pragma("unroll") for (int j = 0; j < NJ; ++j) {                                        \
               acc[i][j] = __builtin_amdgcn_mfma_f32_32x32x2f32(f4elem(wf[i][kk], t), f4elem(xf[j][kk], t), \
                                                                acc[i][j], 0, 0, 0);                  \
             }                                                                                       \
@@ -543,117 +588,170 @@
 
   __syncthreads();
   if (acc_out != nullptr) {
-    float4* dst = reinterpret_cast<float4*>(acc_out) + (wave * 16) * 64 + lane;
+    float4* dst = reinterpret_cast<float4*>(acc_out) + (wave * 8 * NJ) * 64 + lane;
 #pragma unroll
     for (int i = 0; i < 2; ++i)
 #pragma unroll
-      for (int j = 0; j < 2; ++j)
+      for (int j = 0; j < NJ; ++j)
 #pragma unroll
         for (int q = 0; q < 4; ++q)
-          dst[((i * 2 + j) * 4 + q) * 64] =
+          dst[((i * NJ + j) * 4 + q) * 64] =
               make_float4(acc[i][j][q * 4 + 0], acc[i][j][q * 4 + 1], acc[i][j][q * 4 + 2], acc[i][j][q * 4 + 3]);
     return;
   }
-  float* sE = lds + wave * (32 * EROW);
-  const int half = lane >> 5;
-  const int c4 = lane & 15;
-  const int n_lane = n0 + wn * 64 + c4 * 4;
-  const bool n_ok = n_lane < a.N;
-  const bool part = a.ksplit > 1;
+  if constexpr (NJ == 1) {
+    static_assert(WAVES_N == 1, "the half-height tile is 4 waves x 32 pixels, 64 channels wide");
+    float* sH = lds + wave * (32 * EROW_H);
+    if (m0 + BM <= a.M && n0 + BN <= a.N) {
+      const int wave_u = __builtin_amdgcn_readfirstlane(wave);
+      const int mw = m0 + wave_u * 32;
+      char* ou = reinterpret_cast<char*>(a.out) + ((size_t)mw * a.out_ps + n0) * 4;
+      const char* ru = reinterpret_cast<const char*>(a.res) + ((size_t)mw * a.res_ps + n0) * 4;
+      const float* bp = a.bias + n0 + (lane & 7) * 4;
+#define HANDS_EPI(ACT)                                                                               \
+      if (a.res != nullptr) epilogue_full_ht<ACT, true>(acc, sH, lane, bp, ru, a.res_ps, ou, a.out_ps); \
+      else                  epilogue_full_ht<ACT, false>(acc, sH, lane, bp, ru, a.res_ps, ou, a.out_ps)
+      if (a.relu == HANDS_ACT_RELU) { HANDS_EPI(HANDS_ACT_RELU); }
+      else if (a.relu == HANDS_ACT_NONE) { HANDS_EPI(HANDS_ACT_NONE); }
+      else if (a.relu == HANDS_ACT_LEAKY_RELU) { HANDS_EPI(HANDS_ACT_LEAKY_RELU); }
+      else { HANDS_EPI(HANDS_ACT_GELU); }
+#undef HANDS_EPI
+      return;
+    }
+    const bool has_res = a.res != nullptr;
+    const int mbase = m0 + wm * 32 + (lane >> 3);
+#pragma unroll
+    for (int i = 0; i < 2; ++i) {
+#pragma unroll
+      for (int q = 0; q < 4; ++q)
+        *reinterpret_cast<float4*>(sH + (lane & 31) * EROW_H + q * 8 + (lane >> 5) * 4) =
+            make_float4(acc[i][0][q * 4 + 0], acc[i][0][q * 4 + 1], acc[i][0][q * 4 + 2], acc[i][0][q * 4 + 3]);
+      const int n_lane = n0 + i * 32 + (lane & 7) * 4;
+      const bool n_ok = n_lane < a.N;
+      const float4 bv = *reinterpret_cast<const float4*>(a.bias + n_lane);
+      float4 rv[4];
+#pragma unroll
+      for (int r = 0; r < 4; ++r) {
+        const int m = mbase + 8 * r;
+        const int mc = m < a.M ? m : a.M - 1;
+        rv[r] = has_res ? *reinterpret_cast<const float4*>(a.res + (size_t)mc * a.res_ps + (n_ok ? n_lane : 0))
+                        : make_float4(0.f, 0.f, 0.f, 0.f);
+      }
+#pragma unroll
+      for (int r = 0; r < 4; ++r) {
+        const int m = mbase + 8 * r;
+        const float4 t = *reinterpret_cast<const float4*>(sH + ((lane >> 3) + 8 * r) * EROW_H + (lane & 7) * 4);
+        float4 v;
+        v.x = t.x + bv.x + rv[r].x;
+        v.y = t.y + bv.y + rv[r].y;
+        v.z = t.z + bv.z + rv[r].z;
+        v.w = t.w + bv.w + rv[r].w;
+        v = apply_act(v, a.relu);
+        if (m < a.M && n_ok) *reinterpret_cast<float4*>(a.out + (size_t)m * a.out_ps + n_lane) = v;
+      }
+    }
+  } else {
+    float* sE = lds + wave * (32 * EROW);
+    const int half = lane >> 5;
+    const int c4 = lane & 15;
+    const int n_lane = n0 + wn * 64 + c4 * 4;
+    const bool n_ok = n_lane < a.N;
+    const bool part = a.ksplit > 1;
 #ifdef HANDS_ABL_NO_EPI
-  if (!part && m0 + BM <= a.M && n0 + BN <= a.N) {
-    float sacc = 0.f;
-#pragma unroll
-    for (int i = 0; i < 2; ++i)
-#pragma unroll
-      for (int j = 0; j < 2; ++j) sacc += acc[i][j][0] + acc[i][j][7] + acc[i][j][15];
-    if (sacc == 123456.789f) a.out[(size_t)m0 * a.out_ps + n0 + lane] = sacc;
-    return;
-  }
+    if (!part && m0 + BM <= a.M && n0 + BN <= a.N) {
+      float sacc = 0.f;
+#pragma unroll
+      for (int i = 0; i < 2; ++i)
+#pragma unroll
+        for (int j = 0; j < NJ; ++j) sacc += acc[i][j][0] + acc[i][j][7] + acc[i][j][15];
+      if (sacc == 123456.789f) a.out[(size_t)m0 * a.out_ps + n0 + lane] = sacc;
+      return;
+    }
 #endif
-  if (!F64 && !part && m0 + BM <= a.M && n0 + BN <= a.N) {
-    const int wave_u = __builtin_amdgcn_readfirstlane(wave);
-    const int mw = m0 + (wave_u / WAVES_N) * 64, nw = n0 + (wave_u % WAVES_N) * 64;
-    char* ou = reinterpret_cast<char*>(a.out) + ((size_t)mw * a.out_ps + nw) * 4;
-    const char* ru = reinterpret_cast<const char*>(a.res) + ((size_t)mw * a.res_ps + nw) * 4;
-    const float* bp = a.bias + n_lane;
+    if (!F64 && !part && m0 + BM <= a.M && n0 + BN <= a.N) {
+      const int wave_u = __builtin_amdgcn_readfirstlane(wave);
+      const int mw = m0 + (wave_u / WAVES_N) * 64, nw = n0 + (wave_u % WAVES_N) * 64;
+      char* ou = reinterpret_cast<char*>(a.out) + ((size_t)mw * a.out_ps + nw) * 4;
+      const char* ru = reinterpret_cast<const char*>(a.res) + ((size_t)mw * a.res_ps + nw) * 4;
+      const float* bp = a.bias + n_lane;
 #define HANDS_EPI(ACT)                                                                            \
-    if (a.res != nullptr) epilogue_full<ACT, true>(acc, sE, lane, bp, ru, a.res_ps, ou, a.out_ps); \
-    else                  epilogue_full<ACT, false>(acc, sE, lane, bp, ru, a.res_ps, ou, a.out_ps)
-    if (a.relu == HANDS_ACT_RELU) { HANDS_EPI(HANDS_ACT_RELU); }
-    else if (a.relu == HANDS_ACT_NONE) { HANDS_EPI(HANDS_ACT_NONE); }
-    else if (a.relu == HANDS_ACT_LEAKY_RELU) { HANDS_EPI(HANDS_ACT_LEAKY_RELU); }
-    else { HANDS_EPI(HANDS_ACT_GELU); }
+      if (a.res != nullptr) epilogue_full<ACT, true>(acc, sE, lane, bp, ru, a.res_ps, ou, a.out_ps); \
+      else                  epilogue_full<ACT, false>(acc, sE, lane, bp, ru, a.res_ps, ou, a.out_ps)
+      if (a.relu == HANDS_ACT_RELU) { HANDS_EPI(HANDS_ACT_RELU); }
+      else if (a.relu == HANDS_ACT_NONE) { HANDS_EPI(HANDS_ACT_NONE); }
+      else if (a.relu == HANDS_ACT_LEAKY_RELU) { HANDS_EPI(HANDS_ACT_LEAKY_RELU); }
+      else { HANDS_EPI(HANDS_ACT_GELU); }
 #undef HANDS_EPI
-    return;
-  }
-  const float4 bv = (part || F64) ? make_float4(0.f, 0.f, 0.f, 0.f) : *reinterpret_cast<const float4*>(a.bias + n_lane);
-  double bd[F64 ? 4 : 1][F64 ? 4 : 1];
-  if constexpr (F64) {
-#pragma unroll
-    for (int i = 0; i < 4; ++i)
-#pragma unroll
-      for (int r = 0; r < 4; ++r) {
-        const int ch = n0 + wn * 64 + 16 * i + (lane >> 4) + 4 * r;
-        bd[i][r] = (!part && ch < a.N) ? (double)a.bias[ch] : 0.0;
+      return;
+    }
+    const float4 bv = (part || F64) ? make_float4(0.f, 0.f, 0.f, 0.f) : *reinterpret_cast<const float4*>(a.bias + n_lane);
+    double bd[F64 ? 4 : 1][F64 ? 4 : 1];
+    if constexpr (F64) {
+#pragma unroll
+      for (int i = 0; i < 4; ++i)
+#pragma unroll
+        for (int r = 0; r < 4; ++r) {
+          const int ch = n0 + wn * 64 + 16 * i + (lane >> 4) + 4 * r;
+          bd[i][r] = (!part && ch < a.N) ? (double)a.bias[ch] : 0.0;
+        }
+      if (part) {
+        double* pd = reinterpret_cast<double*>(a.partial) + (size_t)split * a.M * a.part_ps;
+#pragma unroll
+        for (int i = 0; i < 4; ++i)
+#pragma unroll
+          for (int jb = 0; jb < 4; ++jb)
+#pragma unroll
+            for (int r = 0; r < 4; ++r) {
+              const int ch = n0 + wn * 64 + 16 * i + (lane >> 4) + 4 * r;
+              const int m = m0 + wm * 64 + 16 * jb + (lane & 15);
+              if (m < a.M && ch < a.N) pd[(size_t)m * a.part_ps + ch] = accd[i][jb][r];
+            }
+        return;
       }
-    if (part) {
-      double* pd = reinterpret_cast<double*>(a.partial) + (size_t)split * a.M * a.part_ps;
-#pragma unroll
-      for (int i = 0; i < 4; ++i)
-#pragma unroll
-        for (int jb = 0; jb < 4; ++jb)
-#pragma unroll
-          for (int r = 0; r < 4; ++r) {
-            const int ch = n0 + wn * 64 + 16 * i + (lane >> 4) + 4 * r;
-            const int m = m0 + wm * 64 + 16 * jb + (lane & 15);
-            if (m < a.M && ch < a.N) pd[(size_t)m * a.part_ps + ch] = accd[i][jb][r];
-          }
-      return;
-    }
-  }
-  const bool has_res = !part && a.res != nullptr;
-  const int act = part ? HANDS_ACT_NONE : a.relu;
-  float* const obase = part ? a.partial + (size_t)split * a.M * a.part_ps : a.out;
-  const int ops = part ? a.part_ps : a.out_ps;
-#pragma unroll
-  for (int j = 0; j < 2; ++j) {
-    if constexpr (F64) {
-#pragma unroll
-      for (int i = 0; i < 4; ++i)
-#pragma unroll
-        for (int jj = 0; jj < 2; ++jj)
-#pragma unroll
-          for (int r = 0; r < 4; ++r)
-            sE[(jj * 16 + (lane & 15)) * EROW + 16 * i + (lane >> 4) + 4 * r] = (float)(accd[i][2 * j + jj][r] + bd[i][r]);
-    } else {
-#pragma unroll
-    for (int i = 0; i < 2; ++i)
-#pragma unroll
-      for (int q = 0; q < 4; ++q)
-        *reinterpret_cast<float4*>(sE + (lane & 31) * EROW + i * 32 + q * 8 + half * 4) =
-            make_float4(acc[i][j][q * 4 + 0], acc[i][j][q * 4 + 1], acc[i][j][q * 4 + 2], acc[i][j][q * 4 + 3]);
-    }
-    const int mbase = m0 + wm * 64 + j * 32 + (lane >> 4);
-    float4 rv[8];
-#pragma unroll
-    for (int r = 0; r < 8; ++r) {
-      const int m = mbase + 4 * r;
-      const int mc = m < a.M ? m : a.M - 1;
-      rv[r] = has_res ? *reinterpret_cast<const float4*>(a.res + (size_t)mc * a.res_ps + (n_ok ? n_lane : 0))
-                      : make_float4(0.f, 0.f, 0.f, 0.f);
-    }
-#pragma unroll
-    for (int r = 0; r < 8; ++r) {
-      const int m = mbase + 4 * r;
-      const float4 t = *reinterpret_cast<const float4*>(sE + ((lane >> 4) + 4 * r) * EROW + c4 * 4);
-      float4 v;
-      v.x = t.x + bv.x + rv[r].x;
-      v.y = t.y + bv.y + rv[r].y;
-      v.z = t.z + bv.z + rv[r].z;
-      v.w = t.w + bv.w + rv[r].w;
-      v = apply_act(v, act);
-      if (m < a.M && n_ok) *reinterpret_cast<float4*>(obase + (size_t)m * ops + n_lane) = v;
+    }
+    const bool has_res = !part && a.res != nullptr;
+    const int act = part ? HANDS_ACT_NONE : a.relu;
+    float* const obase = part ? a.partial + (size_t)split * a.M * a.part_ps : a.out;
+    const int ops = part ? a.part_ps : a.out_ps;
+#pragma unroll
+    for (int j = 0; j < 2; ++j) {
+      if constexpr (F64) {
+#pragma unroll
+        for (int i = 0; i < 4; ++i)
+#pragma unroll
+          for (int jj = 0; jj < 2; ++jj)
+#pragma unroll
+            for (int r = 0; r < 4; ++r)
+              sE[(jj * 16 + (lane & 15)) * EROW + 16 * i + (lane >> 4) + 4 * r] = (float)(accd[i][2 * j + jj][r] + bd[i][r]);
+      } else {
+#pragma unroll
+      for (int i = 0; i < 2; ++i)
+#pragma unroll
+        for (int q = 0; q < 4; ++q)
+          *reinterpret_cast<float4*>(sE + (lane & 31) * EROW + i * 32 + q * 8 + half * 4) =
+              make_float4(acc[i][j][q * 4 + 0], acc[i][j][q * 4 + 1], acc[i][j][q * 4 + 2], acc[i][j][q * 4 + 3]);
+      }
+      const int mbase = m0 + wm * 64 + j * 32 + (lane >> 4);
+      float4 rv[8];
+#pragma unroll
+      for (int r = 0; r < 8; ++r) {
+        const int m = mbase + 4 * r;
+        const int mc = m < a.M ? m : a.M - 1;
+        rv[r] = has_res ? *reinterpret_cast<const float4*>(a.res + (size_t)mc * a.res_ps + (n_ok ? n_lane : 0))
+                        : make_float4(0.f, 0.f, 0.f, 0.f);
+      }
+#pragma unroll
+      for (int r = 0; r < 8; ++r) {
+        const int m = mbase + 4 * r;
+        const float4 t = *reinterpret_cast<const float4*>(sE + ((lane >> 4) + 4 * r) * EROW + c4 * 4);
+        float4 v;
+        v.x = t.x + bv.x + rv[r].x;
+        v.y = t.y + bv.y + rv[r].y;
+        v.z = t.z + bv.z + rv[r].z;
+        v.w = t.w + bv.w + rv[r].w;
+        v = apply_act(v, act);
+        if (m < a.M && n_ok) *reinterpret_cast<float4*>(obase + (size_t)m * ops + n_lane) = v;
+      }
     }
   }
 #undef LOAD_TILES
@@ -677,6 +775,28 @@
     tile_coords(a, tile, mt, nt);
     splitk_fused_tail<64 * WAVES_M, 64 * WAVES_N, PREC == 2>(a, lds, tile, mt * 64 * WAVES_M, nt * 64 * WAVES_N, wave_u);
   }
+}
+
+constexpr int HT_BM = 128, HT_BN = 64;
+constexpr int HT_RING = 2 * (HT_BM + HT_BN) * LDS_ROW;
+static_assert(EPI_FLOATS_H <= HT_RING, "the half-height epilogue reuses the ring");
+#ifndef HANDS_HT_WAVES
+#define HANDS_HT_WAVES 5
+#endif
+__global__ void __launch_bounds__(256) __attribute__((amdgpu_waves_per_eu(HANDS_HT_WAVES, HANDS_HT_WAVES)))
+conv_igemm_ht_f32_kernel(ConvArgs a) {
+  __shared__ __attribute__((aligned(16))) float lds[HT_RING];
+  const int ntiles = a.nblk_m * a.nblk_n;
+  conv_tile<4, 1, 2, 0, false, 0, 1>(a, lds, xcd_remap(blockIdx.x, ntiles), 0, 0, a.Kpad / BK, nullptr, nullptr);
+}
+
+int launch_ht(ConvArgs& a, hipStream_t stream) {
+  a.nblk_m = (a.M + HT_BM - 1) / HT_BM;
+  a.nblk_n = (a.N + HT_BN - 1) / HT_BN;
+  const long long nwg = (long long)a.nblk_m * a.nblk_n;
+  if (nwg <= 0 || nwg > 0x7fffffffLL) return HANDS_EINVAL;
+  hipLaunchKernelGGL(conv_igemm_ht_f32_kernel, dim3((unsigned)nwg), dim3(256), 0, stream, a);
+  return (int)hipGetLastError();
 }
 
 constexpr int GROUP_MAX = 8;
@@ -1058,9 +1178,9 @@
                          : launch_streamk<2, 2, 0>(a, s, workspace, workspace_bytes, epoch);
 }
 
-extern "C" int hands_conv1x1_dual_nhwc_f32(const hands_conv_desc* d, const float* in, const float* in2, int Cin2, int H2,
-                                           int W2, int stride2, int in2_pix_stride, const float* w_packed,
-                                           const float* bias, float* out, hands_stream_t stream) {
+namespace {
+int dual_launch(const hands_conv_desc* d, const float* in, const float* in2, int Cin2, int H2, int W2, int stride2,
+                int in2_pix_stride, const float* w_packed, const float* bias, float* out, hands_stream_t stream, bool ht) {
   if (!d || !in || !in2 || !w_packed || !bias || !out) return HANDS_EINVAL;
   if (d->B <= 0 || d->KH != 1 || d->KW != 1 || d->stride != 1 || d->pad != 0 || d->H != d->Ho || d->W != d->Wo)
     return HANDS_EINVAL;
@@ -1078,12 +1198,42 @@
       return HANDS_EINVAL;
   }
   if (d->act & HANDS_ACC_F64) return HANDS_EINVAL;
+  if (ht && (d->act < 0 || d->act > HANDS_ACT_LEAKY_RELU)) return HANDS_EINVAL;
   ConvArgs a;
   fill_plain_args(d, in, w_packed, bias, nullptr, out, nullptr, nullptr, a);
   a.in2 = in2; a.K0 = d->Cin; a.H2 = H2; a.W2 = W2; a.stride2 = stride2; a.in2_ps = in2_pix_stride;
+  if (ht) return launch_ht(a, (hipStream_t)stream);
   hands_conv_desc one_chain = *d;
   one_chain.act &= ~(HANDS_SUM_BLOCK128 | HANDS_SUM_BLOCK64);
   return launch_conv(&one_chain, a, false, (d->act & HANDS_MATH_BF16X3) != 0, (hipStream_t)stream);
+}
+
+bool half_tile_ok(const hands_conv_desc* d) {
+  return d && conv_geometry_ok(d) && pointwise_route_ok(d) && (d->act & ~HANDS_ACT_MASK) == 0;
+}
+}
+
+extern "C" int hands_conv1x1_dual_nhwc_f32(const hands_conv_desc* d, const float* in, const float* in2, int Cin2, int H2,
+                                           int W2, int stride2, int in2_pix_stride, const float* w_packed,
+                                           const float* bias, float* out, hands_stream_t stream) {
+  return dual_launch(d, in, in2, Cin2, H2, W2, stride2, in2_pix_stride, w_packed, bias, out, stream, false);
+}
+
+extern "C" int hands_conv1x1_dual_nhwc_ht_f32(const hands_conv_desc* d, const float* in, const float* in2, int Cin2, int H2,
+                                              int W2, int stride2, int in2_pix_stride, const float* w_packed,
+                                              const float* bias, float* out, hands_stream_t stream) {
+  return dual_launch(d, in, in2, Cin2, H2, W2, stride2, in2_pix_stride, w_packed, bias, out, stream, true);
+}
+
+extern "C" int hands_conv2d_ht_supported(const hands_conv_desc* d) { return half_tile_ok(d) ? 1 : 0; }
+
+extern "C" int hands_conv2d_nhwc_ht_f32(const hands_conv_desc* d, const float* in, const float* w_packed, const float* bias,
+                                        const float* residual, float* out, hands_stream_t stream) {
+  if (!d || !in || !w_packed || !bias || !out) return HANDS_EINVAL;
+  if (!half_tile_ok(d) || !residual_ok(d, residual)) return HANDS_EINVAL;
+  ConvArgs a;
+  fill_plain_args(d, in, w_packed, bias, residual, out, nullptr, nullptr, a);
+  return launch_ht(a, (hipStream_t)stream);
 }
 
 namespace {
diff --git a/hands_amd/engine.py b/hands_amd/engine.py
--- a/hands_amd/engine.py
+++ b/hands_amd/engine.py
@@ -10,6 +10,14 @@
 MATH_BF16X3 = 0x100
 _SUM_BLOCK = {128: 0x200, 64: 0x400}
 ACC_F64 = 0x800
+
+
+HALF_TILE_MAX_PLAIN_TILES = 128
+
+
+def half_tile_rule(Kpad, Cout, M):
+    plain_tiles = -(-M // 256) if Cout <= 64 else -(-M // 128) * -(-Cout // 128)
+    return plain_tiles <= HALF_TILE_MAX_PLAIN_TILES
 
 
 class ConvEngine:
@@ -33,6 +41,7 @@
         self.acc64 = True
         self.fuse_splitk_reduce = True
         self.group_launches = True
+        self.half_tile = False
         self.last_acc64 = False
         self.hook = None
         self.last_wino_macs = 0
@@ -46,7 +55,7 @@
     def clone_settings(self) -> "ConvEngine":
         e = ConvEngine()
         for k in ("use_splitk", "latency_mode", "overlap", "fuse_stem_pool", "fuse_downsample", "winograd", "winograd4", "fuse_mano", "fuse_pre", "stream_k", "math", "chain_limit",
-                  "chain_min_k", "chain_max_pix", "chain_skip_tokens", "chain_in_kernel", "acc64", "group_launches", "fuse_splitk_reduce"):
+                  "chain_min_k", "chain_max_pix", "chain_skip_tokens", "chain_in_kernel", "acc64", "group_launches", "fuse_splitk_reduce", "half_tile"):
             setattr(e, k, getattr(self, k))
         return e
 
@@ -109,6 +118,8 @@
         if acc64:
             d.act |= ACC_F64
         if kind == "dual":
+            if not acc64 and fp32 and self._half_tile(pc.Kpad, pc.Cout, d.B * d.Ho * d.Wo):
+                return _Route("dual_half", 1, 0, False, "conv_igemm_ht_f32_kernel")
             return _Route("dual", 1, 0, acc64, "conv_igemm_f32_kernel")
         S = 1
         if kind == "conv":
@@ -150,7 +161,15 @@
         if (not sum_block and not acc64 and fp32 and ((not self.overlap) if self.stream_k == "auto" else self.stream_k)
                 and L.hands_conv2d_streamk_grid(C.byref(d)) > 0 and not self._capturing(L, stream)):
             return _Route("streamk", S, 0, False, "conv_igemm_sk_f32_kernel")
+        if (kind == "conv" and not sum_block and not acc64 and fp32 and self._half_tile(pc.Kpad, pc.Cout, d.B * d.Ho * d.Wo)
+                and L.hands_conv2d_ht_supported(C.byref(d))):
+            return _Route("half", S, 0, False, "conv_igemm_ht_f32_kernel")
         return _Route("plain", S, sum_block, acc64, "conv_igemm_f32_kernel")
+
+    def _half_tile(self, Kpad, Cout, M):
+        if not self.half_tile or self.latency_mode:
+            return False
+        return self.half_tile == "force" or half_tile_rule(Kpad, Cout, M)
 
     def _launch(self, kernel, pc, npix, stream, has_res, fn, *args):
         hook = self.hook
@@ -187,6 +206,8 @@
             fn, args = L.hands_conv2d_nhwc_streamk_f32, (dp, xp, wp, bp, rp, op, ptr(sk[0]), sk[0].numel() * 4, sk[1], stream)
         elif r.entry == "plain":
             fn, args = L.hands_conv2d_nhwc_f32, (dp, xp, wp, bp, rp, op, stream)
+        elif r.entry == "half":
+            fn, args = L.hands_conv2d_nhwc_ht_f32, (dp, xp, wp, bp, rp, op, stream)
         else:
             ws = self._workspace(x.device, stream, L.hands_conv2d_workspace_floats(dp, r.S), r.capturing) if r.S > 1 else None
             wsp, wsn = (ptr(ws), ws.numel()) if ws is not None else (None, 0)
@@ -235,10 +256,12 @@
         K0, K1, stride2 = split
         d = ConvDesc(B, Ho, Wo, K0, Ho, Wo, pc.Cout, 1, 1, 1, 0, K0, pc.Cout, 0, pc.Kpad,
                      int(act) | (MATH_BF16X3 if self.math == "bf16x3" else 0))
-        if self._route(L, pc, d, stream, "dual").acc64:
+        r = self._route(L, pc, d, stream, "dual")
+        if r.acc64:
             raise ValueError("hands_amd: conv_dual has no fp64 accumulation (hands_conv1x1_dual_nhwc_f32): a layer marked acc64 "
                              "takes its conv3 and downsample as separate launches")
-        self._launch("conv_igemm_f32_kernel", pc, B * Ho * Wo, stream, False, L.hands_conv1x1_dual_nhwc_f32,
+        self._launch(r.kernel, pc, B * Ho * Wo, stream, False,
+                     L.hands_conv1x1_dual_nhwc_ht_f32 if r.entry == "dual_half" else L.hands_conv1x1_dual_nhwc_f32,
                      C.byref(d), ptr(x), ptr(x2), K1, H2, W2, stride2, K1, ptr(pc.w), ptr(pc.bias), ptr(out, out_off), stream)
 
     def stem_pool(self, L, pc, x4, x_off, out, B, H, W, act, stream):
diff --git a/hands_amd/hands_light.py b/hands_amd/hands_light.py
--- a/hands_amd/hands_light.py
+++ b/hands_amd/hands_light.py
@@ -44,6 +44,7 @@
         self.engine = ConvEngine()
         self.winograd4_stages = (1, 2, 3, 4)
         self.engine.winograd4 = True
+        self.engine.half_tile = True
         self.trunk_chunks = (1, 2)
         self.async_tail = True
         self._calls = 0
@@ -100,6 +101,7 @@
         if vit:
             self.vit_conv = vit_conv_params()
             self.trunk_chunks = (1, 1)
+            self.engine.half_tile = False
         self.enc_channels = ({1: 4, 2: 16, 3: 20}[IMAGE_ENC[pos_enc]] * self.n_freq if self.enc_mode == "image" else
                              4 * self.n_freq if self.enc_mode == "dense" else 0)
         if self.separate_hands:
diff --git a/include/hands_hip.h b/include/hands_hip.h
--- a/include/hands_hip.h
+++ b/include/hands_hip.h
@@ -94,6 +94,13 @@
 int hands_conv1x1_dual_nhwc_f32(const hands_conv_desc* d, const float* in, const float* in2, int Cin2, int H2,
                                 int W2, int stride2, int in2_pix_stride, const float* w_packed,
                                 const float* bias, float* out, hands_stream_t stream);
+
+int hands_conv2d_ht_supported(const hands_conv_desc* d);
+int hands_conv2d_nhwc_ht_f32(const hands_conv_desc* d, const float* in, const float* w_packed, const float* bias,
+                             const float* residual, float* out, hands_stream_t stream);
+int hands_conv1x1_dual_nhwc_ht_f32(const hands_conv_desc* d, const float* in, const float* in2, int Cin2, int H2,
+                                   int W2, int stride2, int in2_pix_stride, const float* w_packed,
+                                   const float* bias, float* out, hands_stream_t stream);
 
 int hands_stem_conv_maxpool_nhwc_f32(const float* x4, const float* w_packed, const float* bias, float* out,
                                      int B, int H, int W, int act, hands_stream_t stream);
```

After: 12160 hands/s. About the same (-0.0%).
